# ExistentialRobotics/CORSAIR

Hardware: AMD Instinct MI355X
Metric: end-to-end queries/sec (embed+retrieve+register), Scan2CAD chair (higher is better)
Workload: dtype f32 sparse conv + embedding / f64 RANSAC, k-NN, Chamfer, top-k / f16 MFMA bounds and shortlists (survivors recounted in f64)

## Files before the change

### corsair_amd/_lib.py

```python
from __future__ import annotations

import ctypes
import threading
import os
import re
from ctypes import POINTER, c_char_p, c_double, c_float, c_int, c_int32, c_int64, c_uint64, c_void_p

_HERE = os.path.dirname(os.path.abspath(__file__))
LIB_PATH = os.environ.get("CORSAIR_HIP_LIB") or os.path.join(_HERE, "csrc", "libcorsair_hip.so")
HEADER_PATH = os.path.join(os.path.dirname(_HERE), "include", "corsair_hip.h")

_lib = None


class CorsairHipError(RuntimeError):
    """Raised when a cs_* entry point returns a negative status (message = cs_last_error())."""


def _declare(lib):
    vp = c_void_p
    sigs = {
        "cs_last_error": (c_char_p, []),
        "cs_version": (c_int, []),
        "cs_device_count": (c_int, []),
        "cs_coordmap_create": (c_int, [vp, c_int64, c_int, vp, POINTER(vp)]),
        "cs_coordmap_stride": (c_int, [vp, c_int, vp, POINTER(vp)]),
        "cs_coordmap_pyramid": (c_int, [vp, c_int64, c_int, c_int, c_int, vp, POINTER(vp)]),
        "cs_coordmap_size": (c_int64, [vp]),
        "cs_coordmap_tensor_stride": (c_int, [vp]),
        "cs_coordmap_coords": (vp, [vp]),
        "cs_coordmap_free": (None, [vp]),
        "cs_kernelmap_build": (c_int, [vp, vp, c_int, c_int, vp, POINTER(vp)]),
        "cs_kernelmap_build_many": (c_int, [c_int, POINTER(vp), POINTER(vp), POINTER(c_int), POINTER(c_int), vp, POINTER(vp)]),
        "cs_kernelmap_num_pairs": (c_int64, [vp]),
        "cs_kernelmap_rows": (c_int64, [vp]),
        "cs_kernelmap_table": (vp, [vp]),
        "cs_kernelmap_export": (c_int64, [vp, vp, vp, vp, c_int64, vp]),
        "cs_kernelmap_free": (None, [vp]),
        "cs_conv_fwd": (c_int, [vp, c_int64, c_int64, vp, c_int, c_int, vp, c_int, vp, vp, vp,
                                c_int, c_int, vp, c_int, vp]),
        "cs_conv_wgrad": (c_int, [vp, c_int64, c_int64, vp, c_int, c_int, vp, c_int, c_int, vp, vp]),
        "cs_affine_act": (c_int, [c_int64, c_int, vp, c_int, vp, vp, vp, c_int, c_int, vp, c_int, vp]),
        "cs_row_l2_normalize": (c_int, [c_int64, c_int, vp, c_int, c_float, vp, c_int, vp]),
        "cs_segmented_max": (c_int, [c_int64, c_int, vp, c_int, vp, c_int, c_int, vp, vp]),
        "cs_instance_norm": (c_int, [c_int64, c_int, vp, c_int, vp, c_int, vp, vp, c_float, vp, c_int, vp]),
        "cs_voxelize": (c_int, [vp, POINTER(c_int64), c_int, c_double, vp, vp, POINTER(c_int64), vp]),
        "cs_voxelize_f64": (c_int, [vp, POINTER(c_int64), c_int, c_double, vp, vp, POINTER(c_int64), vp]),
        "cs_l2_topk": (c_int, [vp, c_int64, vp, c_int64, c_int, c_int, vp, vp, vp]),
        "cs_l2_topk_sq": (c_int, [vp, c_int64, vp, c_int64, c_int, c_int, vp, vp, vp]),
        "cs_knn_feat": (c_int, [vp, POINTER(c_int64), vp, POINTER(c_int64), POINTER(c_int32),
                                POINTER(c_int32), c_int, c_int, c_int, vp, vp, vp, vp, vp, vp]),
        "cs_chamfer_1dir": (c_int, [vp, POINTER(c_int64), vp, POINTER(c_int64), POINTER(c_int32),
                                    POINTER(c_int32), c_int, vp, vp, vp]),
        "cs_chamfer_2dir": (c_int, [vp, POINTER(c_int64), vp, POINTER(c_int64), POINTER(c_int32),
                                    POINTER(c_int32), c_int, vp, vp, vp]),
        "cs_hausdorff_1dir": (c_int, [vp, POINTER(c_int64), vp, POINTER(c_int64), POINTER(c_int32),
                                      POINTER(c_int32), c_int, vp, vp, vp]),
        "cs_ransac_batch": (c_int, [vp, vp, POINTER(c_int64), c_int, c_double, c_int, c_int, c_double,
                                    c_uint64, vp, vp, vp, vp, vp]),
        "cs_ransac_prefilter_stats": (None, [POINTER(c_uint64), c_int]),
        "cs_knn_shortlist_stats": (None, [POINTER(c_uint64), c_int]),
        "cs_chamfer_f16_stats": (None, [POINTER(c_uint64), c_int]),
        "cs_l2_topk_stats": (None, [POINTER(c_uint64), c_int]),
        "cs_topk_catalog_create": (c_int, [vp, c_int64, c_int, vp, POINTER(vp)]),
        "cs_l2_topk_catalog": (c_int, [vp, c_int64, vp, c_int, vp, vp, c_int, vp]),
        "cs_topk_catalog_free": (None, [vp]),
        "cs_symcut_fit": (c_int, [vp, c_int, vp, POINTER(c_int64), c_int, vp, c_int,
                                  POINTER(c_int32), c_int, c_int, c_int, vp, vp, vp, vp, vp]),
        "cs_symcut_labels": (c_int, [vp, POINTER(c_int64), c_int, POINTER(c_int32), vp, vp, vp]),
        "cs_partition_by_label": (c_int, [vp, vp, c_int, vp, vp]),
        "cs_cfg_bad": (c_int, [vp, c_int, vp, c_int, vp, vp]),
        "cs_rows_nonfinite": (c_int, [vp, c_int, vp, c_int, vp, vp]),
        "cs_corr_assemble": (c_int, [vp, vp, vp, vp, c_int, vp, c_int, c_int64, vp, vp, vp]),
        "cs_radius_pairs": (c_int, [vp, POINTER(c_int64), vp, POINTER(c_int64), POINTER(c_int32), POINTER(c_int32),
                                    c_int, c_double, c_int, vp, vp, POINTER(vp)]),
        "cs_radius_pairs_fill": (c_int, [vp, vp, vp, vp]),
        "cs_radius_plan_free": (None, [vp]),
        "cs_sample_pairs": (c_int, [vp, POINTER(c_int64), POINTER(c_int32), POINTER(c_int32), POINTER(c_int32),
                                    POINTER(c_int32), c_int, POINTER(c_int64), vp, vp, c_int, c_uint64, c_int,
                                    c_double, c_int, vp, vp, vp, vp, vp]),
        "cs_transform_f64": (c_int, [vp, POINTER(c_int64), POINTER(c_int32), c_int, vp, vp, vp]),
        "cs_pair_loss_fwd": (c_int, [c_int, POINTER(vp), POINTER(c_int64), POINTER(c_int32), c_int, c_int,
                                     POINTER(c_int32), POINTER(c_int32), POINTER(c_int32), POINTER(c_float),
                                     POINTER(c_double), POINTER(vp), POINTER(c_int64), vp, vp, vp]),
        "cs_pair_loss_bwd": (c_int, [c_int, POINTER(vp), POINTER(c_int64), POINTER(c_int32), c_int, c_int,
                                     POINTER(c_int32), POINTER(c_int32), POINTER(c_int32), POINTER(c_float),
                                     POINTER(c_double), POINTER(vp), POINTER(c_int64), vp, POINTER(vp),
                                     POINTER(c_int32), vp]),
        "cs_hardest_negatives": (c_int, [vp, c_int, vp, POINTER(c_int64), vp, c_int, vp, POINTER(c_int64),
                                         POINTER(c_int32), POINTER(c_int32), c_int, c_int, vp, c_int64, c_double, vp, vp,
                                         vp]),
        "cs_hardest_stats": (None, [POINTER(c_uint64), c_int]),
        "cs_icp_batch": (c_int, [vp, POINTER(c_int64), vp, POINTER(c_int64), POINTER(c_int32), POINTER(c_int32), c_int, vp,
                                 c_double, c_int, c_double, c_double, vp, vp, vp, vp, vp, vp, vp, vp]),
        "cs_icp_stats": (None, [POINTER(c_uint64), c_int]),
        "cs_icp_plane_batch": (c_int, [vp, POINTER(c_int64), vp, vp, POINTER(c_int64), POINTER(c_int32), POINTER(c_int32),
                                       c_int, vp, c_double, c_int, c_double, c_double, vp, vp, vp, vp, vp, vp, vp, vp]),
        "cs_icp_plane_robust_batch": (c_int, [vp, POINTER(c_int64), vp, vp, POINTER(c_int64), POINTER(c_int32),
                                              POINTER(c_int32), c_int, vp, c_double, c_int, c_double, c_double, c_int,
                                              c_double, vp, vp, vp, vp, vp, vp, vp, vp, vp]),
        "cs_icp_scale_batch": (c_int, [vp, POINTER(c_int64), vp, vp, POINTER(c_int64), POINTER(c_int32), POINTER(c_int32),
                                       c_int, vp, c_double, c_int, c_double, c_double, c_double, c_double, vp, vp, vp, vp,
                                       vp, vp, vp, vp, vp]),
        "cs_icp_gicp_batch": (c_int, [vp, vp, POINTER(c_int64), vp, vp, POINTER(c_int64), POINTER(c_int32), POINTER(c_int32),
                                      c_int, vp, c_double, c_int, c_double, c_double, c_double, vp, vp, vp, vp, vp, vp, vp,
                                      vp, vp]),
        "cs_estimate_normals": (c_int, [vp, POINTER(c_int64), c_int, c_int, vp, vp]),
        "cs_estimate_normals_hybrid": (c_int, [vp, POINTER(c_int64), c_int, c_double, c_int, vp, vp]),
        "cs_normals_stats": (None, [POINTER(c_uint64), c_int]),
        "cs_fgr_batch": (c_int, [vp, vp, POINTER(c_int64), c_int, c_double, c_double, c_double, c_int, c_int, c_double,
                                 c_int, c_uint64, vp, vp, vp, vp, vp, vp, vp]),
        "cs_prof_enable": (None, [c_int]),
        "cs_prof_reset": (None, []),
        "cs_prof_get": (c_int, [c_char_p, POINTER(c_double), POINTER(c_int64)]),
        "cs_prof_get_units": (c_int, [c_char_p, POINTER(c_double)]),
        "cs_pool_trim": (None, []),
        "cs_pool_stats": (None, [POINTER(c_uint64)]),
    }
    for name, (res, args) in sigs.items():
        fn = getattr(lib, name)
        fn.restype = res
        fn.argtypes = args
    return sigs


def header_symbols():
    with open(HEADER_PATH) as f:
        text = f.read()
    text = re.sub(r"/\*.*?\*/", "", text, flags=re.S)
    return sorted(set(re.findall(r"\b(cs_[a-z0-9_]+)\s*\(", text)))


def load():
    global _lib
    if _lib is None:
        if not os.path.exists(LIB_PATH):
            raise ImportError(
                f"{LIB_PATH} is missing: build it with `python -c 'import __graft_entry__ as g; "
                "g.build()'` (hipcc --offload-arch=gfx950). There is no CPU fallback."
            )
        lib = ctypes.CDLL(LIB_PATH)
        _declare(lib)
        _lib = lib
    return _lib


def check(rc):
    if rc < 0:
        raise CorsairHipError(load().cs_last_error().decode("utf-8", "replace"))
    return rc


def require_gpu():
    if load().cs_device_count() < 1:
        raise CorsairHipError("no HIP device visible: the corsair_amd hot path has no CPU fallback")


def ptr(t):
    if t is None:
        return None
    return c_void_p(t.data_ptr())


def stream_ptr():
    import torch

    return c_void_p(torch.cuda.current_stream().cuda_stream)


def i64_array(values):
    arr = (c_int64 * len(values))(*[int(v) for v in values])
    return arr


def i32_array(values):
    arr = (c_int32 * len(values))(*[int(v) for v in values])
    return arr


def prof_enable(on=True):
    load().cs_prof_enable(1 if on else 0)


def prof_reset():
    load().cs_prof_reset()


def prof_get(name):
    ms = c_double(0.0)
    n = c_int64(0)
    check(load().cs_prof_get(name.encode(), ctypes.byref(ms), ctypes.byref(n)))
    units = c_double(0.0)
    check(load().cs_prof_get_units(name.encode(), ctypes.byref(units)))
    return ms.value, n.value, units.value


_pinned = threading.local()


def to_host(*tensors):
    import torch

    cache = getattr(_pinned, "bufs", None)
    if cache is None:
        cache = _pinned.bufs = {}
    staged = []
    for i, t in enumerate(tensors):
        t = t.detach()
        key = (i, tuple(t.shape), t.dtype)
        buf = cache.get(key)
        if buf is None:
            if len(cache) > 64:
                cache.clear()
            buf = cache[key] = torch.empty(t.shape, dtype=t.dtype, pin_memory=True)
        buf.copy_(t, non_blocking=True)
        staged.append(buf)
    ev = torch.cuda.Event()
    ev.record()
    ev.synchronize()
    return [b.numpy().copy() for b in staged]
```

### corsair_amd/backend.py

```python
from __future__ import annotations

import ctypes
from ctypes import c_void_p
from typing import NamedTuple, Optional

import numpy as np
import torch

from . import _lib
from ._lib import check, i32_array, i64_array, ptr, stream_ptr

KERNEL_VOLUME = 27


def _dev(t, dtype, what):
    if not isinstance(t, torch.Tensor) or not t.is_cuda:
        raise _lib.CorsairHipError(f"{what} must be a device tensor (the HIP path has no CPU fallback)")
    if t.dtype != dtype:
        raise TypeError(f"{what} must be {dtype}, got {t.dtype}")
    return t


def _rows(t, what):
    if t.dim() != 2 or t.stride(1) != 1:
        raise ValueError(f"{what} must be 2-D with unit inner stride")
    return t, t.stride(0) if t.shape[0] > 1 else max(t.stride(0), t.shape[1])


class CoordMap:

    def __init__(self, handle, device):
        self._h = c_void_p(handle)
        self.device = device
        lib = _lib.load()
        self.n = int(lib.cs_coordmap_size(self._h))
        self.tensor_stride = int(lib.cs_coordmap_tensor_stride(self._h))
        self._coords = None

    @classmethod
    def create(cls, coords, tensor_stride=1):
        _lib.require_gpu()
        coords = _dev(coords, torch.int32, "coordinates").contiguous()
        if coords.dim() != 2 or coords.shape[1] != 4:
            raise ValueError("coordinates must be int32 [N, 4] (batch, x, y, z)")
        out = c_void_p()
        check(_lib.load().cs_coordmap_create(ptr(coords), coords.shape[0], tensor_stride,
                                             stream_ptr(), ctypes.byref(out)))
        return cls(out.value, coords.device)

    @classmethod
    def pyramid(cls, coords, n_levels=4, n_batch=0, tensor_stride=1):
        _lib.require_gpu()
        coords = _dev(coords, torch.int32, "coordinates").contiguous()
        if coords.dim() != 2 or coords.shape[1] != 4:
            raise ValueError("coordinates must be int32 [N, 4] (batch, x, y, z)")
        outs = (c_void_p * n_levels)()
        check(_lib.load().cs_coordmap_pyramid(ptr(coords), coords.shape[0], tensor_stride, n_levels, int(n_batch or 0),
                                              stream_ptr(), outs))
        return [cls(h, coords.device) for h in outs]

    def stride(self, s=2):
        out = c_void_p()
        check(_lib.load().cs_coordmap_stride(self._h, s, stream_ptr(), ctypes.byref(out)))
        return CoordMap(out.value, self.device)

    @property
    def coords(self):
        if self._coords is None:
            t = torch.empty((self.n, 4), dtype=torch.int32, device=self.device)
            if self.n:
                src = _lib.load().cs_coordmap_coords(self._h)
                _hip_memcpy_d2d(t.data_ptr(), src, self.n * 16)
            self._coords = t
        return self._coords

    def __del__(self):
        try:
            if self._h:
                _lib.load().cs_coordmap_free(self._h)
                self._h = None
        except Exception:
            pass


def _hip_memcpy_d2d(dst, src, nbytes):
    import ctypes as C

    hip = _hip_runtime()
    rc = hip.hipMemcpyAsync(c_void_p(dst), c_void_p(src), C.c_size_t(nbytes), 3,
                            c_void_p(torch.cuda.current_stream().cuda_stream))
    if rc != 0:
        raise _lib.CorsairHipError(f"hipMemcpyAsync failed with {rc}")


_hip = None


def _hip_runtime():
    global _hip
    if _hip is None:
        _hip = ctypes.CDLL("libamdhip64.so")
    return _hip


class KernelMap:

    def __init__(self, handle, in_map, out_map, transposed, kernel_size=3):
        self._h = c_void_p(handle)
        self.kvol = int(kernel_size) ** 3
        lib = _lib.load()
        self.n_out = int(lib.cs_kernelmap_rows(self._h))
        self.n_in = in_map.n
        self._num_pairs = None
        self.transposed = transposed
        self.stride1 = not transposed and in_map.tensor_stride == out_map.tensor_stride
        self.device = in_map.device

    @property
    def num_pairs(self):
        if self._num_pairs is None:
            self._num_pairs = int(_lib.load().cs_kernelmap_num_pairs(self._h))
        return self._num_pairs

    @classmethod
    def build(cls, in_map, out_map, kernel_size=3, transposed=False):
        out = c_void_p()
        check(_lib.load().cs_kernelmap_build(in_map._h, out_map._h, kernel_size,
                                             1 if transposed else 0, stream_ptr(),
                                             ctypes.byref(out)))
        return cls(out.value, in_map, out_map, transposed, kernel_size)

    @classmethod
    def build_many(cls, specs):
        full = [(sp[0], sp[1], sp[2] if len(sp) > 2 else 3, bool(sp[3]) if len(sp) > 3 else False) for sp in specs]
        n = len(full)
        if n == 0:
            return []
        VP, CI = c_void_p * n, ctypes.c_int * n
        ins = VP(*[sp[0]._h.value for sp in full])
        outs = VP(*[sp[1]._h.value for sp in full])
        ks = CI(*[int(sp[2]) for sp in full])
        tr = CI(*[1 if sp[3] else 0 for sp in full])
        kms = VP()
        check(_lib.load().cs_kernelmap_build_many(n, ins, outs, ks, tr, stream_ptr(), kms))
        return [cls(kms[i], full[i][0], full[i][1], full[i][3], full[i][2]) for i in range(n)]

    def export(self):
        n = max(self.num_pairs, 1)
        k = torch.empty(n, dtype=torch.int32, device=self.device)
        i = torch.empty(n, dtype=torch.int32, device=self.device)
        o = torch.empty(n, dtype=torch.int32, device=self.device)
        got = check(_lib.load().cs_kernelmap_export(self._h, ptr(k), ptr(i), ptr(o), n, stream_ptr()))
        return k[:got], i[:got], o[:got]

    def table(self):
        t = torch.empty((self.n_out, KERNEL_VOLUME), dtype=torch.int32, device=self.device)
        if self.n_out:
            _hip_memcpy_d2d(t.data_ptr(), _lib.load().cs_kernelmap_table(self._h), self.n_out * 27 * 4)
        return t

    def __del__(self):
        try:
            if self._h:
                _lib.load().cs_kernelmap_free(self._h)
                self._h = None
        except Exception:
            pass


def conv_fwd(kmap, x, weight, scale=None, shift=None, residual=None, relu=False, out=None,
             n_out=None):
    x, ld_in = _rows(_dev(x, torch.float32, "input features"), "input features")
    weight = _dev(weight, torch.float32, "kernel").contiguous()
    if weight.dim() == 2:
        cin, cout = weight.shape
    else:
        cin, cout = weight.shape[1], weight.shape[2]
    if x.shape[1] != cin:
        raise ValueError(f"input has {x.shape[1]} channels, kernel expects {cin}")
    n_in = x.shape[0]
    if kmap is None:
        n_out = n_in
    else:
        n_out = kmap.n_out
    if out is None:
        out = torch.empty((n_out, cout), dtype=torch.float32, device=x.device)
    out, ld_out = _rows(out, "output")
    if out.shape[0] != n_out or out.shape[1] != cout:
        raise ValueError("output buffer has the wrong shape")
    ld_res = 0
    if residual is not None:
        residual, ld_res = _rows(_dev(residual, torch.float32, "residual"), "residual")
    check(_lib.load().cs_conv_fwd(kmap._h if kmap is not None else None, n_in, n_out, ptr(x), ld_in,
                                  cin, ptr(weight), cout, ptr(scale), ptr(shift), ptr(residual),
                                  ld_res, 1 if relu else 0, ptr(out), ld_out, stream_ptr()))
    return out


def conv_wgrad(kmap, x, g):
    x, ld_in = _rows(_dev(x, torch.float32, "input features"), "input features")
    g, ld_g = _rows(_dev(g, torch.float32, "output gradient"), "output gradient")
    n_in, cin = x.shape
    n_out, cout = g.shape
    if kmap is not None and (kmap.n_in, kmap.n_out) != (n_in, n_out):
        raise ValueError(f"kernel map is for {kmap.n_in} -> {kmap.n_out} rows, tensors have {n_in} -> {n_out}")
    kvol = 1 if kmap is None else kmap.kvol
    dw = torch.empty((cin, cout) if kvol == 1 else (kvol, cin, cout), dtype=torch.float32, device=x.device)
    check(_lib.load().cs_conv_wgrad(kmap._h if kmap is not None else None, n_in, n_out, ptr(x), ld_in, cin, ptr(g),
                                    ld_g, cout, ptr(dw), stream_ptr()))
    return dw


def dgrad_weight(kmap, weight):
    if kmap is None or kmap.kvol == 1:
        return weight.reshape(weight.shape[-2:]).t().contiguous()
    if kmap.stride1:
        return weight.flip(0).transpose(1, 2).contiguous()
    return weight.transpose(1, 2).contiguous()


def conv_dgrad(kmap, rev_kmap, g, weight):
    wt = dgrad_weight(kmap, weight)
    if kmap is None:
        return conv_fwd(None, g, wt)
    if kmap.stride1:
        rev_kmap = kmap if rev_kmap is None else rev_kmap
    if rev_kmap is None or (rev_kmap.n_in, rev_kmap.n_out, rev_kmap.kvol) != (kmap.n_out, kmap.n_in, kmap.kvol):
        raise ValueError("conv_dgrad: the reverse map must take the forward's output rows to its input rows")
    return conv_fwd(rev_kmap, g, wt)


def affine_act(x, scale=None, shift=None, residual=None, relu=False, out=None):
    x, ld_in = _rows(_dev(x, torch.float32, "input"), "input")
    if out is None:
        out = torch.empty((x.shape[0], x.shape[1]), dtype=torch.float32, device=x.device)
    out, ld_out = _rows(out, "output")
    ld_res = 0
    if residual is not None:
        residual, ld_res = _rows(residual, "residual")
    check(_lib.load().cs_affine_act(x.shape[0], x.shape[1], ptr(x), ld_in, ptr(scale), ptr(shift),
                                    ptr(residual), ld_res, 1 if relu else 0, ptr(out), ld_out,
                                    stream_ptr()))
    return out


def row_l2_normalize(x, eps=0.0, out=None):
    if out is None and torch.is_grad_enabled() and x.requires_grad:
        from .autograd import RowL2NormalizeFunction

        return RowL2NormalizeFunction.apply(x, float(eps))
    x, ld_in = _rows(_dev(x, torch.float32, "input"), "input")
    if out is None:
        out = torch.empty((x.shape[0], x.shape[1]), dtype=torch.float32, device=x.device)
    out, ld_out = _rows(out, "output")
    check(_lib.load().cs_row_l2_normalize(x.shape[0], x.shape[1], ptr(x), ld_in, float(eps), ptr(out),
                                          ld_out, stream_ptr()))
    return out


def segmented_max(x, coords, n_batch):
    if torch.is_grad_enabled() and x.requires_grad:
        from .autograd import SegmentedMaxFunction

        return SegmentedMaxFunction.apply(x, coords, int(n_batch))
    x, ld_in = _rows(_dev(x, torch.float32, "input"), "input")
    coords = _dev(coords, torch.int32, "coords")
    out = torch.empty((n_batch, x.shape[1]), dtype=torch.float32, device=x.device)
    check(_lib.load().cs_segmented_max(x.shape[0], x.shape[1], ptr(x), ld_in, ptr(coords),
                                       coords.stride(0), n_batch, ptr(out), stream_ptr()))
    return out


def instance_norm(x, seg, weight=None, bias=None, eps=1e-8, out=None):
    x, ld_in = _rows(_dev(x, torch.float32, "input"), "input")
    seg = _dev(seg, torch.int32, "segment offsets").contiguous()
    if out is None:
        out = torch.empty((x.shape[0], x.shape[1]), dtype=torch.float32, device=x.device)
    out, ld_out = _rows(_dev(out, torch.float32, "output"), "output")
    if out.shape != x.shape:
        raise ValueError("instance_norm: output buffer has the wrong shape")
    w = _dev(weight, torch.float32, "weight").contiguous().reshape(-1) if weight is not None else None
    b = _dev(bias, torch.float32, "bias").contiguous().reshape(-1) if bias is not None else None
    for t, name in ((w, "weight"), (b, "bias")):
        if t is not None and t.numel() != x.shape[1]:
            raise ValueError("instance_norm: %s must have %d entries" % (name, x.shape[1]))
    check(_lib.load().cs_instance_norm(x.shape[0], x.shape[1], ptr(x), ld_in, ptr(seg), seg.numel() - 1,
                                       ptr(w) if w is not None else None, ptr(b) if b is not None else None,
                                       float(eps), ptr(out), ld_out, stream_ptr()))
    return out


def voxelize(xyz, offsets, voxel_size):
    f64 = torch.is_tensor(xyz) and xyz.dtype == torch.float64
    xyz = _dev(xyz, torch.float64 if f64 else torch.float32, "xyz").contiguous()
    n = xyz.shape[0]
    nseg = len(offsets) - 1
    keep = torch.empty(max(n, 1), dtype=torch.int64, device=xyz.device)
    grid = torch.empty((max(n, 1), 4), dtype=torch.int32, device=xyz.device)
    h_off = i64_array(offsets)
    h_out = (ctypes.c_int64 * (nseg + 1))()
    fn = _lib.load().cs_voxelize_f64 if f64 else _lib.load().cs_voxelize
    check(fn(ptr(xyz), h_off, nseg, float(voxel_size), ptr(keep), ptr(grid), h_out, stream_ptr()))
    out_off = [int(v) for v in h_out]
    m = out_off[-1]
    return keep[:m], grid[:m], out_off


class TopkCatalog:

    def __init__(self, x):
        self.x = _dev(x, torch.float32, "catalog").contiguous()
        out = c_void_p()
        check(_lib.load().cs_topk_catalog_create(ptr(self.x), self.x.shape[0], self.x.shape[1], stream_ptr(),
                                                 ctypes.byref(out)))
        self._h = out
        self.shape = self.x.shape

    def __del__(self):
        try:
            if self._h:
                _lib.load().cs_topk_catalog_free(self._h)
                self._h = None
        except Exception:
            pass


def l2_topk(q, x, k, return_distance=False, squared=False):
    q = _dev(q, torch.float32, "queries").contiguous()
    idx = torch.empty((q.shape[0], k), dtype=torch.int64, device=q.device)
    dist = torch.empty((q.shape[0], k), dtype=torch.float64, device=q.device) if return_distance else None
    if isinstance(x, TopkCatalog):
        if x.shape[1] != q.shape[1]:
            raise ValueError("query and catalog dimensions differ")
        check(_lib.load().cs_l2_topk_catalog(ptr(q), q.shape[0], x._h, k, ptr(idx), ptr(dist), 1 if squared else 0,
                                             stream_ptr()))
        return (idx, dist) if return_distance else idx
    x = _dev(x, torch.float32, "catalog").contiguous()
    fn = _lib.load().cs_l2_topk_sq if squared else _lib.load().cs_l2_topk
    check(fn(ptr(q), q.shape[0], ptr(x), x.shape[0], q.shape[1], k, ptr(idx), ptr(dist), stream_ptr()))
    return (idx, dist) if return_distance else idx


def knn_feat(qf, qoff, tf, toff, k, qseg=None, tseg=None, qlabel=None, tlabel=None, perm=None,
             return_distance=False):
    qf = _dev(qf, torch.float32, "query features").contiguous()
    tf = _dev(tf, torch.float32, "target features").contiguous()
    if qseg is None:
        qseg = list(range(len(qoff) - 1))
        tseg = list(range(len(toff) - 1))
    n_prob = len(qseg)
    total = sum(int(qoff[s + 1]) - int(qoff[s]) for s in qseg)
    idx = torch.empty((total, k), dtype=torch.int32, device=qf.device)
    dist = torch.empty((total, k), dtype=torch.float64, device=qf.device) if return_distance else None
    check(_lib.load().cs_knn_feat(ptr(qf), i64_array(qoff), ptr(tf), i64_array(toff), i32_array(qseg),
                                  i32_array(tseg), n_prob, qf.shape[1], k, ptr(qlabel), ptr(tlabel),
                                  ptr(perm), ptr(idx), ptr(dist), stream_ptr()))
    return (idx, dist) if return_distance else idx


def hardest_negatives(qf, qxyz, qoff, tf, txyz, toff, anchors, radius, qseg=None, tseg=None, return_distance=False):
    qf, ld_q = _rows(_dev(qf, torch.float32, "query features"), "query features")
    tf, ld_t = _rows(_dev(tf, torch.float32, "target features"), "target features")
    qxyz = _dev(qxyz, torch.float32, "query points").contiguous()
    txyz = _dev(txyz, torch.float32, "target points").contiguous()
    anchors = _dev(anchors, torch.int32, "anchors").contiguous()
    if qf.shape[1] != tf.shape[1]:
        raise ValueError("hardest_negatives: query and target widths differ")
    if qxyz.shape != (qf.shape[0], 3) or txyz.shape != (tf.shape[0], 3):
        raise ValueError("hardest_negatives: points must be [n, 3], one row per feature row")
    if anchors.dim() != 1:
        raise ValueError("hardest_negatives: anchors must be 1-D")
    if qseg is None:
        qseg = list(range(len(qoff) - 1))
        tseg = list(range(len(toff) - 1))
    if len(qseg) != len(tseg):
        raise ValueError("hardest_negatives: qseg and tseg differ in length")
    if qseg and (int(qoff[max(qseg) + 1]) > qf.shape[0] or int(toff[max(tseg) + 1]) > tf.shape[0]):
        raise ValueError("hardest_negatives: the offset tables exceed the feature matrices")
    n = anchors.shape[0]
    idx = torch.empty(n, dtype=torch.int32, device=qf.device)
    dist = torch.empty(n, dtype=torch.float64, device=qf.device) if return_distance else None
    check(_lib.load().cs_hardest_negatives(ptr(qf), ld_q, ptr(qxyz), i64_array(qoff), ptr(tf), ld_t, ptr(txyz),
                                           i64_array(toff), i32_array(qseg), i32_array(tseg), len(qseg),
                                           int(qf.shape[1]), ptr(anchors), n, float(radius), ptr(idx), ptr(dist),
                                           stream_ptr()))
    return (idx, dist) if return_distance else idx


def hardest_stats(reset=False):
    out = (ctypes.c_uint64 * 2)()
    _lib.load().cs_hardest_stats(out, 1 if reset else 0)
    return int(out[0]), int(out[1])


def chamfer_1dir(src, soff, tgt, toff, src_seg, tgt_seg, T):
    src = _dev(src, torch.float32, "source").contiguous()
    tgt = _dev(tgt, torch.float32, "target").contiguous()
    T = _dev(T, torch.float32, "transforms").contiguous()
    n_prob = len(src_seg)
    out = torch.empty(n_prob, dtype=torch.float64, device=src.device)
    check(_lib.load().cs_chamfer_1dir(ptr(src), i64_array(soff), ptr(tgt), i64_array(toff),
                                      i32_array(src_seg), i32_array(tgt_seg), n_prob, ptr(T), ptr(out),
                                      stream_ptr()))
    return out


def chamfer_2dir(src, soff, tgt, toff, src_seg, tgt_seg, T):
    src = _dev(src, torch.float32, "source").contiguous()
    tgt = _dev(tgt, torch.float32, "target").contiguous()
    T = _dev(T, torch.float32, "transforms").contiguous()
    n_prob = len(src_seg)
    if len(tgt_seg) != n_prob or T.numel() != 16 * n_prob:
        raise ValueError("chamfer_2dir: %d source segments, %d target segments, %d transform entries"
                         % (n_prob, len(tgt_seg), T.numel()))
    if src.dim() != 2 or src.shape[1] != 3 or tgt.dim() != 2 or tgt.shape[1] != 3:
        raise ValueError("chamfer_2dir: clouds must be [n,3]")
    for name, off, seg, rows in (("source", soff, src_seg, src.shape[0]), ("target", toff, tgt_seg, tgt.shape[0])):
        if n_prob and not (0 <= min(seg) and max(seg) + 1 < len(off)):
            raise ValueError("chamfer_2dir: a %s segment id is outside its offset table" % name)
        if n_prob and not (0 <= int(min(off)) and int(max(off)) <= rows):
            raise ValueError("chamfer_2dir: the %s offset table exceeds the cloud (%d rows)" % (name, rows))
    out = torch.empty((n_prob, 2), dtype=torch.float64, device=src.device)
    if n_prob == 0:
        return out
    check(_lib.load().cs_chamfer_2dir(ptr(src), i64_array(soff), ptr(tgt), i64_array(toff),
                                      i32_array(src_seg), i32_array(tgt_seg), n_prob, ptr(T), ptr(out),
                                      stream_ptr()))
    return out


def hausdorff_1dir(src, soff, tgt, toff, src_seg, tgt_seg, T):
    src = _dev(src, torch.float32, "source").contiguous()
    tgt = _dev(tgt, torch.float32, "target").contiguous()
    T = _dev(T, torch.float32, "transforms").contiguous()
    n_prob = len(src_seg)
    out = torch.empty(n_prob, dtype=torch.float64, device=src.device)
    check(_lib.load().cs_hausdorff_1dir(ptr(src), i64_array(soff), ptr(tgt), i64_array(toff),
                                        i32_array(src_seg), i32_array(tgt_seg), n_prob, ptr(T), ptr(out),
                                        stream_ptr()))
    return out


class IcpResult(NamedTuple):
    T: torch.Tensor
    T32: torch.Tensor
    fitness: torch.Tensor
    rmse: torch.Tensor
    iters: torch.Tensor
    ncorr: torch.Tensor
    corr: Optional[torch.Tensor]
    corr_off: Optional[list]
    wfitness: Optional[torch.Tensor] = None
    scale: Optional[torch.Tensor] = None
    mrmse = None


class GicpResult(IcpResult):
    def __new__(cls, *fields, mrmse=None):
        self = super().__new__(cls, *fields)
        self.mrmse = mrmse
        return self


ICP_KERNELS = {"l2": 0, "huber": 1, "cauchy": 2, "tukey": 3}


def estimate_normals(xyz, offsets, k=16, radius=None):
    xyz = _dev(xyz, torch.float32, "points").contiguous()
    if xyz.dim() != 2 or xyz.shape[1] != 3:
        raise ValueError("estimate_normals: points must be [n, 3]")
    if len(offsets) < 1 or int(offsets[-1]) > xyz.shape[0]:
        raise ValueError("estimate_normals: the offset table exceeds the point array")
    out = torch.empty_like(xyz)
    if radius is None:
        check(_lib.load().cs_estimate_normals(ptr(xyz), i64_array(offsets), len(offsets) - 1, int(k), ptr(out), stream_ptr()))
    else:
        check(_lib.load().cs_estimate_normals_hybrid(ptr(xyz), i64_array(offsets), len(offsets) - 1, float(radius), int(k),
                                                     ptr(out), stream_ptr()))
    return out


def normals_stats(reset=False):
    out = (ctypes.c_uint64 * 2)()
    _lib.load().cs_normals_stats(out, 1 if reset else 0)
    return int(out[0]), int(out[1])


def icp_batch(src, soff, tgt, toff, src_seg, tgt_seg, T0, max_dist, max_iter=30, relative_fitness=1e-6,
              relative_rmse=1e-6, return_corr=False, tgt_normals=None, kernel="l2", kernel_scale=None, with_scaling=False,
              scale_bounds=(0.5, 2.0), *, estimation=None, src_normals=None, gicp_epsilon=1e-3):
    if estimation not in (None, "gicp"):
        raise ValueError("icp_batch: estimation must be None or 'gicp', got %r" % (estimation,))
    gicp = estimation == "gicp"
    if gicp:
        if kernel != "l2" or with_scaling:
            raise ValueError("icp_batch: estimation 'gicp' with a robust kernel or with_scaling is out of scope")
        if tgt_normals is None or src_normals is None:
            raise ValueError("icp_batch: estimation 'gicp' needs tgt_normals and src_normals")
        eps = float(gicp_epsilon)
        if not (np.isfinite(eps) and 2.0 ** -10 <= eps <= 1.0):
            raise ValueError("icp_batch: gicp_epsilon must lie in [2^-10, 1], got %r" % (gicp_epsilon,))
    elif src_normals is not None:
        raise ValueError("icp_batch: src_normals are used by estimation = 'gicp' only")
    if with_scaling:
        if kernel != "l2":
            raise ValueError("icp_batch: with_scaling with a robust kernel (%r) is out of scope: robust kernels exist for "
                             "the rigid plane estimation only" % (kernel,))
        try:
            smin, smax = float(scale_bounds[0]), float(scale_bounds[1])
        except (TypeError, ValueError, IndexError):
            raise ValueError("icp_batch: scale_bounds must be a pair (min, max), got %r" % (scale_bounds,))
        if not (np.isfinite(smin) and np.isfinite(smax) and 0.0 < smin <= 1.0 <= smax):
            raise ValueError("icp_batch: scale_bounds must be finite with 0 < min <= 1 <= max, got %r" % (scale_bounds,))
    if kernel not in ICP_KERNELS:
        raise ValueError("icp_batch: kernel must be one of %s, got %r" % (sorted(ICP_KERNELS), kernel))
    if kernel != "l2" and tgt_normals is None:
        raise ValueError("icp_batch: kernel %r needs tgt_normals (robust kernels exist for the plane estimation only)"
                         % (kernel,))
    if kernel != "l2" and kernel_scale is None:
        raise ValueError("icp_batch: kernel %r needs a kernel_scale" % (kernel,))
    src = _dev(src, torch.float32, "source").contiguous()
    tgt = _dev(tgt, torch.float32, "target").contiguous()
    T0 = _dev(T0, torch.float32, "initial transforms").contiguous()
    n_prob = len(src_seg)
    if len(tgt_seg) != n_prob:
        raise ValueError("icp_batch: src_seg and tgt_seg differ in length")
    if T0.numel() != 16 * n_prob:
        raise ValueError("icp_batch: one 4x4 initial transform per problem")
    if src.dim() != 2 or src.shape[1] != 3 or tgt.dim() != 2 or tgt.shape[1] != 3:
        raise ValueError("icp_batch: points must be [n, 3]")
    sane = all(0 <= int(s) < len(soff) - 1 for s in src_seg) and all(0 <= int(t) < len(toff) - 1 for t in tgt_seg)
    if n_prob and sane and (int(soff[max(src_seg) + 1]) > src.shape[0] or int(toff[max(tgt_seg) + 1]) > tgt.shape[0]):
        raise ValueError("icp_batch: the offset tables exceed the point arrays")
    if n_prob and not sane and min(min(src_seg), min(tgt_seg)) >= 0:
        raise ValueError("icp_batch: a segment id exceeds its offset table")
    dev = src.device
    T = torch.empty((n_prob, 4, 4), dtype=torch.float64, device=dev)
    T32 = torch.empty((n_prob, 4, 4), dtype=torch.float32, device=dev)
    fitness = torch.empty(n_prob, dtype=torch.float64, device=dev)
    rmse = torch.empty(n_prob, dtype=torch.float64, device=dev)
    iters = torch.empty(n_prob, dtype=torch.int32, device=dev)
    ncorr = torch.empty(n_prob, dtype=torch.int32, device=dev)
    corr = corr_off = None
    if return_corr:
        lens = [int(soff[s + 1]) - int(soff[s]) for s in src_seg] if sane else []
        corr_off = np.concatenate([[0], np.cumsum(lens)]).astype(np.int64).tolist()
        corr = torch.full((max(corr_off[-1], 1),), -1, dtype=torch.int32, device=dev)
    head = (i64_array(toff), i32_array(src_seg), i32_array(tgt_seg), n_prob, ptr(T0), float(max_dist), int(max_iter),
            float(relative_fitness), float(relative_rmse))
    tail = head + (ptr(T), ptr(T32), ptr(fitness), ptr(rmse), ptr(iters), ptr(ncorr), ptr(corr), stream_ptr())
    wfitness = scale = None
    nrm = None
    if tgt_normals is not None:
        nrm = _dev(tgt_normals, torch.float32, "target normals").contiguous()
        if nrm.shape != tgt.shape:
            raise ValueError("icp_batch: tgt_normals must have the shape of the target points")
    mrmse = None
    if gicp:
        snrm = _dev(src_normals, torch.float32, "source normals").contiguous()
        if snrm.shape != src.shape:
            raise ValueError("icp_batch: src_normals must have the shape of the source points")
        mrmse = torch.empty(n_prob, dtype=torch.float64, device=dev)
        check(_lib.load().cs_icp_gicp_batch(
            ptr(src), ptr(snrm), i64_array(soff), ptr(tgt), ptr(nrm), *head, eps, ptr(T), ptr(T32), ptr(fitness), ptr(rmse),
            ptr(mrmse), ptr(iters), ptr(ncorr), ptr(corr), stream_ptr()))
    elif with_scaling:
        scale = torch.empty(n_prob, dtype=torch.float64, device=dev)
        check(_lib.load().cs_icp_scale_batch(
            ptr(src), i64_array(soff), ptr(tgt), ptr(nrm), *head, smin, smax, ptr(T), ptr(T32), ptr(fitness), ptr(rmse),
            ptr(scale), ptr(iters), ptr(ncorr), ptr(corr), stream_ptr()))
    elif nrm is None:
        check(_lib.load().cs_icp_batch(ptr(src), i64_array(soff), ptr(tgt), *tail))
    else:
        if kernel == "l2":
            check(_lib.load().cs_icp_plane_batch(ptr(src), i64_array(soff), ptr(tgt), ptr(nrm), *tail))
        else:
            wfitness = torch.empty(n_prob, dtype=torch.float64, device=dev)
            check(_lib.load().cs_icp_plane_robust_batch(
                ptr(src), i64_array(soff), ptr(tgt), ptr(nrm), *head, ICP_KERNELS[kernel], float(kernel_scale), ptr(T),
                ptr(T32), ptr(fitness), ptr(rmse), ptr(wfitness), ptr(iters), ptr(ncorr), ptr(corr), stream_ptr()))
    if corr is not None:
        corr = corr[:corr_off[-1]]
    if gicp:
        return GicpResult(T, T32, fitness, rmse, iters, ncorr, corr, corr_off, wfitness, scale, mrmse=mrmse)
    return IcpResult(T, T32, fitness, rmse, iters, ncorr, corr, corr_off, wfitness, scale)


def icp_stats(reset=False):
    out = (ctypes.c_uint64 * 2)()
    _lib.load().cs_icp_stats(out, 1 if reset else 0)
    return int(out[0]), int(out[1])


def ransac_batch(src, tgt, offsets, max_corr, ransac_n=10, max_iter=100000, confidence=0.999, seed=0):
    src = _dev(src, torch.float32, "source correspondences").contiguous()
    tgt = _dev(tgt, torch.float32, "target correspondences").contiguous()
    n_prob = len(offsets) - 1
    dev = src.device
    T = torch.empty((n_prob, 4, 4), dtype=torch.float32, device=dev)
    inl = torch.empty(n_prob, dtype=torch.int32, device=dev)
    rmse = torch.empty(n_prob, dtype=torch.float64, device=dev)
    iters = torch.empty(n_prob, dtype=torch.int32, device=dev)
    check(_lib.load().cs_ransac_batch(ptr(src), ptr(tgt), i64_array(offsets), n_prob, float(max_corr),
                                      ransac_n, max_iter, float(confidence), int(seed), ptr(T),
                                      ptr(inl), ptr(rmse), ptr(iters), stream_ptr()))
    return T, inl, rmse, iters


class FgrResult(NamedTuple):
    T: torch.Tensor
    T64: torch.Tensor
    inliers: torch.Tensor
    rmse: torch.Tensor
    iters: torch.Tensor
    n_tuple: torch.Tensor


def fgr_batch(src, tgt, offsets, max_corr, mu_floor=0.025, division_factor=1.4, iteration_number=64, tuple_test=True,
              tuple_scale=0.95, max_tuple=1000, seed=0):
    src = _dev(src, torch.float32, "source correspondences").contiguous()
    tgt = _dev(tgt, torch.float32, "target correspondences").contiguous()
    if src.shape != tgt.shape or src.dim() != 2 or src.shape[1] != 3:
        raise ValueError("fgr_batch: correspondences must be two [M, 3] arrays of one shape")
    if len(offsets) < 1 or int(offsets[-1]) > src.shape[0]:
        raise ValueError("fgr_batch: the offset table exceeds the correspondence arrays")
    n_prob = len(offsets) - 1
    dev = src.device
    T = torch.empty((n_prob, 4, 4), dtype=torch.float32, device=dev)
    T64 = torch.empty((n_prob, 4, 4), dtype=torch.float64, device=dev)
    inl = torch.empty(n_prob, dtype=torch.int32, device=dev)
    rmse = torch.empty(n_prob, dtype=torch.float64, device=dev)
    iters = torch.empty(n_prob, dtype=torch.int32, device=dev)
    n_tuple = torch.empty(n_prob, dtype=torch.int32, device=dev)
    check(_lib.load().cs_fgr_batch(ptr(src), ptr(tgt), i64_array(offsets), n_prob, float(max_corr), float(mu_floor),
                                   float(division_factor), int(iteration_number), 1 if tuple_test else 0,
                                   float(tuple_scale), int(max_tuple), int(seed) & 0xFFFFFFFFFFFFFFFF, ptr(T), ptr(T64),
                                   ptr(inl), ptr(rmse), ptr(iters), ptr(n_tuple), stream_ptr()))
    return FgrResult(T, T64, inl, rmse, iters, n_tuple)


def partition_by_label(label, d_off, n_cloud):
    label = _dev(label, torch.int32, "labels").contiguous()
    order = torch.empty(label.shape[0], dtype=torch.int64, device=label.device)
    check(_lib.load().cs_partition_by_label(ptr(label), ptr(d_off), n_cloud, ptr(order), stream_ptr()))
    return order


def cfg_bad(nn, d_first, n_cfg):
    nn = _dev(nn, torch.int32, "neighbour lists").contiguous()
    bad = torch.empty(n_cfg, dtype=torch.int32, device=nn.device)
    check(_lib.load().cs_cfg_bad(ptr(nn), nn.shape[1], ptr(d_first), n_cfg, ptr(bad), stream_ptr()))
    return bad


def rows_nonfinite(x, d_first, n_seg):
    x = _dev(x, torch.float32, "rows").contiguous()
    bad = torch.empty(n_seg, dtype=torch.int32, device=x.device)
    check(_lib.load().cs_rows_nonfinite(ptr(x), x.shape[1], ptr(d_first), n_seg, ptr(bad), stream_ptr()))
    return bad


def corr_assemble(xyz0, xyz1, rows, nn, desc, total, max_len):
    xyz0 = _dev(xyz0, torch.float32, "query xyz").contiguous()
    xyz1 = _dev(xyz1, torch.float32, "CAD xyz").contiguous()
    nn = _dev(nn, torch.int32, "neighbour lists").contiguous()
    k = nn.shape[1]
    dev = xyz0.device
    src = torch.empty((total * k, 3), dtype=torch.float32, device=dev)
    tgt = torch.empty((total * k, 3), dtype=torch.float32, device=dev)
    d_desc = torch.from_numpy(np.ascontiguousarray(desc, dtype=np.int64)).to(dev, non_blocking=True)
    check(_lib.load().cs_corr_assemble(ptr(xyz0), ptr(xyz1), ptr(rows) if rows is not None else None, ptr(nn), k,
                                       ptr(d_desc), len(desc), int(max_len), ptr(src), ptr(tgt), stream_ptr()))
    return src, tgt


def symcut_fit(feat, xyz, offsets, anchors, Ks, n_nn=50, n_init=10, max_iter=300):
    feat = _dev(feat, torch.float32, "features").contiguous()
    xyz = _dev(xyz, torch.float32, "xyz").contiguous()
    anchors = _dev(anchors, torch.int32, "anchors").contiguous()
    nc, na = anchors.shape
    dev = feat.device
    centers = torch.empty((nc, na, 4, 3), dtype=torch.float64, device=dev)
    counts = torch.empty((nc, na, 4), dtype=torch.int32, device=dev)
    mcd = torch.empty((nc, na), dtype=torch.float64, device=dev)
    mer = torch.empty((nc, na), dtype=torch.float64, device=dev)
    check(_lib.load().cs_symcut_fit(ptr(feat), feat.shape[1], ptr(xyz), i64_array(offsets), nc,
                                    ptr(anchors), na, i32_array(Ks), n_nn, n_init, max_iter,
                                    ptr(centers), ptr(counts), ptr(mcd), ptr(mer), stream_ptr()))
    return centers, counts, mcd, mer


def symcut_labels(xyz, offsets, Ks, sel_centers):
    xyz = _dev(xyz, torch.float32, "xyz").contiguous()
    sel_centers = _dev(sel_centers, torch.float64, "centres").contiguous()
    labels = torch.empty(xyz.shape[0], dtype=torch.int32, device=xyz.device)
    check(_lib.load().cs_symcut_labels(ptr(xyz), i64_array(offsets), len(Ks), i32_array(Ks),
                                       ptr(sel_centers), ptr(labels), stream_ptr()))
    return labels


class RadiusPlan:

    def __init__(self, handle, keep):
        self._h = c_void_p(handle)
        self._keep = keep

    def fill(self, row_ptr, total):
        idx = torch.empty(max(int(total), 1), dtype=torch.int32, device=row_ptr.device)
        check(_lib.load().cs_radius_pairs_fill(self._h, ptr(row_ptr), ptr(idx), stream_ptr()))
        return idx[:int(total)]

    def __del__(self):
        try:
            if self._h:
                _lib.load().cs_radius_plan_free(self._h)
                self._h = None
        except Exception:
            pass


def radius_pairs_begin(src, soff, tgt, toff, src_seg=None, tgt_seg=None, radius=0.03, k=None):
    src = _dev(src, torch.float64, "source points").contiguous()
    tgt = _dev(tgt, torch.float64, "target points").contiguous()
    if src_seg is None:
        src_seg = list(range(len(soff) - 1))
        tgt_seg = list(range(len(toff) - 1))
    if len(src_seg) != len(tgt_seg):
        raise ValueError("radius_pairs: src_seg and tgt_seg differ in length")
    if k is not None and int(k) < 1:
        raise ValueError("radius_pairs: k must be None or >= 1")
    rows = sum(int(soff[s + 1]) - int(soff[s]) for s in src_seg)
    row_ptr = torch.empty(rows + 1, dtype=torch.int64, device=src.device)
    plan = c_void_p()
    check(_lib.load().cs_radius_pairs(ptr(src), i64_array(soff), ptr(tgt), i64_array(toff), i32_array(src_seg),
                                      i32_array(tgt_seg), len(src_seg), float(radius), int(k or 0), ptr(row_ptr),
                                      stream_ptr(), ctypes.byref(plan)))
    return row_ptr, RadiusPlan(plan.value, (src, tgt))


def radius_pairs(src, soff, tgt, toff, src_seg=None, tgt_seg=None, radius=0.03, k=None):
    row_ptr, plan = radius_pairs_begin(src, soff, tgt, toff, src_seg, tgt_seg, radius, k)
    total = int(_lib.to_host(row_ptr[-1:])[0][0])
    return row_ptr, plan.fill(row_ptr, total)


def sample_pairs(xyz, offsets, base_seg, pos_seg, neg_seg, slots, row_base, row_ptr, tgt_idx, lists, seed, round_,
                 radius, sample, out=None):
    xyz = _dev(xyz, torch.float32, "points").contiguous()
    n_prob = len(base_seg)
    dev = xyz.device
    if out is None:
        out = tuple(torch.zeros((n_prob * sample, 2), dtype=torch.int32, device=dev) for _ in range(3)) + (
            torch.zeros((n_prob, 4), dtype=torch.int32, device=dev),)
    pip, pin, nin, counts = out
    if tgt_idx is not None and tgt_idx.numel() == 0:
        tgt_idx = torch.zeros(1, dtype=torch.int32, device=dev)
    check(_lib.load().cs_sample_pairs(ptr(xyz), i64_array(offsets), i32_array(base_seg), i32_array(pos_seg),
                                      i32_array(neg_seg), i32_array(slots), n_prob, i64_array(row_base), ptr(row_ptr),
                                      ptr(tgt_idx), int(lists), int(seed) & 0xFFFFFFFFFFFFFFFF, int(round_),
                                      float(radius), int(sample), ptr(pip), ptr(pin), ptr(nin), ptr(counts),
                                      stream_ptr()))
    return out


def transform_f64(xyz, offsets, seg, T):
    xyz = _dev(xyz, torch.float32, "points").contiguous()
    T = _dev(T, torch.float64, "transforms").contiguous()
    if T.shape[0] != len(seg):
        raise ValueError("transform_f64: one transform per segment")
    total = sum(int(offsets[s + 1]) - int(offsets[s]) for s in seg)
    out = torch.empty((max(total, 1), 3), dtype=torch.float64, device=xyz.device)
    check(_lib.load().cs_transform_f64(ptr(xyz), i64_array(offsets), i32_array(seg), len(seg), ptr(T), ptr(out),
                                       stream_ptr()))
    return out[:total]


PAIR_PULL, PAIR_PUSH = 0, 1


def _pair_loss_args(mats, terms):
    if not mats:
        raise ValueError("pair_loss: no feature matrix")
    C = int(mats[0].shape[1])
    lds = []
    for m in mats:
        _dev(m, torch.float32, "features")
        _, ld = _rows(m, "features")
        if int(m.shape[1]) != C:
            raise ValueError("pair_loss: the feature matrices differ in width")
        lds.append(ld)
    pairs = []
    for t in terms:
        p = _dev(t[2], torch.int32, "pairs")
        if p.dim() != 2 or p.shape[1] != 2:
            raise ValueError("pair_loss: pairs must be [P, 2]")
        pairs.append(p.contiguous())
    vp = (c_void_p * len(mats))(*[m.data_ptr() for m in mats])
    pp = (c_void_p * max(len(terms), 1))(*[p.data_ptr() if p.numel() else None for p in pairs])
    head = (len(mats), vp, i64_array([m.shape[0] for m in mats]), i32_array(lds), C, len(terms),
            i32_array([t[0] for t in terms]), i32_array([t[1] for t in terms]), i32_array([t[3] for t in terms]),
            (ctypes.c_float * max(len(terms), 1))(*[float(t[4]) for t in terms]),
            (ctypes.c_double * max(len(terms), 1))(*[float(t[5]) for t in terms]), pp,
            i64_array([p.shape[0] for p in pairs]))
    return head, pairs, C


def pair_loss_fwd(mats, terms, out=None):
    head, keep, _ = _pair_loss_args(mats, terms)
    dev = mats[0].device
    if out is None:
        out = (torch.empty(max(len(terms), 1), dtype=torch.float64, device=dev),
               torch.empty(1, dtype=torch.float32, device=dev))
    check(_lib.load().cs_pair_loss_fwd(*head, ptr(out[0]), ptr(out[1]), stream_ptr()))
    return out[0][:len(terms)], out[1]


def pair_loss_bwd(mats, terms, grad_up, out=None):
    head, keep, C = _pair_loss_args(mats, terms)
    g = _dev(grad_up, torch.float32, "upstream gradient").reshape(-1)
    if g.numel() != 1:
        raise ValueError("pair_loss_bwd: the upstream gradient is one scalar")
    if out is None:
        out = [torch.empty((m.shape[0], C), dtype=torch.float32, device=m.device) for m in mats]
    lds = [_rows(_dev(o, torch.float32, "gradient"), "gradient")[1] for o in out]
    gp = (c_void_p * len(out))(*[o.data_ptr() for o in out])
    check(_lib.load().cs_pair_loss_bwd(*head, ptr(g), gp, i32_array(lds), stream_ptr()))
    return out
```

### corsair_amd/csrc/ransac.hip

```cpp
#include <math.h>

#include <algorithm>
#include <atomic>
#include <vector>

#include "ransac.h"

namespace cs {

__device__ __forceinline__ int est_bound(int c, int m, int ransac_n, double log_1mc, int est_k0) {
  const double ratio = fmin(1.0, (double)c / (double)m);
  double pw = 1.0;
  for (int j = 0; j < ransac_n; ++j) pw = pw * ratio;
  const double den = log(1.0 - pw);
  if (den < 0.0) {
    const double est = log_1mc / den;
    if (est < (double)est_k0) return (int)ceil(est);
  }
  return est_k0;
}

__global__ __launch_bounds__(256) void k_ransac_scan1(RansacProb* probs, int n_prob,
                                                     const int32_t* __restrict__ res_cnt, int it0,
                                                     int bcount, int bmax, int ransac_n,
                                                     int max_iter, double log_1mc,
                                                     int32_t* __restrict__ cand, int* n_active,
                                                     const unsigned long long* __restrict__ err_by_h,
                                                     const double* __restrict__ hyp, int32_t* __restrict__ next_nsurv,
                                                     int* __restrict__ next_nactive) {
  extern __shared__ int32_t lcnt[];
  const int p = blockIdx.x;
  if (err_by_h && threadIdx.x == 0) {
    next_nsurv[p] = 0;
    if (p == 0) *next_nactive = 0;
  }
  RansacProb pr = probs[p];
  if (pr.done) return;
  const int seg = (bcount + 63) / 64;
  {
    const int32_t* g = res_cnt + (int64_t)p * bmax;
    for (int h = threadIdx.x; h < bcount; h += 256) lcnt[h + h / seg] = g[h];
  }
  __syncthreads();
  if (threadIdx.x >= 64) return;
  const int lane = threadIdx.x;
  const int32_t* cnt = lcnt + lane;
  const int s0 = lane * seg, s1 = min(bcount, s0 + seg);
  int lmax = 0;
  for (int h = s0; h < s1; ++h)
    if (it0 + h < pr.est_k) lmax = max(lmax, cnt[h]);
  int incl = lmax;
#pragma unroll
  for (int off = 1; off < 64; off <<= 1) {
    const int o = __shfl_up(incl, off);
    if (lane >= off) incl = max(incl, o);
  }
  int pre = __shfl_up(incl, 1);
  if (lane == 0) pre = 0;
  pre = max(pre, pr.best_cnt);
  int stop = 0x7fffffff;
  {
    int cur = pre;
    int ek = cur > pr.best_cnt ? est_bound(cur, pr.m, ransac_n, log_1mc, pr.est_k) : pr.est_k;
    for (int h = s0; h < s1; ++h) {
      if (it0 + h >= ek) {
        stop = h;
        break;
      }
      const int c = cnt[h];
      if (c > cur) {
        cur = c;
        ek = est_bound(cur, pr.m, ransac_n, log_1mc, pr.est_k);
      }
    }
  }
#pragma unroll
  for (int off = 32; off >= 1; off >>= 1) stop = min(stop, __shfl_xor(stop, off));
  if (stop > bcount) stop = bcount;
  int cmax = 0;
  for (int h = s0; h < min(s1, stop); ++h) cmax = max(cmax, cnt[h]);
#pragma unroll
  for (int off = 32; off >= 1; off >>= 1) cmax = max(cmax, __shfl_xor(cmax, off));
  int new_ek = pr.est_k;
  if (cmax > pr.best_cnt) new_ek = est_bound(cmax, pr.m, ransac_n, log_1mc, pr.est_k);
  int ncand = 0;
  unsigned long long e_min = ~0ULL;
  int h_min = 0x7fffffff;
  if (cmax > 0 && cmax >= pr.best_cnt) {
    if (err_by_h) {
      for (int h = s0; h < min(s1, stop); ++h)
        if (cnt[h] == cmax) {
          const unsigned long long e = err_by_h[(int64_t)p * bmax + h];
          if (e < e_min) {
            e_min = e;
            h_min = h;
          }
        }
#pragma unroll
      for (int off = 32; off >= 1; off >>= 1) {
        const unsigned long long eo = __shfl_xor(e_min, off);
        const int ho = __shfl_xor(h_min, off);
        if (eo < e_min || (eo == e_min && ho < h_min)) {
          e_min = eo;
          h_min = ho;
        }
      }
    } else {
      int mine = 0;
      for (int h = s0; h < min(s1, stop); ++h) mine += cnt[h] == cmax;
      int incl2 = mine;
#pragma unroll
      for (int off = 1; off < 64; off <<= 1) {
        const int o = __shfl_up(incl2, off);
        if (lane >= off) incl2 += o;
      }
      int pos = incl2 - mine;
      ncand = __shfl(incl2, 63);
      for (int h = s0; h < min(s1, stop); ++h)
        if (cnt[h] == cmax) cand[(int64_t)p * bmax + pos++] = h;
    }
  }
  if (lane == 0) {
    const int consumed = it0 + stop;
    pr.est_k = new_ek;
    pr.n_cand = ncand;
    pr.chunk_max = cmax;
    if (consumed >= pr.est_k || consumed >= max_iter) {
      pr.done = 1;
      pr.iters = consumed < max_iter ? consumed : max_iter;
    } else {
      atomicAdd(n_active, 1);
    }
    if (err_by_h && h_min != 0x7fffffff && (cmax > pr.best_cnt || e_min < pr.best_err)) {
      pr.best_cnt = cmax;
      pr.best_err = e_min;
      pr.best_itr = it0 + h_min;
      for (int c = 0; c < 12; ++c) pr.best_T[c] = hyp[((int64_t)p * 12 + c) * bmax + h_min];
    }
    probs[p] = pr;
  }
}

__global__ void k_ransac_scan2(RansacProb* probs, int n_prob, const double* __restrict__ hyp,
                               const int32_t* __restrict__ cand,
                               const unsigned long long* __restrict__ cand_err, int by_h, int it0,
                               int bmax, int32_t* __restrict__ next_nsurv, int* __restrict__ next_nactive) {
  const int p = blockIdx.x * blockDim.x + threadIdx.x;
  if (p >= n_prob) return;
  next_nsurv[p] = 0;
  if (p == 0) *next_nactive = 0;
  RansacProb pr = probs[p];
  if (pr.n_cand <= 0) return;
  bool changed = false;
  int best_h = -1;
  for (int c = 0; c < pr.n_cand; ++c) {
    const unsigned long long e = cand_err[(int64_t)p * bmax + (by_h ? cand[(int64_t)p * bmax + c] : c)];
    if (pr.chunk_max > pr.best_cnt || e < pr.best_err) {
      pr.best_cnt = pr.chunk_max;
      pr.best_err = e;
      best_h = cand[(int64_t)p * bmax + c];
      changed = true;
    }
  }
  pr.n_cand = 0;
  if (changed) {
    pr.best_itr = it0 + best_h;
    for (int c = 0; c < 12; ++c) pr.best_T[c] = hyp[((int64_t)p * 12 + c) * bmax + best_h];
  }
  probs[p] = pr;
}

__global__ void k_ransac_finish(const RansacProb* __restrict__ probs, int n_prob, double scale,
                                float* __restrict__ T, int32_t* __restrict__ inliers,
                                double* __restrict__ rmse, int32_t* __restrict__ iters) {
  const int p = blockIdx.x * blockDim.x + threadIdx.x;
  if (p >= n_prob) return;
  const RansacProb pr = probs[p];
  float* o = T + (int64_t)p * 16;
  if (pr.best_cnt > 0) {
    for (int c = 0; c < 12; ++c) o[c] = (float)pr.best_T[c];
  } else {
    for (int c = 0; c < 12; ++c) o[c] = (c % 5 == 0) ? 1.f : 0.f;
  }
  o[12] = 0.f;
  o[13] = 0.f;
  o[14] = 0.f;
  o[15] = 1.f;
  if (inliers) inliers[p] = pr.best_cnt;
  if (rmse)
    rmse[p] = pr.best_cnt > 0 ? sqrt(((double)pr.best_err / scale) / (double)pr.best_cnt) : 0.0;
  if (iters) iters[p] = pr.iters;
}

}

using namespace cs;

namespace {
std::atomic<unsigned long long> g_pf_stats[5];

struct PinnedScratch {
  char* p = nullptr;
  size_t n = 0;
  ~PinnedScratch() {
    if (p) (void)hipHostFree(p);
  }
};
thread_local PinnedScratch t_pinned;
char* pinned_scratch(size_t bytes) {
  if (t_pinned.n < bytes) {
    if (t_pinned.p) (void)hipHostFree(t_pinned.p);
    t_pinned.p = nullptr;
    t_pinned.n = 0;
    void* q = nullptr;
    if (hipHostMalloc(&q, bytes, hipHostMallocDefault) != hipSuccess) return nullptr;
    t_pinned.p = static_cast<char*>(q);
    t_pinned.n = bytes;
  }
  return t_pinned.p;
}

struct Options {
  bool prefilter;
  bool check;
  int pf_nm;
  bool stage2;
  int first_chunk;
  int force_jacobi;
  bool overlap;
  int trace_it0;
  const char* trace_file;
};
Options read_options() {
  const char* pf = getenv("CS_RANSAC_PREFILTER");
  const char* ck = getenv("CS_RANSAC_CHECK");
  const char* k = getenv("CS_RANSAC_PF_K");
  const char* s2 = getenv("CS_RANSAC_STAGE2");
  const char* first = getenv("CS_RANSAC_FIRST");
  const char* jac = getenv("CS_RANSAC_JACOBI");
  const char* ov = getenv("CS_RANSAC_OVERLAP");
  const char* tr = getenv("CS_PF_TRACE");
  const char* trf = getenv("CS_PF_TRACE_FILE");
  Options o;
  o.prefilter = !(pf && pf[0] == '0');
  o.check = ck && ck[0] == '1';
  o.pf_nm = (k && atoi(k) == 32) ? 2 : 1;
  o.stage2 = !(s2 && s2[0] == '0');
  o.first_chunk = ((std::min(std::max(first ? atoi(first) : 64, 64), BMAX) + 63) / 64) * 64;
  o.force_jacobi = jac && atoi(jac) != 0;
  o.overlap = !(ov && ov[0] == '0');
  o.trace_it0 = tr ? atoi(tr) : -1;
  o.trace_file = trf ? trf : "/tmp/pf_trace.bin";
  return o;
}

struct Scratch {
  int n_prob = 0;
  size_t st_probs = 0, st_surv = 0, st_cnt = 0, st_bytes = 0;
  PoolBuf<char> state;
  char* h_state = nullptr;
  PoolBuf<float> pk;
  PoolBuf<float4> pair32;
  PoolBuf<double> hyp;
  PoolBuf<int32_t> res_cnt, cand;
  PoolBuf<unsigned long long> cand_err;
  PoolBuf<int64_t> off16;
  PoolBuf<_Float16> B16, A16;
  PoolBuf<float> c_h;
  PoolBuf<int32_t> cnt_up, hlist;
  PoolBuf<unsigned> pf_stat;
  PoolBuf<double> pf_sums;
  PoolBuf<_Float16> B32, A16s;
  PoolBuf<float> c_hs;
  PoolBuf<int32_t> cnt2;
  PoolBuf<int32_t> exact_dbg;
  PoolBuf<unsigned long long> chk_stats;
  PoolBuf<int32_t> xcd_buf;
  PoolBuf<unsigned long long> trace;
  size_t trace_cap = 1;

  bool alloc(int n, int64_t tot1, int64_t rows16, int pf_nm, bool pf, bool stage2, bool check, bool tracing) {
    n_prob = n;
    st_probs = sizeof(RansacProb) * (size_t)n;
    st_surv = ((sizeof(int32_t) * (size_t)n + 7) / 8) * 8;
    st_cnt = st_surv + 8;
    st_bytes = st_probs + 2 * st_cnt;
    h_state = pinned_scratch(st_bytes);
    const size_t nb = (size_t)n * BMAX, ns2 = (size_t)n * PF_S2_CAP;
    if (tracing) trace_cap = (size_t)8 * n * 64 * 16 * 16;
    return h_state && state.alloc(st_bytes) && pk.alloc((size_t)tot1 * 6) && pair32.alloc((size_t)tot1 * 2) &&
           hyp.alloc(2 * nb * 12) && res_cnt.alloc(nb) && cand.alloc(nb) && cand_err.alloc(nb) && off16.alloc(n + 1) &&
           B16.alloc(pf ? (size_t)rows16 * pf_pitch(pf_nm) : 8) && A16.alloc(pf ? 2 * nb * PF_K : 8) &&
           c_h.alloc(pf ? 2 * nb : 1) && cnt_up.alloc(pf ? 2 * nb : 1) && hlist.alloc(pf ? nb : 1) &&
           pf_stat.alloc((size_t)n * PF_STAT) && pf_sums.alloc((size_t)n * 6) &&
           B32.alloc(stage2 ? (size_t)rows16 * PF_PITCH : 8) && A16s.alloc(stage2 ? ns2 * PF_K : 8) &&
           c_hs.alloc(stage2 ? ns2 : 1) && cnt2.alloc(stage2 ? ns2 : 1) &&
           exact_dbg.alloc(check ? nb : 1) && chk_stats.alloc(4) && xcd_buf.alloc((size_t)16 * n) && trace.alloc(trace_cap);
  }
  RansacProb* probs() const { return reinterpret_cast<RansacProb*>(state.p); }
  int32_t* nsurv(int par) const { return reinterpret_cast<int32_t*>(state.p + st_probs + par * st_cnt); }
  int* nactive(int par) const { return reinterpret_cast<int*>(state.p + st_probs + par * st_cnt + st_surv); }
  const int32_t* h_nsurv(int par) const { return reinterpret_cast<const int32_t*>(h_state + st_probs + par * st_cnt); }
  int h_nactive(int par) const { return *reinterpret_cast<const int*>(h_state + st_probs + par * st_cnt + st_surv); }
  double* hyp_of(int par) const { return hyp.p + (size_t)par * n_prob * 12 * BMAX; }
  _Float16* A16_of(int par) const { return A16.p + (size_t)par * n_prob * BMAX * PF_K; }
  float* c_h_of(int par) const { return c_h.p + (size_t)par * n_prob * BMAX; }
  int32_t* cnt_up_of(int par) const { return cnt_up.p + (size_t)par * n_prob * BMAX; }
  int32_t* xcd_of(int par) const { return xcd_buf.p + (size_t)par * 8 * n_prob; }
};

struct Event {
  hipEvent_t e = nullptr;
  ~Event() {
    if (e) (void)hipEventDestroy(e);
  }
};
struct SideDrain {
  hipStream_t st = nullptr;
  bool clean = false;
  ~SideDrain() {
    if (st && !clean) (void)hipStreamSynchronize(st);
  }
};

struct RansacCall {
  int n_prob = 0, ransac_n = 0, max_iter = 0, m_max = 0;
  uint64_t seed = 0;
  int64_t total = 0, tot1 = 1;
  double thr2 = 0.0, scale = 0.0, log_1mc = 0.0, tcap = 0.0;
  Options opt;
  bool pf_alloc = false, stage2 = false, check = false;
  std::vector<RansacProb> hp;
  std::vector<int64_t> h_off16;
  std::vector<int32_t> h_xcd[2];
  Scratch sc;
  Event round_done, front_done[2], hyp_done[2];
  hipStream_t s = nullptr, side = nullptr, side_hyp = nullptr;
  SideDrain side_drain, side_hyp_drain;
  int max_surv_prev = 1 << 30;
  unsigned long long tot_surv = 0, tot_eval = 0;
  size_t trace_n = 0;

  int init(const int64_t* h_off, int n, double max_corr, int rn, int iters, double confidence, uint64_t sd, hipStream_t st);
  int setup(const float* d_src, const float* d_tgt);
  int open_streams();
  RansacIn in() const { return RansacIn{sc.probs(), n_prob, m_max, tot1, sc.pk.p, sc.pair32.p}; }
  bool prefiltered(int it0) const { return pf_alloc && it0 >= opt.first_chunk; }
  int chunk_of(int it0) const {
    const int b = it0 < opt.first_chunk ? opt.first_chunk : it0 < 512 ? 512 - it0 : (it0 < BMAX ? it0 : BMAX);
    return b > max_iter - it0 ? max_iter - it0 : b;
  }
  int chunk_splits(int tiles) const {
    int splits = (int)(4096 / ((int64_t)n_prob * tiles > 0 ? (int64_t)n_prob * tiles : 1));
    if (splits < 1) splits = 1;
    if (splits > 16) splits = 16;
    while (splits > 1 && m_max / splits < 4 * RC_CHUNK) --splits;
    return splits;
  }
  int place(int it0, int par, int* live);
  Front enqueue_front(int it0, int par, hipStream_t st);
  int back_half(const Front& cur);
  int count_chunk(const Front& cur, double eval_pairs);
  int count_survivors(const Front& cur, bool* err_known);
  bool read_back(const Front& cur);
  int finish(float* d_T, int32_t* d_inliers, double* d_rmse, int32_t* d_iters);
};

int RansacCall::init(const int64_t* h_off, int n, double max_corr, int rn, int iters, double confidence, uint64_t sd,
                     hipStream_t st) {
  n_prob = n;
  ransac_n = rn;
  max_iter = iters;
  seed = sd;
  s = st;
  total = h_off[n_prob] - h_off[0];
  tot1 = total ? total : 1;
  hp.resize(n_prob);
  h_off16.assign(n_prob + 1, 0);
  for (int p = 0; p < n_prob; ++p) {
    int64_t m = h_off[p + 1] - h_off[p];
    CS_REQUIRE(m >= 0 && m < (1LL << 24), CS_ERR_INVALID,
               "cs_ransac_batch: bad segment %d (a problem holds fewer than 2^24 correspondences)", p);
    RansacProb& pr = hp[p];
    memset(&pr, 0, sizeof(pr));
    pr.off = h_off[p];
    pr.m = (int32_t)m;
    pr.est_k = max_iter;
    pr.best_itr = -1;
    pr.done = m < ransac_n ? 1 : 0;
    if (m > m_max) m_max = (int)m;
    h_off16[p + 1] = h_off16[p] + pf_padded(m);
  }
  thr2 = max_corr * max_corr;
  int ex = 0;
  (void)frexp(thr2, &ex);
  scale = ldexp(1.0, 38 - ex);
  log_1mc = log(1.0 - confidence);
  opt = read_options();
  pf_alloc = opt.prefilter && total > 0 && max_iter > opt.first_chunk;
  stage2 = pf_alloc && opt.pf_nm == 1 && opt.stage2;
  check = pf_alloc && opt.check;
  tcap = opt.pf_nm == 2 ? 0.0 : PF_TCAP;
  const bool ok = sc.alloc(n_prob, tot1, h_off16[n_prob] ? h_off16[n_prob] : 1, opt.pf_nm, pf_alloc, stage2, check,
                           opt.trace_it0 >= 0);
  CS_REQUIRE(ok, CS_ERR_HIP, "cs_ransac_batch: scratch allocation failed");
  return CS_OK;
}

int RansacCall::setup(const float* d_src, const float* d_tgt) {
  memset(sc.h_state, 0, sc.st_bytes);
  memcpy(sc.h_state, hp.data(), sc.st_probs);
  CS_HIP_CHECK(hipMemcpyAsync(sc.state.p, sc.h_state, sc.st_bytes, hipMemcpyHostToDevice, s));
  if (pf_alloc) {
    CS_HIP_CHECK(hipMemcpyAsync(sc.off16.p, h_off16.data(), sizeof(int64_t) * (n_prob + 1),
                                hipMemcpyHostToDevice, s));
    ransac_launch_images(in(), sc.off16.p, d_src, d_tgt, sc.pf_sums.p, sc.pf_stat.p, sc.chk_stats.p,
                         opt.pf_nm == 2 ? sc.B16.p : (stage2 ? sc.B32.p : nullptr), opt.pf_nm == 1 ? sc.B16.p : nullptr, tcap, s);
    CS_LAUNCH_CHECK();
  } else if (total > 0) {
    ransac_launch_pack(in(), d_src, d_tgt, s);
    CS_LAUNCH_CHECK();
  }
  if (opt.trace_it0 >= 0) CS_HIP_CHECK(hipMemsetAsync(sc.trace.p, 0, sizeof(unsigned long long) * sc.trace_cap, s));
  return CS_OK;
}

int RansacCall::open_streams() {
  for (Event* ev : {&round_done, &front_done[0], &front_done[1], &hyp_done[0], &hyp_done[1]})
    CS_HIP_CHECK(hipEventCreateWithFlags(&ev->e, hipEventDisableTiming));
  side = opt.overlap ? side_stream() : nullptr;
  side_hyp = side ? side_stream(1) : nullptr;
  side_drain.st = side;
  side_hyp_drain.st = side_hyp;
  return CS_OK;
}

int RansacCall::place(int it0, int par, int* live) {
  std::vector<int> order;
  for (int p = 0; p < n_prob; ++p)
    if (!hp[p].done && hp[p].est_k > it0) order.push_back(p);
  *live = (int)order.size();
  std::sort(order.begin(), order.end(), [&](int a, int c) { return hp[a].m > hp[c].m; });
  std::vector<std::vector<int>> lists(8);
  int64_t load[8] = {0, 0, 0, 0, 0, 0, 0, 0};
  for (int p : order) {
    int best = 0;
    for (int x = 1; x < 8; ++x)
      if (load[x] < load[best]) best = x;
    lists[best].push_back(p);
    load[best] += pf_padded(hp[p].m);
  }
  int pslots = 1;
  for (int x = 0; x < 8; ++x) pslots = std::max(pslots, (int)lists[x].size());
  std::vector<int32_t>& tab = h_xcd[par];
  tab.assign((size_t)8 * pslots, -1);
  for (int x = 0; x < 8; ++x)
    for (size_t i = 0; i < lists[x].size(); ++i) tab[(size_t)x * pslots + i] = lists[x][i];
  return pslots;
}

Front RansacCall::enqueue_front(int it0, int par, hipStream_t st) {
  Front f;
  f.it0 = it0;
  f.b = chunk_of(it0);
  f.par = par;
  f.pf = prefiltered(it0);
  f.on_side = st != s;
  const int b = f.b;
  int live = 0;
  f.pslots = place(it0, par, &live);
  const int pslots = f.pslots;
  hipStream_t sh = (f.on_side && f.pf && side_hyp) ? side_hyp : st;
  if (pslots <= XCD_SLOTS) {
    memcpy(f.xtab.v, h_xcd[par].data(), sizeof(int32_t) * 8 * pslots);
  } else {
    (void)hipMemcpyAsync(sc.xcd_of(par), h_xcd[par].data(), sizeof(int32_t) * 8 * pslots, hipMemcpyHostToDevice, sh);
    f.xcd_prob = sc.xcd_of(par);
  }
  _Float16* A16_r = f.pf ? sc.A16_of(par) : nullptr;
  float* c_h_r = f.pf ? sc.c_h_of(par) : nullptr;
  int32_t* cnt_up_r = f.pf ? sc.cnt_up_of(par) : nullptr;
  const int ptiles = (b + PF_HYP - 1) / PF_HYP;
  int psplits = (int)((8 * 1024 + (int64_t)live * ptiles - 1) / std::max<int64_t>((int64_t)live * ptiles, 1));
  if (psplits < 1) psplits = 1;
  if (psplits > 16) psplits = 16;
  while (psplits > 1 && m_max / psplits < 8 * PF_ROWS) --psplits;
  {
    ProfScope prof("ransac_hyp", sh);
    int32_t* fz = psplits > 1 ? cnt_up_r : nullptr;
    ransac_launch_hyp(in(), f, ransac_n, seed, opt.force_jacobi, sc.hyp_of(par), sc.pf_stat.p, sc.pf_sums.p, thr2, tcap, A16_r,
                      c_h_r, fz, sh);
  }
  if (f.pf) {
    if (sh != st) {
      (void)hipEventRecord(hyp_done[par].e, sh);
      (void)hipStreamWaitEvent(st, hyp_done[par].e, 0);
    }
    ProfScope prof("ransac_pre", st);
    unsigned long long* tr = (opt.trace_it0 == it0) ? sc.trace.p : nullptr;
    const unsigned nblk = ransac_launch_prefilter(opt.pf_nm, in(), sc.off16.p, sc.B16.p, A16_r, c_h_r, f, ptiles, psplits,
                                                  cnt_up_r, tr, nullptr, st);
    if (tr) trace_n = (size_t)nblk * 16;
  }
  if (f.on_side) (void)hipEventRecord(front_done[par].e, st);
  return f;
}

int RansacCall::count_chunk(const Front& cur, double eval_pairs) {
  const int b = cur.b;
  const int hpw = b <= 64 ? 64 : RC_HYP;
  const int tiles = (b + hpw - 1) / hpw;
  const int splits = chunk_splits(tiles);
  if (splits > 1 || hpw != RC_HYP)
    CS_HIP_CHECK(hipMemset2DAsync(sc.res_cnt.p, sizeof(int32_t) * BMAX, 0, sizeof(int32_t) * b, n_prob, s));
  ProfScope prof("ransac_eval", s, 30.0 * eval_pairs);
  ransac_launch_count_chunk(in(), sc.hyp_of(cur.par), cur.it0, b, hpw, tiles, splits, thr2, sc.res_cnt.p, s);
  return CS_OK;
}

int RansacCall::count_survivors(const Front& cur, bool* err_known) {
  const int b = cur.b;
  const double* hyp_r = sc.hyp_of(cur.par);
  const int32_t* cnt_up_r = sc.cnt_up_of(cur.par);
  int32_t* const d_nsurv = sc.nsurv(cur.par);
  const int surv_cap = std::min(max_surv_prev, b);
  const bool few = max_surv_prev <= FEW_MAX || b <= FEW_MAX;
  const bool run_s2 = stage2 && few && surv_cap <= PF_S2_CAP;
  Stage2Rows s2rows{};
  if (run_s2) {
    s2rows.A16 = sc.A16_of(cur.par);
    s2rows.c_h = sc.c_h_of(cur.par);
    s2rows.stat = sc.pf_stat.p;
    s2rows.tcap = tcap;
    s2rows.A16s = sc.A16s.p;
    s2rows.c_hs = sc.c_hs.p;
    s2rows.cnt2 = sc.cnt2.p;
  }
  ransac_launch_survivors(in(), cur, cnt_up_r, sc.res_cnt.p, sc.cand_err.p, sc.hlist.p, d_nsurv, s2rows, s);
  {
    ProfScope prof("ransac_eval", s);
    if (few) {
      if (run_s2) {
        const int s2tiles = std::max(1, (std::min(b, PF_S2_CAP) + PF_HYP - 1) / PF_HYP);
        int s2splits = 8;
        while (s2splits > 1 && m_max / s2splits < 8 * PF_ROWS) --s2splits;
        ransac_launch_prefilter(2, in(), sc.off16.p, sc.B32.p, sc.A16s.p, sc.c_hs.p, cur, s2tiles, s2splits, sc.cnt2.p, nullptr,
                                d_nsurv, s);
      }
      const int fslots = surv_cap <= 256 ? 4 : 8;
      ransac_launch_count_few(in(), hyp_r, thr2, scale, sc.res_cnt.p, sc.cand_err.p, sc.hlist.p, d_nsurv, fslots,
                              run_s2 ? sc.cnt2.p : nullptr, s);
      *err_known = true;
    } else {
      ransac_launch_count_list(in(), hyp_r, cur.it0, b, thr2, sc.res_cnt.p, sc.hlist.p, d_nsurv, s);
    }
  }
  if (check) {
    const int tiles = (b + RC_HYP - 1) / RC_HYP;
    const int splits = chunk_splits(tiles);
    CS_HIP_CHECK(hipMemset2DAsync(sc.exact_dbg.p, sizeof(int32_t) * BMAX, 0, sizeof(int32_t) * b, n_prob, s));
    ransac_launch_count_chunk(in(), hyp_r, cur.it0, b, RC_HYP, tiles, splits, thr2, sc.exact_dbg.p, s);
    ransac_launch_check(in(), cur, sc.exact_dbg.p, cnt_up_r, sc.hlist.p, d_nsurv, run_s2 ? sc.cnt2.p : nullptr, sc.chk_stats.p, s);
  }
  return CS_OK;
}

int RansacCall::back_half(const Front& cur) {
  const int it0 = cur.it0, b = cur.b;
  double eval_pairs = 0.0;
  for (int p = 0; p < n_prob; ++p) {
    if (hp[p].done) continue;
    const int nh = std::min(hp[p].est_k - it0, b);
    if (nh > 0) {
      eval_pairs += (double)nh * (double)hp[p].m;
      tot_eval += (unsigned long long)nh;
    }
  }
  bool err_known = false;
  if (!cur.pf) {
    if (int rc = count_chunk(cur, eval_pairs)) return rc;
  } else {
    prof_add_units("ransac_pre", 30.0 * eval_pairs);
    if (int rc = count_survivors(cur, &err_known)) return rc;
  }
  static const hipError_t scan1_lds = hipFuncSetAttribute(
      reinterpret_cast<const void*>(k_ransac_scan1), hipFuncAttributeMaxDynamicSharedMemorySize, 80 * 1024);
  CS_REQUIRE(scan1_lds == hipSuccess, CS_ERR_HIP, "cs_ransac_batch: cannot reserve LDS for k_ransac_scan1");
  RansacProb* const d_probs = sc.probs();
  const double* hyp_r = sc.hyp_of(cur.par);
  int32_t* const next_nsurv = sc.nsurv(cur.par ^ 1);
  int* const next_nactive = sc.nactive(cur.par ^ 1);
  hipLaunchKernelGGL(k_ransac_scan1, dim3((unsigned)n_prob), dim3(256), sizeof(int32_t) * (b + 64), s, d_probs, n_prob,
                     sc.res_cnt.p, it0, b, BMAX, ransac_n, max_iter, log_1mc, sc.cand.p, sc.nactive(cur.par),
                     err_known ? sc.cand_err.p : (const unsigned long long*)nullptr, hyp_r, next_nsurv, next_nactive);
  if (!err_known) {
    ransac_launch_err(in(), hyp_r, sc.cand.p, thr2, scale, sc.cand_err.p, s);
    hipLaunchKernelGGL(k_ransac_scan2, dim3((unsigned)ceil_div(n_prob, 64)), dim3(64), 0, s,
                       d_probs, n_prob, hyp_r, sc.cand.p, sc.cand_err.p, 0, it0, BMAX, next_nsurv, next_nactive);
  }
  CS_LAUNCH_CHECK();
  return CS_OK;
}

bool RansacCall::read_back(const Front& cur) {
  if (cur.pf) {
    const int32_t* h_surv = sc.h_nsurv(cur.par);
    max_surv_prev = 0;
    for (int p = 0; p < n_prob; ++p)
      if (!hp[p].done) {
        tot_surv += (unsigned long long)h_surv[p];
        if (h_surv[p] > max_surv_prev) max_surv_prev = h_surv[p];
      }
  }
  memcpy(hp.data(), sc.h_state, sc.st_probs);
  return sc.h_nactive(cur.par) != 0;
}

int RansacCall::finish(float* d_T, int32_t* d_inliers, double* d_rmse, int32_t* d_iters) {
  if (trace_n) {
    std::vector<unsigned long long> ht(trace_n);
    CS_HIP_CHECK(hipMemcpy(ht.data(), sc.trace.p, sizeof(unsigned long long) * trace_n, hipMemcpyDeviceToHost));
    FILE* f = fopen(opt.trace_file, "wb");
    if (f) {
      fwrite(ht.data(), sizeof(unsigned long long), trace_n, f);
      fclose(f);
    }
  }
  g_pf_stats[3] += tot_surv;
  g_pf_stats[4] += tot_eval;
  if (check) {
    unsigned long long h_stats[4] = {0, 0, 0, 0};
    CS_HIP_CHECK(hipMemcpyAsync(h_stats, sc.chk_stats.p, sizeof(h_stats), hipMemcpyDeviceToHost, s));
    CS_HIP_CHECK(hipStreamSynchronize(s));
    g_pf_stats[0] += h_stats[0];
    g_pf_stats[1] += h_stats[1];
    g_pf_stats[2] += h_stats[2];
    CS_REQUIRE(h_stats[0] == 0, CS_ERR_INTERNAL,
               "cs_ransac_batch: prefilter bound violated for %llu hypotheses", h_stats[0]);
  }
  hipLaunchKernelGGL(k_ransac_finish, dim3((unsigned)ceil_div(n_prob, 64)), dim3(64), 0, s,
                     sc.probs(), n_prob, scale, d_T, d_inliers, d_rmse, d_iters);
  CS_LAUNCH_CHECK();
  CS_HIP_CHECK(hipStreamSynchronize(s));
  side_drain.clean = true;
  side_hyp_drain.clean = true;
  return CS_OK;
}
}

extern "C" {

void cs_ransac_prefilter_stats(uint64_t out[5], int reset) {
  for (int i = 0; i < 5; ++i) {
    if (out) out[i] = g_pf_stats[i].load();
    if (reset) g_pf_stats[i].store(0);
  }
}

int cs_ransac_batch(const float* d_src, const float* d_tgt, const int64_t* h_off, int n_prob,
                    double max_corr, int ransac_n, int max_iter, double confidence, uint64_t seed,
                    float* d_T, int32_t* d_inliers, double* d_rmse, int32_t* d_iters,
                    void* stream) {
  CS_REQUIRE(h_off && d_T, CS_ERR_INVALID, "cs_ransac_batch: NULL argument");
  CS_REQUIRE(ransac_n >= 3 && ransac_n <= 64, CS_ERR_INVALID,
             "cs_ransac_batch: ransac_n %d not in [3, 64]", ransac_n);
  CS_REQUIRE(max_corr > 0.0 && max_iter >= 1, CS_ERR_INVALID,
             "cs_ransac_batch: need max_corr > 0 and max_iter >= 1");
  CS_REQUIRE(confidence > 0.0 && confidence <= 1.0, CS_ERR_INVALID,
             "cs_ransac_batch: confidence must be in (0, 1]");
  if (n_prob <= 0) return CS_OK;
  hipStream_t s = (hipStream_t)stream;
  pool_use_stream(s);
  const int64_t total = h_off[n_prob] - h_off[0];
  CS_REQUIRE(h_off[0] == 0 && total >= 0, CS_ERR_INVALID, "cs_ransac_batch: bad offsets");
  CS_REQUIRE(total == 0 || (d_src && d_tgt), CS_ERR_INVALID, "cs_ransac_batch: NULL correspondences");
  RansacCall c;
  if (int rc = c.init(h_off, n_prob, max_corr, ransac_n, max_iter, confidence, seed, s)) return rc;
  if (int rc = c.setup(d_src, d_tgt)) return rc;
  if (int rc = c.open_streams()) return rc;

  Front cur = c.enqueue_front(0, 0, s);
  CS_LAUNCH_CHECK();
  bool side_pending = false;
  int side_par = 0;
  while (true) {
    if (cur.on_side) {
      CS_HIP_CHECK(hipStreamWaitEvent(s, c.front_done[cur.par].e, 0));
      side_pending = false;
    }
    if (int rc = c.back_half(cur)) return rc;
    CS_HIP_CHECK(hipMemcpyAsync(c.sc.h_state, c.sc.state.p, c.sc.st_bytes, hipMemcpyDeviceToHost, s));
    CS_HIP_CHECK(hipEventRecord(c.round_done.e, s));
    Front nxt;
    const int it1 = cur.it0 + cur.b;
    const bool have_next = it1 < max_iter;
    if (have_next) {
      nxt = c.enqueue_front(it1, cur.par ^ 1, (c.side && cur.pf && c.prefiltered(it1)) ? c.side : s);
      if (nxt.on_side) {
        side_pending = true;
        side_par = nxt.par;
      }
      CS_LAUNCH_CHECK();
    }
    CS_HIP_CHECK(hipEventSynchronize(c.round_done.e));
    const bool active = c.read_back(cur);
    if (!active || !have_next) break;
    cur = nxt;
  }
  if (side_pending) CS_HIP_CHECK(hipStreamWaitEvent(s, c.front_done[side_par].e, 0));
  return c.finish(d_T, d_inliers, d_rmse, d_iters);
}

}
```

### corsair_amd/csrc/symcut.hip

```cpp
#include <algorithm>
#include <vector>

#include "common.h"
#define KM_DRAWS_QUAL __device__
#include "kmeans_draws.h"

namespace cs {

constexpr int SYM_MAX_NN = 64;
constexpr int SYM_SEL_J = 32;
constexpr int SYM_MAX_INIT = 10;

__device__ __forceinline__ double dist2_3(double ax, double ay, double az, double bx, double by,
                                          double bz) {
  const double dx = ax - bx, dy = ay - by, dz = az - bz;
  return fma(dz, dz, fma(dy, dy, dx * dx));
}

struct KmState {
  double cx[4], cy[4], cz[4];
};

__device__ __forceinline__ int nearest_center(const KmState& st, int K, double px, double py,
                                              double pz, double* dmin) {
  int best = 0;
  double bd = dist2_3(px, py, pz, st.cx[0], st.cy[0], st.cz[0]);
#pragma unroll
  for (int c = 1; c < 4; ++c) {
    if (c < K) {
      const double d = dist2_3(px, py, pz, st.cx[c], st.cy[c], st.cz[c]);
      if (d < bd) {
        bd = d;
        best = c;
      }
    }
  }
  *dmin = bd;
  return best;
}

__device__ __forceinline__ int block_excl_scan256(int v, int* wsum, int* total) {
  const int lane = threadIdx.x & 63, wave = threadIdx.x >> 6;
  int incl = v;
#pragma unroll
  for (int off = 1; off < 64; off <<= 1) {
    const int o = __shfl_up(incl, off);
    if (lane >= off) incl += o;
  }
  __syncthreads();
  if (lane == 63) wsum[wave] = incl;
  __syncthreads();
  int base = 0;
#pragma unroll
  for (int w = 0; w < 4; ++w) base += w < wave ? wsum[w] : 0;
  *total = wsum[0] + wsum[1] + wsum[2] + wsum[3];
  return base + incl - v;
}

constexpr int SYM_KEYS_MAX_ANCHOR = 128;
template <int DIM>
__global__ __launch_bounds__(256) void k_symcut_keys(const float* __restrict__ feat,
                                                     const int64_t* __restrict__ off,
                                                     const int32_t* __restrict__ anchors, int n_anchor,
                                                     unsigned long long* __restrict__ key_scratch,
                                                     const int64_t* __restrict__ key_off) {
  __shared__ double af[SYM_KEYS_MAX_ANCHOR][DIM];
  const int cloud = blockIdx.y;
  const int64_t base = off[cloud];
  const int n = (int)(off[cloud + 1] - base);
  if ((int)blockIdx.x * 256 >= n) return;
  for (int a0 = 0; a0 < n_anchor; a0 += SYM_KEYS_MAX_ANCHOR) {
    const int na = min(SYM_KEYS_MAX_ANCHOR, n_anchor - a0);
    __syncthreads();
    for (int i = threadIdx.x; i < na * DIM; i += 256) {
      const int a = i / DIM, c = i - a * DIM;
      af[a][c] = (double)feat[(base + anchors[(int64_t)cloud * n_anchor + a0 + a]) * DIM + c];
    }
    __syncthreads();
    const int row = blockIdx.x * 256 + threadIdx.x;
    if (row < n) {
      double f[DIM];
#pragma unroll
      for (int c = 0; c < DIM; ++c) f[c] = (double)feat[(base + row) * DIM + c];
      unsigned long long* keys = key_scratch + key_off[cloud] * n_anchor + (int64_t)a0 * n + row;
      for (int a = 0; a < na; ++a) {
        double d = 0.0;
#pragma unroll
        for (int c = 0; c < DIM; ++c) {
          const double diff = af[a][c] - f[c];
          d = fma(diff, diff, d);
        }
        keys[(int64_t)a * n] = (unsigned long long)__double_as_longlong(d);
      }
    }
  }
}

template <int DIM>
__global__ __launch_bounds__(256) void k_symcut_select(
    const float* __restrict__ feat, const float* __restrict__ xyz,
    const int64_t* __restrict__ off, const int32_t* __restrict__ anchors, int n_anchor,
    const int32_t* __restrict__ Ks, int n_nn, int n_init, int max_iter, uint64_t seed,
    unsigned long long* __restrict__ key_scratch, const int64_t* __restrict__ key_off,
    double* __restrict__ out_centers, int32_t* __restrict__ out_counts,
    double* __restrict__ out_min_cdist, double* __restrict__ out_max_err,
    double* __restrict__ pts_g, int32_t* __restrict__ nsel_g) {
  __shared__ int hist[256];
  __shared__ unsigned long long s_prefix;
  __shared__ int s_remaining;
  __shared__ int scan_a[256], scan_b[256];
  __shared__ int wsum[4];
  double (*pts)[3] = reinterpret_cast<double (*)[3]>(pts_g + (int64_t)blockIdx.x * SYM_MAX_NN * 3);

  const int blk = blockIdx.x;
  const int cloud = blk / n_anchor;
  const int tid = threadIdx.x;
  const int64_t base = off[cloud];
  const int n = (int)(off[cloud + 1] - base);
  const int K = Ks[cloud];
  const int n_sel = n < n_nn ? n : n_nn;
  double* oc = out_centers + (int64_t)blk * 12;
  if (n_sel < K || n == 0) {
    if (tid < 12) oc[tid] = 0.0;
    if (tid < 4) out_counts[(int64_t)blk * 4 + tid] = 0;
    if (tid == 0) {
      out_min_cdist[blk] = 0.0;
      out_max_err[blk] = INFINITY;
      nsel_g[blk] = 0;
    }
    return;
  }
  unsigned long long* keys = key_scratch + key_off[cloud] * n_anchor + (int64_t)(blk % n_anchor) * n;

  const int sel_q = ((n + 3) / 4 + 63) / 64 * 64;
  const bool in_regs = sel_q <= 64 * SYM_SEL_J;
  unsigned long long kr[SYM_SEL_J];
  if (in_regs) {
    const int r0 = (tid >> 6) * sel_q + (tid & 63);
#pragma unroll
    for (int j = 0; j < SYM_SEL_J; ++j) {
      const int row = r0 + 64 * j;
      kr[j] = (64 * j < sel_q && row < n) ? keys[row] : ~0ULL;
    }
  }
  if (tid == 0) {
    s_prefix = 0;
    s_remaining = n_sel;
  }
  __syncthreads();

  __shared__ int s_done;
  int shift_final = 0;
  if (tid == 0) s_done = 0;
  for (int pass = 0; pass < 8; ++pass) {
    const int shift = 56 - 8 * pass;
    hist[tid] = 0;
    __syncthreads();
    const unsigned long long prefix = s_prefix;
    int last = -1, run = 0;
    auto tally = [&](unsigned long long key) {
      if (pass == 0 || (key >> (shift + 8)) == prefix) {
        const int digit = (int)((key >> shift) & 255ULL);
        if (digit == last) {
          ++run;
        } else {
          if (run) atomicAdd(&hist[last], run);
          last = digit;
          run = 1;
        }
      }
    };
    if (in_regs) {
#pragma unroll
      for (int j = 0; j < SYM_SEL_J; ++j)
        if (kr[j] != ~0ULL) tally(kr[j]);
    } else {
      for (int i = tid; i < n; i += 256) tally(keys[i]);
    }
    if (run) atomicAdd(&hist[last], run);
    __syncthreads();
    {
      const int rem = s_remaining;
      int total;
      const int hv = hist[tid];
      const int excl = block_excl_scan256(hv, wsum, &total);
      const bool here = excl < rem && excl + hv >= rem;
      if (here) {
        s_remaining = rem - excl;
        s_prefix = (prefix << 8) | (unsigned long long)tid;
        if (excl + hv == rem) s_done = 1;
      }
      if (tid == 0 && total < rem) {
        s_remaining = rem - (total - hist[255]);
        s_prefix = (prefix << 8) | 255ULL;
      }
    }
    __syncthreads();
    shift_final = shift;
    if (s_done) break;
  }
  const unsigned long long kth = s_prefix;
  const int need_eq = s_remaining;

  {
    const int lane = tid & 63, wave = tid >> 6;
    const int q = ((n + 3) / 4 + 63) / 64 * 64;
    const int w0 = wave * q, w1 = min(n, w0 + q);
    const unsigned long long below = (1ULL << lane) - 1ULL;
    int n_lt = 0, n_eq = 0;
    if (in_regs) {
#pragma unroll
      for (int j = 0; j < SYM_SEL_J; ++j) {
        if (w0 + 64 * j >= w1) break;
        const bool in = kr[j] != ~0ULL;
        const unsigned long long key = kr[j] >> shift_final;
        n_lt += __popcll(__ballot(in && key < kth));
        n_eq += __popcll(__ballot(in && key == kth));
      }
    } else {
      for (int i = w0; i < w1; i += 64) {
        const bool in = i + lane < w1;
        const unsigned long long key = in ? keys[i + lane] >> shift_final : ~0ULL;
        n_lt += __popcll(__ballot(in && key < kth));
        n_eq += __popcll(__ballot(in && key == kth));
      }
    }
    if (lane == 0) {
      scan_a[wave] = n_lt;
      scan_b[wave] = n_eq;
    }
    __syncthreads();
    int eq_rank = 0, pos = 0;
    for (int w = 0; w < wave; ++w) {
      const int eq_taken = max(0, min(scan_b[w], need_eq - eq_rank));
      pos += scan_a[w] + eq_taken;
      eq_rank += scan_b[w];
    }
    auto emit = [&](int i, bool in, unsigned long long key) {
      const bool lt = in && key < kth, eq = in && key == kth;
      const unsigned long long eqm = __ballot(eq);
      const bool take = lt || (eq && eq_rank + __popcll(eqm & below) < need_eq);
      const unsigned long long tm = __ballot(take);
      const int my = pos + __popcll(tm & below);
      if (take && my < SYM_MAX_NN) {
        pts[my][0] = (double)xyz[(base + i + lane) * 3 + 0];
        pts[my][1] = (double)xyz[(base + i + lane) * 3 + 1];
        pts[my][2] = (double)xyz[(base + i + lane) * 3 + 2];
      }
      pos += __popcll(tm);
      eq_rank += __popcll(eqm);
    };
    if (in_regs) {
#pragma unroll
      for (int j = 0; j < SYM_SEL_J; ++j) {
        if (w0 + 64 * j >= w1) break;
        emit(w0 + 64 * j, kr[j] != ~0ULL, kr[j] >> shift_final);
      }
    } else {
      for (int i = w0; i < w1; i += 64) {
        const bool in = i + lane < w1;
        emit(i, in, in ? keys[i + lane] >> shift_final : ~0ULL);
      }
    }
  }
  if (tid == 0) nsel_g[blk] = n_sel;
}

__global__ __launch_bounds__(256) void k_symcut_kmeans(const int32_t* __restrict__ Ks, int n_anchor,
                                                       int n_blk, int n_init, int max_iter, int per,
                                                       const double* __restrict__ pts_g,
                                                       const int32_t* __restrict__ nsel_g,
                                                       double* __restrict__ km_centers_g,
                                                       double* __restrict__ km_inertia_g,
                                                       unsigned long long* __restrict__ km_labels_g) {
  extern __shared__ double km_lds[];
  double (*pts_s)[SYM_MAX_NN][3] = reinterpret_cast<double (*)[SYM_MAX_NN][3]>(km_lds);
  double* closest_s = km_lds + (size_t)per * SYM_MAX_NN * 3;
  const int tid = threadIdx.x;
  const int sub = tid / n_init;
  const int blk = blockIdx.x * per + sub;
  for (int i = tid; i < per * SYM_MAX_NN * 3; i += 256) {
    const int sb = i / (SYM_MAX_NN * 3);
    const int64_t gb = (int64_t)blockIdx.x * per + sb;
    (&pts_s[0][0][0])[i] = gb < n_blk ? pts_g[gb * SYM_MAX_NN * 3 + (i - sb * SYM_MAX_NN * 3)] : 0.0;
  }
  __syncthreads();
  if (sub >= per || blk >= n_blk) return;
  const int n_sel = nsel_g[blk];
  if (n_sel == 0) return;
  const int K = Ks[blk / n_anchor];
  double (*pts)[3] = pts_s[sub];
  double* closest = closest_s + tid;
  const int init_id = tid - sub * n_init;
  const int trials = K == 2 ? 2 : 3;
  const double* u = KM_DRAWS + init_id * (1 + (K - 1) * trials);
  KmState st;
#pragma unroll
  for (int c = 0; c < 4; ++c) st.cx[c] = st.cy[c] = st.cz[c] = 0.0;
  double tol;
  {
    double v[3];
#pragma unroll
    for (int a = 0; a < 3; ++a) {
      double m = 0.0, q = 0.0;
      for (int i = 0; i < n_sel; ++i) m += pts[i][a];
      m /= (double)n_sel;
      for (int i = 0; i < n_sel; ++i) q = fma(pts[i][a] - m, pts[i][a] - m, q);
      v[a] = q / (double)n_sel;
    }
    tol = ((v[0] + v[1]) + v[2]) / 3.0 * 1e-4;
  }
  {
    const double p_uniform = (double)(1.0f / (float)n_sel);
    double cdf_last = 0.0;
    for (int i = 0; i < n_sel; ++i) cdf_last += p_uniform;
    int c0 = n_sel - 1;
    double acc = 0.0;
    for (int i = 0; i < n_sel; ++i) {
      acc += p_uniform;
      if (acc / cdf_last > u[0]) {
        c0 = i;
        break;
      }
    }
    st.cx[0] = pts[c0][0];
    st.cy[0] = pts[c0][1];
    st.cz[0] = pts[c0][2];
  }
  double pot = 0.0;
  for (int i = 0; i < n_sel; ++i) {
    const double d = dist2_3(pts[i][0], pts[i][1], pts[i][2], st.cx[0], st.cy[0], st.cz[0]);
    closest[i * 256] = d;
    pot += d;
  }
#pragma unroll
  for (int c = 1; c < 4; ++c) {
    if (c < K) {
      int best_cand = -1;
      double best_pot = 0.0;
      for (int t = 0; t < trials; ++t) {
        const double rv = u[1 + (c - 1) * trials + t] * pot;
        int cand = n_sel - 1;
        double cum = 0.0;
        for (int i = 0; i < n_sel; ++i) {
          cum += closest[i * 256];
          if (cum >= rv) {
            cand = i;
            break;
          }
        }
        const double qx = pts[cand][0], qy = pts[cand][1], qz = pts[cand][2];
        double pc = 0.0;
        for (int i = 0; i < n_sel; ++i) {
          const double d = dist2_3(pts[i][0], pts[i][1], pts[i][2], qx, qy, qz);
          const double cl = closest[i * 256];
          pc += d < cl ? d : cl;
        }
        if (best_cand < 0 || pc < best_pot) {
          best_cand = cand;
          best_pot = pc;
        }
      }
      st.cx[c] = pts[best_cand][0];
      st.cy[c] = pts[best_cand][1];
      st.cz[c] = pts[best_cand][2];
      pot = best_pot;
      for (int i = 0; i < n_sel; ++i) {
        const double d = dist2_3(pts[i][0], pts[i][1], pts[i][2], st.cx[c], st.cy[c], st.cz[c]);
        if (d < closest[i * 256]) closest[i * 256] = d;
      }
    }
  }
  unsigned long long lab_lo = ~0ULL, lab_hi = ~0ULL;
  bool strict = false;
  for (int it = 0; it < max_iter; ++it) {
    double sx[4] = {0, 0, 0, 0}, sy[4] = {0, 0, 0, 0}, sz[4] = {0, 0, 0, 0};
    int cn[4] = {0, 0, 0, 0};
    unsigned long long nlo = 0, nhi = 0;
    for (int i = 0; i < n_sel; ++i) {
      double dm;
      const double px = pts[i][0], py = pts[i][1], pz = pts[i][2];
      const int b = nearest_center(st, K, px, py, pz, &dm);
      if (i < 32)
        nlo |= (unsigned long long)b << (2 * i);
      else
        nhi |= (unsigned long long)b << (2 * (i - 32));
#pragma unroll
      for (int c = 0; c < 4; ++c) {
        if (b == c) {
          sx[c] += px;
          sy[c] += py;
          sz[c] += pz;
          cn[c] += 1;
        }
      }
    }
    unsigned long long taken = 0;
#pragma unroll
    for (int c = 0; c < 4; ++c) {
      if (c < K && cn[c] == 0) {
        int far = -1;
        double fd = -1.0;
        for (int i = 0; i < n_sel; ++i) {
          double dm;
          nearest_center(st, K, pts[i][0], pts[i][1], pts[i][2], &dm);
          if ((taken >> i) & 1ULL) dm = -1.0;
          if (far < 0 || dm > fd) {
            far = i;
            fd = dm;
          }
        }
        taken |= 1ULL << far;
        const int old = (int)((far < 32 ? nlo >> (2 * far) : nhi >> (2 * (far - 32))) & 3ULL);
#pragma unroll
        for (int o = 0; o < 4; ++o) {
          if (o == old) {
            sx[o] -= pts[far][0];
            sy[o] -= pts[far][1];
            sz[o] -= pts[far][2];
            cn[o] -= 1;
          }
        }
        sx[c] = pts[far][0];
        sy[c] = pts[far][1];
        sz[c] = pts[far][2];
        cn[c] = 1;
      }
    }
    double shift = 0.0;
#pragma unroll
    for (int c = 0; c < 4; ++c) {
      if (c < K) {
        const double nx = cn[c] > 0 ? sx[c] / (double)cn[c] : st.cx[c];
        const double ny = cn[c] > 0 ? sy[c] / (double)cn[c] : st.cy[c];
        const double nz = cn[c] > 0 ? sz[c] / (double)cn[c] : st.cz[c];
        shift += dist2_3(nx, ny, nz, st.cx[c], st.cy[c], st.cz[c]);
        st.cx[c] = nx;
        st.cy[c] = ny;
        st.cz[c] = nz;
      }
    }
    const bool same = it > 0 && nlo == lab_lo && nhi == lab_hi;
    lab_lo = nlo;
    lab_hi = nhi;
    if (same) {
      strict = true;
      break;
    }
    if (shift <= tol) break;
  }
  double inertia = 0.0;
  if (!strict) {
    lab_lo = lab_hi = 0;
    for (int i = 0; i < n_sel; ++i) {
      double dm;
      const int b = nearest_center(st, K, pts[i][0], pts[i][1], pts[i][2], &dm);
      if (i < 32)
        lab_lo |= (unsigned long long)b << (2 * i);
      else
        lab_hi |= (unsigned long long)b << (2 * (i - 32));
      inertia += dm;
    }
  } else {
    for (int i = 0; i < n_sel; ++i) {
      const int b = (int)((i < 32 ? lab_lo >> (2 * i) : lab_hi >> (2 * (i - 32))) & 3ULL);
      double cx = st.cx[0], cy = st.cy[0], cz = st.cz[0];
#pragma unroll
      for (int c = 1; c < 4; ++c)
        if (b == c) {
          cx = st.cx[c];
          cy = st.cy[c];
          cz = st.cz[c];
        }
      inertia += dist2_3(pts[i][0], pts[i][1], pts[i][2], cx, cy, cz);
    }
  }
  const int64_t slot = (int64_t)blk * n_init + init_id;
#pragma unroll
  for (int c = 0; c < 4; ++c) {
    km_centers_g[slot * 12 + 3 * c + 0] = st.cx[c];
    km_centers_g[slot * 12 + 3 * c + 1] = st.cy[c];
    km_centers_g[slot * 12 + 3 * c + 2] = st.cz[c];
  }
  km_inertia_g[slot] = inertia;
  km_labels_g[slot * 2 + 0] = lab_lo;
  km_labels_g[slot * 2 + 1] = lab_hi;
}

template <int DIM>
__global__ __launch_bounds__(256) void k_symcut_finish(
    const float* __restrict__ xyz, const int64_t* __restrict__ off, int n_anchor,
    const int32_t* __restrict__ Ks, int n_init, const double* __restrict__ pts_g,
    const int32_t* __restrict__ nsel_g, const double* __restrict__ km_centers_g,
    const double* __restrict__ km_inertia_g, const unsigned long long* __restrict__ km_labels_g,
    double* __restrict__ out_centers, int32_t* __restrict__ out_counts, double* __restrict__ out_min_cdist,
    double* __restrict__ out_max_err) {
  __shared__ double sel_centers[12];
  __shared__ int counts[4];
  const int blk = blockIdx.x;
  const int cloud = blk / n_anchor;
  const int tid = threadIdx.x;
  const int n_sel = nsel_g[blk];
  if (n_sel == 0) return;
  const int64_t base = off[cloud];
  const int n = (int)(off[cloud + 1] - base);
  const int K = Ks[cloud];
  double* oc = out_centers + (int64_t)blk * 12;
  const double (*pts)[3] = reinterpret_cast<const double (*)[3]>(pts_g + (int64_t)blk * SYM_MAX_NN * 3);
  const double (*km_centers)[12] = reinterpret_cast<const double (*)[12]>(km_centers_g + (int64_t)blk * n_init * 12);
  const double* km_inertia = km_inertia_g + (int64_t)blk * n_init;
  __shared__ double s_dist[SYM_MAX_NN];
  __shared__ int s_b[SYM_MAX_NN];
  KmState st;
  if (tid < 64) {
    const unsigned long long* km_lab = km_labels_g + (int64_t)blk * n_init * 2;
    const bool has_r = tid < n_init;
    const double my_in = has_r ? km_inertia[tid] : 0.0;
    const unsigned long long my_lo = has_r ? km_lab[2 * tid] : 0ULL, my_hi = has_r ? km_lab[2 * tid + 1] : 0ULL;
    const bool act = tid < n_sel;
    const int sh = 2 * (tid & 31);
    int best = 0;
    for (int r = 1; r < n_init; ++r) {
      if (!(__shfl(my_in, r) < __shfl(my_in, best))) continue;
      const unsigned long long r_lo = __shfl(my_lo, r), r_hi = __shfl(my_hi, r);
      const unsigned long long b_lo = __shfl(my_lo, best), b_hi = __shfl(my_hi, best);
      const unsigned long long rw = tid < 32 ? r_lo : r_hi;
      const unsigned long long bw = tid < 32 ? b_lo : b_hi;
      const int la = (int)((rw >> sh) & 3ULL), lb = (int)((bw >> sh) & 3ULL);
      bool same_clu = true;
#pragma unroll
      for (int c = 0; c < 4; ++c) {
        const unsigned long long mk = __ballot(act && la == c);
        const int lb_first = __shfl(lb, mk ? __ffsll((long long)mk) - 1 : 0);
        if (__ballot(act && la == c && lb != lb_first)) same_clu = false;
      }
      if (!same_clu) best = r;
    }
    if (tid < 12) {
      const double v = tid < 3 * K ? km_centers[best][tid] : 0.0;
      sel_centers[tid] = v;
      oc[tid] = v;
    }
#pragma unroll
    for (int c = 0; c < 4; ++c) {
      st.cx[c] = km_centers[best][3 * c + 0];
      st.cy[c] = km_centers[best][3 * c + 1];
      st.cz[c] = km_centers[best][3 * c + 2];
    }
    if (act) {
      double dm;
      s_b[tid] = nearest_center(st, K, pts[tid][0], pts[tid][1], pts[tid][2], &dm);
      s_dist[tid] = sqrt(dm);
    }
  }
  __syncthreads();
  {
    if (tid == 0) {
      double min_cd = INFINITY;
#pragma unroll
      for (int c = 0; c < 4; ++c)
#pragma unroll
        for (int d = c + 1; d < 4; ++d)
          if (d < K) {
            const double dd = sqrt(dist2_3(st.cx[c], st.cy[c], st.cz[c], st.cx[d], st.cy[d], st.cz[d]));
            if (dd < min_cd) min_cd = dd;
          }
      double esum[4] = {0, 0, 0, 0};
      int ecnt[4] = {0, 0, 0, 0};
      for (int i = 0; i < n_sel; ++i) {
        const int bsel = s_b[i];
        const double dist = s_dist[i];
#pragma unroll
        for (int c = 0; c < 4; ++c)
          if (bsel == c) {
            esum[c] += dist;
            ecnt[c] += 1;
          }
      }
      double max_err = 0.0;
#pragma unroll
      for (int c = 0; c < 4; ++c) {
        if (c < K) {
          const double e = ecnt[c] > 0 ? esum[c] / (double)ecnt[c] : INFINITY;
          if (e > max_err) max_err = e;
        }
      }
      out_min_cdist[blk] = min_cd;
      out_max_err[blk] = max_err;
    }
  }
  if (tid < 4) counts[tid] = 0;
  __syncthreads();
  {
    KmState st;
#pragma unroll
    for (int c = 0; c < 4; ++c) {
      st.cx[c] = sel_centers[3 * c + 0];
      st.cy[c] = sel_centers[3 * c + 1];
      st.cz[c] = sel_centers[3 * c + 2];
    }
    int local[4] = {0, 0, 0, 0};
    for (int i0 = tid; i0 < n; i0 += 256 * 4) {
      float p[4][3];
#pragma unroll
      for (int u = 0; u < 4; ++u) {
        const int i = i0 + 256 * u;
        const int64_t g = base + (i < n ? i : i0);
#pragma unroll
        for (int a = 0; a < 3; ++a) p[u][a] = xyz[g * 3 + a];
      }
#pragma unroll
      for (int u = 0; u < 4; ++u) {
        double dm;
        const int b = nearest_center(st, K, (double)p[u][0], (double)p[u][1], (double)p[u][2], &dm);
        const bool in = i0 + 256 * u < n;
#pragma unroll
        for (int c = 0; c < 4; ++c) local[c] += (in && b == c);
      }
    }
#pragma unroll
    for (int c = 0; c < 4; ++c)
      if (local[c]) atomicAdd(&counts[c], local[c]);
  }
  __syncthreads();
  if (tid < 4) out_counts[(int64_t)blk * 4 + tid] = counts[tid];
}

__global__ void k_symcut_labels(const float* __restrict__ xyz, const int64_t* __restrict__ off,
                                const int32_t* __restrict__ Ks,
                                const double* __restrict__ centers, int32_t* __restrict__ labels) {
  const int cloud = blockIdx.y;
  const int64_t base = off[cloud];
  const int n = (int)(off[cloud + 1] - base);
  const int K = Ks[cloud];
  KmState st;
#pragma unroll
  for (int c = 0; c < 4; ++c) {
    st.cx[c] = centers[(int64_t)cloud * 12 + 3 * c + 0];
    st.cy[c] = centers[(int64_t)cloud * 12 + 3 * c + 1];
    st.cz[c] = centers[(int64_t)cloud * 12 + 3 * c + 2];
  }
  for (int i = blockIdx.x * blockDim.x + threadIdx.x; i < n; i += gridDim.x * blockDim.x) {
    double dm;
    labels[base + i] = nearest_center(st, K, (double)xyz[(base + i) * 3 + 0],
                                      (double)xyz[(base + i) * 3 + 1],
                                      (double)xyz[(base + i) * 3 + 2], &dm);
  }
}

}

using namespace cs;

extern "C" {

int cs_symcut_fit(const float* d_feat, int dim, const float* d_xyz, const int64_t* h_off,
                  int n_cloud, const int32_t* d_anchor, int n_anchor, const int32_t* h_K,
                  int n_nn, int n_init, int max_iter, double* d_centers,
                  int32_t* d_counts, double* d_min_center_dist, double* d_max_error,
                  void* stream) {
  const uint64_t seed = 0;
  CS_REQUIRE(d_feat && d_xyz && h_off && d_anchor && h_K && d_centers && d_counts &&
                 d_min_center_dist && d_max_error,
             CS_ERR_INVALID, "cs_symcut_fit: NULL argument");
  CS_REQUIRE(dim == 16 || dim == 32, CS_ERR_UNSUPPORTED, "cs_symcut_fit: dim %d unsupported", dim);
  CS_REQUIRE(n_nn >= 4 && n_nn <= SYM_MAX_NN, CS_ERR_UNSUPPORTED,
             "cs_symcut_fit: n_nn %d not in [4, %d]", n_nn, SYM_MAX_NN);
  CS_REQUIRE(n_init >= 1 && n_init <= SYM_MAX_INIT, CS_ERR_UNSUPPORTED,
             "cs_symcut_fit: n_init %d not in [1, %d]", n_init, SYM_MAX_INIT);
  CS_REQUIRE(n_anchor >= 1 && max_iter >= 1, CS_ERR_INVALID, "cs_symcut_fit: bad counts");
  if (n_cloud <= 0) return CS_OK;
  hipStream_t s = (hipStream_t)stream;
  pool_use_stream(s);
  std::vector<int64_t> off(h_off, h_off + n_cloud + 1), key_off(n_cloud + 1, 0);
  std::vector<int32_t> Ks(h_K, h_K + n_cloud);
  for (int c = 0; c < n_cloud; ++c) {
    CS_REQUIRE(off[c + 1] >= off[c] && off[c + 1] - off[c] < (1LL << 31), CS_ERR_INVALID,
               "cs_symcut_fit: bad segment %d", c);
    CS_REQUIRE(Ks[c] == 2 || Ks[c] == 4, CS_ERR_UNSUPPORTED,
               "cs_symcut_fit: K must be 2 or 4 (utils/symmetry.py:246-257)");
    key_off[c + 1] = key_off[c] + (off[c + 1] - off[c]);
  }
  PoolBuf<int64_t> d_off(n_cloud + 1), d_koff(n_cloud + 1);
  PoolBuf<int32_t> d_K(n_cloud);
  PoolBuf<unsigned long long> keys((size_t)key_off[n_cloud] * n_anchor + 1);
  const size_t n_ca = (size_t)n_cloud * n_anchor;
  PoolBuf<double> pts_g(n_ca * SYM_MAX_NN * 3), kmc_g(n_ca * n_init * 12), kmi_g(n_ca * n_init);
  PoolBuf<int32_t> nsel_g(n_ca);
  PoolBuf<unsigned long long> kml_g(n_ca * n_init * 2);
  CS_REQUIRE(d_off.p && d_koff.p && d_K.p && keys.p && pts_g.p && kmc_g.p && kmi_g.p && nsel_g.p && kml_g.p, CS_ERR_HIP,
             "cs_symcut_fit: scratch allocation failed");
  CS_HIP_CHECK(hipMemcpyAsync(d_off.p, off.data(), sizeof(int64_t) * (n_cloud + 1),
                              hipMemcpyHostToDevice, s));
  CS_HIP_CHECK(hipMemcpyAsync(d_koff.p, key_off.data(), sizeof(int64_t) * (n_cloud + 1),
                              hipMemcpyHostToDevice, s));
  CS_HIP_CHECK(hipMemcpyAsync(d_K.p, Ks.data(), sizeof(int32_t) * n_cloud, hipMemcpyHostToDevice, s));
  {
    ProfScope prof("symcut", s);
    const int n_blk = n_cloud * n_anchor;
    dim3 grid((unsigned)n_blk);
    int64_t n_max = 0;
    for (int c = 0; c < n_cloud; ++c) n_max = std::max<int64_t>(n_max, off[c + 1] - off[c]);
    const dim3 kgrid((unsigned)std::max<int64_t>(ceil_div(n_max, 256), 1), (unsigned)n_cloud);
    if (dim == 16)
      hipLaunchKernelGGL((k_symcut_keys<16>), kgrid, dim3(256), 0, s, d_feat, d_off.p, d_anchor, n_anchor,
                         keys.p, d_koff.p);
    else
      hipLaunchKernelGGL((k_symcut_keys<32>), kgrid, dim3(256), 0, s, d_feat, d_off.p, d_anchor, n_anchor,
                         keys.p, d_koff.p);
    if (dim == 16)
      hipLaunchKernelGGL((k_symcut_select<16>), grid, dim3(256), 0, s, d_feat, d_xyz, d_off.p,
                         d_anchor, n_anchor, d_K.p, n_nn, n_init, max_iter, seed, keys.p,
                         d_koff.p, d_centers, d_counts, d_min_center_dist, d_max_error, pts_g.p, nsel_g.p);
    else
      hipLaunchKernelGGL((k_symcut_select<32>), grid, dim3(256), 0, s, d_feat, d_xyz, d_off.p,
                         d_anchor, n_anchor, d_K.p, n_nn, n_init, max_iter, seed, keys.p,
                         d_koff.p, d_centers, d_counts, d_min_center_dist, d_max_error, pts_g.p, nsel_g.p);
    const size_t closest_bytes = sizeof(double) * 256 * (size_t)n_nn;
    const size_t lds_budget = 156 * 1024;
    int per = 256 / n_init;
    const int per_fit = (int)((lds_budget - closest_bytes) / (sizeof(double) * SYM_MAX_NN * 3));
    if (per > per_fit) per = per_fit;
    if (per < 1) per = 1;
    const size_t km_lds_bytes = closest_bytes + sizeof(double) * SYM_MAX_NN * 3 * (size_t)per;
    CS_HIP_CHECK(hipFuncSetAttribute((const void*)k_symcut_kmeans, hipFuncAttributeMaxDynamicSharedMemorySize, (int)lds_budget));
    hipLaunchKernelGGL(k_symcut_kmeans, dim3((unsigned)((n_blk + per - 1) / per)), dim3(256), km_lds_bytes, s, d_K.p, n_anchor,
                       n_blk, n_init, max_iter, per, pts_g.p, nsel_g.p, kmc_g.p, kmi_g.p, kml_g.p);
    hipLaunchKernelGGL((k_symcut_finish<16>), grid, dim3(256), 0, s, d_xyz, d_off.p, n_anchor, d_K.p,
                       n_init, pts_g.p, nsel_g.p, kmc_g.p, kmi_g.p, kml_g.p, d_centers, d_counts,
                       d_min_center_dist, d_max_error);
    CS_LAUNCH_CHECK();
  }
  return CS_OK;
}

int cs_symcut_labels(const float* d_xyz, const int64_t* h_off, int n_cloud, const int32_t* h_K,
                     const double* d_sel_centers, int32_t* d_labels, void* stream) {
  CS_REQUIRE(d_xyz && h_off && h_K && d_sel_centers && d_labels, CS_ERR_INVALID,
             "cs_symcut_labels: NULL argument");
  if (n_cloud <= 0) return CS_OK;
  hipStream_t s = (hipStream_t)stream;
  pool_use_stream(s);
  PoolBuf<int64_t> d_off(n_cloud + 1);
  PoolBuf<int32_t> d_K(n_cloud);
  CS_REQUIRE(d_off.p && d_K.p, CS_ERR_HIP, "cs_symcut_labels: scratch allocation failed");
  int64_t nmax = 0;
  for (int c = 0; c < n_cloud; ++c) {
    CS_REQUIRE(h_K[c] == 2 || h_K[c] == 4, CS_ERR_UNSUPPORTED, "cs_symcut_labels: K must be 2 or 4");
    if (h_off[c + 1] - h_off[c] > nmax) nmax = h_off[c + 1] - h_off[c];
  }
  CS_HIP_CHECK(hipMemcpyAsync(d_off.p, h_off, sizeof(int64_t) * (n_cloud + 1),
                              hipMemcpyHostToDevice, s));
  CS_HIP_CHECK(hipMemcpyAsync(d_K.p, h_K, sizeof(int32_t) * n_cloud, hipMemcpyHostToDevice, s));
  if (nmax > 0) {
    dim3 grid((unsigned)ceil_div(nmax, 256), (unsigned)n_cloud);
    hipLaunchKernelGGL(k_symcut_labels, grid, dim3(256), 0, s, d_xyz, d_off.p, d_K.p,
                       d_sel_centers, d_labels);
    CS_LAUNCH_CHECK();
  }
  return CS_OK;
}

}
```

### corsair_amd/csrc/sympose.hip

```cpp
#include "common.h"

namespace cs {

__global__ __launch_bounds__(256) void k_partition_by_label(const int32_t* __restrict__ label,
                                                            const int64_t* __restrict__ off,
                                                            int64_t* __restrict__ order) {
  __shared__ int hist[8];
  __shared__ int base[8];
  __shared__ int wcnt[4][8];
  const int c = blockIdx.x;
  const int64_t r0 = off[c], r1 = off[c + 1];
  const int tid = threadIdx.x, lane = tid & 63, wave = tid >> 6;
  if (tid < 8) hist[tid] = 0;
  __syncthreads();
  for (int64_t r = r0 + tid; r < r1; r += 256) {
    int l = label[r];
    l = l < 0 ? 0 : (l > 7 ? 7 : l);
    atomicAdd(&hist[l], 1);
  }
  __syncthreads();
  if (tid == 0) {
    int run = 0;
    for (int l = 0; l < 8; ++l) {
      base[l] = run;
      run += hist[l];
    }
  }
  __syncthreads();
  for (int64_t rb = r0; rb < r1; rb += 256) {
    const int64_t r = rb + tid;
    int l = -1;
    if (r < r1) {
      l = label[r];
      l = l < 0 ? 0 : (l > 7 ? 7 : l);
    }
    int my_rank = 0;
#pragma unroll
    for (int q = 0; q < 8; ++q) {
      const unsigned long long m = __ballot(l == q);
      if (l == q) my_rank = __popcll(m & ((1ULL << lane) - 1ULL));
      if (lane == 0) wcnt[wave][q] = __popcll(m);
    }
    __syncthreads();
    if (l >= 0) {
      int pos = base[l] + my_rank;
      for (int w = 0; w < wave; ++w) pos += wcnt[w][l];
      order[r0 + pos] = r;
    }
    __syncthreads();
    if (tid < 8) base[tid] += wcnt[0][tid] + wcnt[1][tid] + wcnt[2][tid] + wcnt[3][tid];
    __syncthreads();
  }
}

struct CorrDesc {
  int64_t q_first, n_first, t_first, len, out_first;
};
__global__ __launch_bounds__(256) void k_corr_assemble(const float* __restrict__ xyz0, const float* __restrict__ xyz1,
                                                       const int64_t* __restrict__ rows, const int32_t* __restrict__ nn,
                                                       int k, const CorrDesc* __restrict__ desc,
                                                       float* __restrict__ src, float* __restrict__ tgt) {
  const CorrDesc d = desc[blockIdx.y];
  for (int64_t e = (int64_t)blockIdx.x * 256 + threadIdx.x; e < d.len * k; e += (int64_t)gridDim.x * 256) {
    const int64_t i = e / k;
    const int nb = (int)(e - i * k);
    const int64_t q = rows ? rows[d.q_first + i] : d.q_first + i;
    const int32_t nbv = nn[(d.n_first + i) * k + nb];
    const int64_t t = d.t_first + (nbv < 0 ? 0 : nbv);
    const int64_t o = (d.out_first * k + e) * 3;
    src[o] = xyz0[q * 3];
    src[o + 1] = xyz0[q * 3 + 1];
    src[o + 2] = xyz0[q * 3 + 2];
    tgt[o] = xyz1[t * 3];
    tgt[o + 1] = xyz1[t * 3 + 1];
    tgt[o + 2] = xyz1[t * 3 + 2];
  }
}

__global__ __launch_bounds__(256) void k_cfg_bad(const int32_t* __restrict__ nn, int k, const int64_t* __restrict__ first,
                                                 int32_t* __restrict__ bad) {
  const int j = blockIdx.y;
  const int64_t a = first[j] * k, b = first[j + 1] * k;
  int any = 0;
  for (int64_t e = a + (int64_t)blockIdx.x * 256 + threadIdx.x; e < b; e += (int64_t)gridDim.x * 256) any |= nn[e] < 0;
  if (__any(any) && (threadIdx.x & 63) == 0) atomicOr(&bad[j], 1);
}
__global__ void k_zero_i32(int32_t* p, int n) {
  const int i = blockIdx.x * blockDim.x + threadIdx.x;
  if (i < n) p[i] = 0;
}

__global__ __launch_bounds__(256) void k_rows_nonfinite(const float* __restrict__ x, int dim,
                                                        const int64_t* __restrict__ first, int32_t* __restrict__ bad) {
  const int j = blockIdx.y;
  const int64_t a = first[j] * dim, b = first[j + 1] * dim;
  int any = 0;
  for (int64_t e = a + (int64_t)blockIdx.x * 256 + threadIdx.x; e < b; e += (int64_t)gridDim.x * 256)
    any |= !(fabsf(x[e]) < INFINITY);
  if (__any(any) && (threadIdx.x & 63) == 0) atomicOr(&bad[j], 1);
}

}

using namespace cs;

extern "C" {

int cs_partition_by_label(const int32_t* d_label, const int64_t* d_off, int n_cloud, int64_t* d_order, void* stream) {
  CS_REQUIRE(n_cloud >= 0 && (n_cloud == 0 || (d_label && d_off && d_order)), CS_ERR_INVALID,
             "cs_partition_by_label: bad argument");
  if (n_cloud == 0) return CS_OK;
  hipLaunchKernelGGL(k_partition_by_label, dim3((unsigned)n_cloud), dim3(256), 0, (hipStream_t)stream, d_label, d_off,
                     d_order);
  CS_LAUNCH_CHECK();
  return CS_OK;
}

int cs_corr_assemble(const float* d_xyz0, const float* d_xyz1, const int64_t* d_rows, const int32_t* d_nn, int k,
                     const int64_t* d_desc, int n_cfg, int64_t max_len, float* d_src, float* d_tgt, void* stream) {
  CS_REQUIRE(k >= 1 && n_cfg >= 0 && max_len >= 0, CS_ERR_INVALID, "cs_corr_assemble: bad argument");
  if (n_cfg == 0 || max_len == 0) return CS_OK;
  CS_REQUIRE(d_xyz0 && d_xyz1 && d_nn && d_desc && d_src && d_tgt, CS_ERR_INVALID, "cs_corr_assemble: NULL tensor");
  unsigned gx = (unsigned)ceil_div(max_len * k, 256);
  if (gx > 64) gx = 64;
  hipLaunchKernelGGL(k_corr_assemble, dim3(gx, (unsigned)n_cfg), dim3(256), 0, (hipStream_t)stream, d_xyz0, d_xyz1, d_rows,
                     d_nn, k, reinterpret_cast<const CorrDesc*>(d_desc), d_src, d_tgt);
  CS_LAUNCH_CHECK();
  return CS_OK;
}

int cs_cfg_bad(const int32_t* d_nn, int k, const int64_t* d_first, int n_cfg, int32_t* d_bad, void* stream) {
  CS_REQUIRE(k >= 1 && n_cfg >= 0, CS_ERR_INVALID, "cs_cfg_bad: bad argument");
  if (n_cfg == 0) return CS_OK;
  CS_REQUIRE(d_nn && d_first && d_bad, CS_ERR_INVALID, "cs_cfg_bad: NULL tensor");
  hipStream_t s = (hipStream_t)stream;
  hipLaunchKernelGGL(k_zero_i32, dim3((unsigned)ceil_div(n_cfg, 256)), dim3(256), 0, s, d_bad, n_cfg);
  hipLaunchKernelGGL(k_cfg_bad, dim3(16, (unsigned)n_cfg), dim3(256), 0, s, d_nn, k, d_first, d_bad);
  CS_LAUNCH_CHECK();
  return CS_OK;
}

int cs_rows_nonfinite(const float* d_x, int dim, const int64_t* d_first, int n_seg, int32_t* d_bad, void* stream) {
  CS_REQUIRE(dim >= 1 && n_seg >= 0, CS_ERR_INVALID, "cs_rows_nonfinite: bad argument");
  if (n_seg == 0) return CS_OK;
  CS_REQUIRE(d_x && d_first && d_bad, CS_ERR_INVALID, "cs_rows_nonfinite: NULL tensor");
  hipStream_t s = (hipStream_t)stream;
  hipLaunchKernelGGL(k_zero_i32, dim3((unsigned)ceil_div(n_seg, 256)), dim3(256), 0, s, d_bad, n_seg);
  hipLaunchKernelGGL(k_rows_nonfinite, dim3(16, (unsigned)n_seg), dim3(256), 0, s, d_x, dim, d_first, d_bad);
  CS_LAUNCH_CHECK();
  return CS_OK;
}

}
```

### corsair_amd/registration.py

```python
from __future__ import annotations

import inspect
import os
from dataclasses import dataclass

import numpy as np
import torch

from . import _helper
from . import backend as B
from ._lib import to_host

ANCHOR_KEY = 0x5A11C0DE



@dataclass
class SymPoseResult:
    T_best: torch.Tensor
    cd_best: torch.Tensor
    T_ransac: torch.Tensor
    cd_ransac: torch.Tensor
    ok: np.ndarray
    iters: torch.Tensor
    n_problems: int
    T_all: torch.Tensor = None
    cd_all: torch.Tensor = None
    inliers: torch.Tensor = None
    prob_pair: list = None
    prob_cfg: list = None
    best: np.ndarray = None
    T_icp: torch.Tensor = None
    cd_icp: torch.Tensor = None
    icp_fitness: torch.Tensor = None
    icp_rmse: torch.Tensor = None
    icp_iters: torch.Tensor = None
    icp_wfitness: torch.Tensor = None
    icp_scale: torch.Tensor = None
    icp_mrmse: torch.Tensor = None

    def hypotheses(self, p):
        return [j for j, q in enumerate(self.prob_pair) if q == p]


def draw_anchors(n, n_anchor, counter):
    if n < n_anchor:
        return None
    gen = np.random.Generator(np.random.Philox(key=ANCHOR_KEY, counter=counter))
    return gen.choice(n, n_anchor, replace=False).astype(np.int32)


GATE_REFERENCE = (0.15, 0.15)
GATE_ANY = (0.0, float("inf"))


def gate_and_order(centers, counts, min_cdist, max_err, n, K, gate=GATE_REFERENCE):
    ratios = counts[:, :K].astype(np.float64) / float(n)
    std = np.sqrt(np.var(ratios, axis=1))
    valid = (min_cdist > gate[0]) & (gate[1] > max_err) & (std < 100)
    if not valid.any():
        return None
    a = int(np.argmin(np.where(valid, std, np.inf)))
    c = centers[a]
    out = np.zeros((4, 3), np.float64)
    if K == 2:
        out[:2] = c[:2]
        return out
    d = np.linalg.norm(c[0][None, :] - c[1:4], axis=1)
    rank = np.argsort(d, kind="stable")
    out[:] = c[[0, rank[0] + 1, rank[2] + 1, rank[1] + 1]]
    return out


def gate_and_order_batch(centers, counts, min_cdist, max_err, n, Ks, cand, gate=GATE_REFERENCE):
    P = centers.shape[0]
    sel = np.zeros((P, 4, 3), np.float64)
    ok = np.zeros(P, dtype=bool)
    n = np.asarray(n, dtype=np.float64)
    Ks = np.asarray(Ks)
    cand = np.asarray(cand, dtype=np.int64)
    for K in (2, 4):
        idx = cand[Ks[cand] == K]
        if idx.size == 0:
            continue
        ratios = counts[idx][:, :, :K].astype(np.float64) / n[idx][:, None, None]
        std = np.sqrt(np.var(ratios, axis=2))
        valid = (min_cdist[idx] > gate[0]) & (gate[1] > max_err[idx]) & (std < 100)
        has = valid.any(axis=1)
        a = np.argmin(np.where(valid, std, np.inf), axis=1)
        c = centers[idx, a]
        out = np.zeros((idx.size, 4, 3), np.float64)
        if K == 2:
            out[:, :2] = c[:, :2]
        else:
            d = np.linalg.norm(c[:, 0:1] - c[:, 1:4], axis=2)
            rank = np.argsort(d, axis=1, kind="stable")
            order = np.stack([np.zeros(idx.size, np.int64), rank[:, 0] + 1, rank[:, 2] + 1, rank[:, 1] + 1], 1)
            out = np.take_along_axis(c, order[:, :, None], axis=1)
        sel[idx[has]] = out[has]
        ok[idx[has]] = True
    return sel, ok


def part_configs(K, pos_sym):
    cfgs = [[(i + s) % K for i in range(K)] for s in range(K)]
    if pos_sym >= 2:
        mirror = [0, 3, 2, 1]
        cfgs += [[mirror[(i + s) % 4] for i in range(4)] for s in range(4)]
    return cfgs


def _refuse_nonfinite(bad_query, bad_cad):
    for side, bad, said in (("CAD", bad_cad, "data must be finite"), ("query", bad_query, "'x' must be finite")):
        hit = np.flatnonzero(np.asarray(bad))
        if hit.size:
            raise ValueError("sym_pose_batch: the %s descriptors of pair %d hold a NaN or an infinite value (the "
                             "reference's KD-tree refuses them: %s)" % (side, int(hit[0]), said))


def _sym_pose_batch(estimator, baseF, xyz0, off0, posF, xyz1, off1, pos_syms, k_nn=5, max_corr=0.20, seed=0,
                    anchor_ids=None, n_anchor=100, max_iter=100000, confidence=0.999,
                    use_symmetry=True, force_gate=False, query_anchors=None, icp_max_iter=0, icp_max_dist=None,
                    icp_estimation="point", icp_normal_k=16, normals1=None, icp_normal_radius=None, icp_with_scaling=False,
                    icp_scale_bounds=None, icp_kernel="l2", icp_kernel_scale=None):
    registration, fgr_mu_floor, fgr_iterations, fgr_tuple_test, normals0, gicp_epsilon = estimator
    if icp_estimation == "gicp" and (icp_with_scaling or icp_kernel != "l2"):
        raise ValueError("sym_pose_batch: icp_estimation 'gicp' with icp_with_scaling or a robust icp_kernel is out of scope")
    if icp_estimation != "gicp" and normals0 is not None:
        raise ValueError("sym_pose_batch: normals0 is used by icp_estimation = 'gicp' only")
    if icp_with_scaling and icp_kernel != "l2":
        raise ValueError("sym_pose_batch: icp_with_scaling with a robust icp_kernel (%r) is out of scope" % (icp_kernel,))
    if icp_kernel not in B.ICP_KERNELS:
        raise ValueError("sym_pose_batch: icp_kernel must be one of %s, got %r" % (sorted(B.ICP_KERNELS), icp_kernel))
    if icp_kernel != "l2" and icp_estimation != "plane":
        raise ValueError("sym_pose_batch: icp_kernel %r needs icp_estimation = 'plane'" % (icp_kernel,))
    if icp_max_iter > 0 and icp_kernel != "l2" and not (icp_kernel_scale is not None and icp_kernel_scale > 0):
        raise ValueError("sym_pose_batch: icp_kernel %r needs a positive icp_kernel_scale" % (icp_kernel,))
    if icp_estimation not in ("point", "plane", "gicp"):
        raise ValueError("sym_pose_batch: icp_estimation must be 'point', 'plane' or 'gicp', got %r" % (icp_estimation,))
    if icp_normal_radius is not None and not (0 < icp_normal_radius < float("inf")):
        raise ValueError("sym_pose_batch: icp_normal_radius must be positive and finite (None = k-NN), got %r"
                         % (icp_normal_radius,))
    if icp_max_iter > 0 and not (icp_max_dist is not None and icp_max_dist > 0):
        raise ValueError("sym_pose_batch: icp_max_iter > 0 needs a positive icp_max_dist")
    dev = baseF.device
    P = len(off0) - 1
    off0 = [int(v) for v in off0]
    off1 = [int(v) for v in off1]
    n0 = [off0[p + 1] - off0[p] for p in range(P)]
    n1 = [off1[p + 1] - off1[p] for p in range(P)]
    k = k_nn

    short = [p for p in range(P) if n0[p] > 0 and n1[p] < k]
    if short:
        raise IndexError("sym_pose_batch: CAD cloud of pair %d has %d voxels, fewer than k_nn = %d (the reference's "
                         "find_kcorr fails on such a pair too)" % (short[0], n1[short[0]], k))
    nn = B.knn_feat(baseF, off0, posF, off1, k)
    nonfinite = None
    if P:
        pair_rows = torch.from_numpy(np.asarray(off0 + off1, dtype=np.int64)).to(dev, non_blocking=True)
        nonfinite = (B.cfg_bad(nn, pair_rows[:P + 1], P), B.rows_nonfinite(posF, pair_rows[P + 1:], P))
    desc_v = np.asarray([[off0[p], off0[p], off1[p], n0[p], off0[p]] for p in range(P)], dtype=np.int64).reshape(P, 5)
    v_src, v_tgt = B.corr_assemble(xyz0, xyz1, None, nn, desc_v, off0[-1], max(n0) if P else 0)
    corr_src = [v_src]
    corr_tgt = [v_tgt]
    prob_len = [n0[p] * k for p in range(P)]
    prob_pair = list(range(P))
    prob_cfg = [None] * P
    ok = np.zeros(P, dtype=bool)
    vanilla = None
    if registration == "ransac" and use_symmetry and dev.type == "cuda" and \
            os.environ.get("CORSAIR_SPLIT_RANSAC", "1") != "0":
        v_offs = np.concatenate([[0], np.cumsum(prob_len)]).tolist()
        for t in (v_src, v_tgt):
            t.record_stream(_helper.stream(dev))
        vanilla = _helper.submit(dev, lambda: B.ransac_batch(v_src, v_tgt, v_offs, max_corr, 10, max_iter,
                                                            confidence, seed))

    try:
        if use_symmetry:
            Ks = [4 if int(pos_syms[p]) >= 2 else 2 for p in range(P)]
            if anchor_ids is None:
                anchor_ids = [(2 * p, 2 * p + 1) for p in range(P)]
            anc0 = query_anchors if query_anchors is not None else \
                [draw_anchors(n0[p], n_anchor, anchor_ids[p][0]) for p in range(P)]
            anc1 = [draw_anchors(n1[p], n_anchor, anchor_ids[p][1]) for p in range(P)]
            cand = [p for p in range(P) if anc0[p] is not None and anc1[p] is not None]
            sel0 = np.zeros((P, 4, 3))
            sel1 = np.zeros((P, 4, 3))
            if cand:
                def anchors_of(anc):
                    return np.stack([anc[p] if anc[p] is not None else np.zeros(n_anchor, np.int32) for p in range(P)])

                a_all = torch.from_numpy(np.concatenate([anchors_of(anc0), anchors_of(anc1)])).to(dev)
                off_all = off0 + [off0[-1] + o for o in off1[1:]]
                c, cnt, mcd, mer = B.symcut_fit(torch.cat([baseF, posF]), torch.cat([xyz0, xyz1]), off_all, a_all,
                                                Ks + Ks, 50, 10, 300)
                if nonfinite is not None:
                    c, cnt, mcd, mer, bad_q, bad_c = to_host(c, cnt, mcd, mer, *nonfinite)
                    nonfinite = None
                    _refuse_nonfinite(bad_q, bad_c)
                else:
                    c, cnt, mcd, mer = to_host(c, cnt, mcd, mer)
                c0, cnt0, mcd0, mer0 = c[:P], cnt[:P], mcd[:P], mer[:P]
                c1, cnt1, mcd1, mer1 = c[P:], cnt[P:], mcd[P:], mer[P:]
                gate = GATE_ANY if force_gate else GATE_REFERENCE
                g0, ok0 = gate_and_order_batch(c0, cnt0, mcd0, mer0, n0, Ks, cand, gate)
                g1, ok1 = gate_and_order_batch(c1, cnt1, mcd1, mer1, n1, Ks, cand, gate)
                ok = ok0 & ok1
                sel0[ok], sel1[ok] = g0[ok], g1[ok]
            good = [p for p in range(P) if ok[p]]
            if good:
                lab0 = B.symcut_labels(xyz0, off0, Ks, torch.from_numpy(sel0).to(dev))
                lab1 = B.symcut_labels(xyz1, off1, Ks, torch.from_numpy(sel1).to(dev))
                qseg, tseg, perms, cfg_pair = [], [], [], []
                for p in good:
                    for cfg in part_configs(Ks[p], int(pos_syms[p])):
                        qseg.append(p)
                        tseg.append(p)
                        perms.append(cfg + [-3] * (8 - len(cfg)))
                        cfg_pair.append(p)
                lens = np.asarray([n0[p] for p in cfg_pair], dtype=np.int64)
                row_start = np.concatenate([[0], np.cumsum(lens)])
                n_cfg = len(cfg_pair)
                host_blk = np.concatenate([np.asarray(off0, np.int64), row_start,
                                           np.asarray(perms, np.int32).reshape(-1).view(np.int64)])
                dev_blk = torch.from_numpy(host_blk).to(dev)
                off0_t = dev_blk[:P + 1]
                first_t = dev_blk[P + 1:P + 2 + n_cfg]
                perm_t = dev_blk[P + 2 + n_cfg:].view(torch.int32).view(n_cfg, 8)
                sorted_rows = B.partition_by_label(lab0, off0_t, P)
                nn_cfg = B.knn_feat(baseF[sorted_rows], off0, posF, off1, k, qseg=qseg, tseg=tseg,
                                    qlabel=lab0[sorted_rows].contiguous(), tlabel=lab1, perm=perm_t)
                bad = to_host(B.cfg_bad(nn_cfg, first_t, n_cfg))[0] > 0
                keep = [j for j in range(n_cfg) if not bad[j]]
                if keep:
                    out_first = np.concatenate([[0], np.cumsum(lens[keep])])
                    desc = np.asarray([[off0[cfg_pair[j]], row_start[j], off1[cfg_pair[j]], lens[j], out_first[i]]
                                       for i, j in enumerate(keep)], dtype=np.int64)
                    s_src, s_tgt = B.corr_assemble(xyz0, xyz1, sorted_rows, nn_cfg, desc, int(out_first[-1]),
                                                   int(lens[keep].max()))
                    corr_src.append(s_src)
                    corr_tgt.append(s_tgt)
                    for j in keep:
                        prob_len.append(n0[cfg_pair[j]] * k)
                        prob_pair.append(cfg_pair[j])
                        prob_cfg.append([c for c in perms[j] if c >= 0])
    except BaseException:
        if vanilla is not None:
            try:
                vanilla.result()
            except Exception:
                pass
        raise

    if vanilla is None:
        src = corr_src[0] if len(corr_src) == 1 else torch.cat(corr_src)
        tgt = corr_tgt[0] if len(corr_tgt) == 1 else torch.cat(corr_tgt)
        offs = np.concatenate([[0], np.cumsum(prob_len)]).tolist()
        if registration == "fgr":
            r = B.fgr_batch(src, tgt, offs, max_corr, mu_floor=fgr_mu_floor, iteration_number=fgr_iterations,
                            tuple_test=fgr_tuple_test, seed=seed)
            T, inl, rmse, iters = r.T, r.inliers, r.rmse, r.iters
        else:
            T, inl, rmse, iters = B.ransac_batch(src, tgt, offs, max_corr, 10, max_iter, confidence, seed)
    else:
        parts = []
        if len(corr_src) > 1:
            offs = np.concatenate([[0], np.cumsum(prob_len[P:])]).tolist()
            parts = [B.ransac_batch(corr_src[1], corr_tgt[1], offs, max_corr, 10, max_iter, confidence, seed)]
        first = vanilla.result()
        cur = torch.cuda.current_stream(dev)
        for t in first:
            t.record_stream(cur)
        T, inl, rmse, iters = (torch.cat([a] + [q[i] for q in parts]) for i, a in enumerate(first))

    cd = B.chamfer_1dir(xyz0, off0, xyz1, off1, prob_pair, prob_pair, T)

    if nonfinite is not None:
        cd_h, bad_q, bad_c = to_host(cd, *nonfinite)
        _refuse_nonfinite(bad_q, bad_c)
    else:
        cd_h = to_host(cd)[0]
    pair_h = np.asarray(prob_pair)
    best = np.arange(P)
    for j in range(P, len(pair_h)):
        p = pair_h[j]
        if cd_h[best[p]] > cd_h[j]:
            best[p] = j
    best_t = torch.from_numpy(best).to(dev)
    res = SymPoseResult(T_best=T[best_t], cd_best=cd[best_t], T_ransac=T[:P], cd_ransac=cd[:P],
                        ok=ok, iters=iters, n_problems=len(prob_pair), T_all=T, cd_all=cd, inliers=inl,
                        prob_pair=prob_pair, prob_cfg=prob_cfg, best=best)

    if icp_max_iter > 0:
        pairs = list(range(P))
        nrm = None
        if icp_estimation in ("plane", "gicp"):
            nrm = normals1 if normals1 is not None else B.estimate_normals(xyz1, off1, icp_normal_k, icp_normal_radius)
        scaling = {}
        if icp_with_scaling:
            scaling = {"with_scaling": True}
            if icp_scale_bounds is not None:
                scaling["scale_bounds"] = icp_scale_bounds
        if icp_estimation == "gicp":
            snrm = normals0 if normals0 is not None else B.estimate_normals(xyz0, off0, icp_normal_k, icp_normal_radius)
            scaling = {"estimation": "gicp", "src_normals": snrm, "gicp_epsilon": gicp_epsilon}
        r = B.icp_batch(xyz0, off0, xyz1, off1, pairs, pairs, res.T_best, icp_max_dist, icp_max_iter, tgt_normals=nrm,
                        kernel=icp_kernel, kernel_scale=icp_kernel_scale, **scaling)
        res.T_icp, res.icp_fitness, res.icp_rmse, res.icp_iters = r.T32, r.fitness, r.rmse, r.iters
        res.icp_wfitness = r.wfitness
        res.icp_scale = r.scale
        res.icp_mrmse = r.mrmse
        res.cd_icp = B.chamfer_1dir(xyz0, off0, xyz1, off1, pairs, pairs, r.T32)
    return res


def sym_pose_batch(*args, registration="ransac", fgr_mu_floor=0.025, fgr_iterations=64, fgr_tuple_test=True, **kwargs):
    if registration not in ("ransac", "fgr"):
        raise ValueError("sym_pose_batch: registration must be 'ransac' or 'fgr', got %r" % (registration,))
    normals0, gicp_epsilon = kwargs.pop("normals0", None), kwargs.pop("gicp_epsilon", 1e-3)
    return _sym_pose_batch((registration, fgr_mu_floor, fgr_iterations, fgr_tuple_test, normals0, gicp_epsilon), *args,
                           **kwargs)


sym_pose_batch.__signature__ = inspect.Signature(list(inspect.signature(_sym_pose_batch).parameters.values())[1:])
```

### include/corsair_hip.h

```cpp
#ifndef CORSAIR_HIP_H
#define CORSAIR_HIP_H

#include <stdint.h>

#ifdef __cplusplus
extern "C" {
#endif

#define CS_OK 0
#define CS_ERR_INVALID (-1)
#define CS_ERR_HIP (-2)
#define CS_ERR_RANGE (-3)
#define CS_ERR_DUPLICATE (-4)
#define CS_ERR_UNSUPPORTED (-5)
#define CS_ERR_INTERNAL (-6)

typedef struct cs_coordmap cs_coordmap;
typedef struct cs_kernelmap cs_kernelmap;

const char* cs_last_error(void);
int cs_version(void);
int cs_device_count(void);

int cs_coordmap_create(const int32_t* d_coords, int64_t n, int tensor_stride, void* stream,
                       cs_coordmap** out);
int cs_coordmap_stride(const cs_coordmap* in, int stride, void* stream, cs_coordmap** out);
int cs_coordmap_pyramid(const int32_t* d_coords, int64_t n, int tensor_stride, int n_levels, int n_batch, void* stream,
                        cs_coordmap** out);
int64_t cs_coordmap_size(const cs_coordmap* m);
int cs_coordmap_tensor_stride(const cs_coordmap* m);
const int32_t* cs_coordmap_coords(const cs_coordmap* m);
void cs_coordmap_free(cs_coordmap* m);

int cs_kernelmap_build(const cs_coordmap* in, const cs_coordmap* out, int kernel_size,
                       int transposed, void* stream, cs_kernelmap** km);
int cs_kernelmap_build_many(int n, const cs_coordmap* const* in, const cs_coordmap* const* out, const int* kernel_size,
                            const int* transposed, void* stream, cs_kernelmap** km);
int64_t cs_kernelmap_num_pairs(const cs_kernelmap* km);
int64_t cs_kernelmap_rows(const cs_kernelmap* km);
const int32_t* cs_kernelmap_table(const cs_kernelmap* km);
int64_t cs_kernelmap_export(const cs_kernelmap* km, int32_t* d_k, int32_t* d_in, int32_t* d_out,
                            int64_t capacity, void* stream);
void cs_kernelmap_free(cs_kernelmap* km);

int cs_conv_fwd(const cs_kernelmap* km, int64_t n_in, int64_t n_out, const float* d_in, int ld_in,
                int cin, const float* d_w, int cout, const float* d_scale, const float* d_shift,
                const float* d_residual, int ld_res, int relu, float* d_out, int ld_out,
                void* stream);

int cs_conv_wgrad(const cs_kernelmap* km, int64_t n_in, int64_t n_out, const float* d_in, int ld_in, int cin,
                  const float* d_gout, int ld_gout, int cout, float* d_dw, void* stream);

int cs_affine_act(int64_t n, int c, const float* d_in, int ld_in, const float* d_scale,
                  const float* d_shift, const float* d_residual, int ld_res, int relu,
                  float* d_out, int ld_out, void* stream);

int cs_row_l2_normalize(int64_t n, int c, const float* d_in, int ld_in, float eps, float* d_out,
                        int ld_out, void* stream);

int cs_segmented_max(int64_t n, int c, const float* d_in, int ld_in, const int32_t* d_batch,
                     int batch_ld, int n_batch, float* d_out, void* stream);

int cs_instance_norm(int64_t n, int c, const float* d_in, int ld_in, const int32_t* d_seg, int n_batch,
                     const float* d_weight, const float* d_bias, float eps, float* d_out, int ld_out,
                     void* stream);

int cs_voxelize(const float* d_xyz, const int64_t* h_offsets, int n_seg, double voxel_size,
                int64_t* d_keep_idx, int32_t* d_grid, int64_t* h_out_offsets, void* stream);
int cs_voxelize_f64(const double* d_xyz, const int64_t* h_offsets, int n_seg, double voxel_size,
                    int64_t* d_keep_idx, int32_t* d_grid, int64_t* h_out_offsets, void* stream);

int cs_l2_topk(const float* d_q, int64_t nq, const float* d_x, int64_t nx, int d, int k,
               int64_t* d_idx, double* d_dist, void* stream);
int cs_l2_topk_sq(const float* d_q, int64_t nq, const float* d_x, int64_t nx, int d, int k, int64_t* d_idx,
                  double* d_dist2, void* stream);
void cs_l2_topk_stats(uint64_t out[2], int reset);
typedef struct cs_topk_catalog cs_topk_catalog;
int cs_topk_catalog_create(const float* d_x, int64_t nx, int d, void* stream, cs_topk_catalog** out);
int cs_l2_topk_catalog(const float* d_q, int64_t nq, const cs_topk_catalog* catalog, int k, int64_t* d_idx,
                       double* d_dist, int squared, void* stream);
void cs_topk_catalog_free(cs_topk_catalog* catalog);

int cs_knn_feat(const float* d_qf, const int64_t* h_qoff, const float* d_tf,
                const int64_t* h_toff, const int32_t* h_qseg, const int32_t* h_tseg, int n_prob,
                int dim, int k, const int32_t* d_qlabel, const int32_t* d_tlabel,
                const int32_t* d_perm, int32_t* d_idx, double* d_dist, void* stream);

void cs_knn_shortlist_stats(uint64_t out[2], int reset);

void cs_chamfer_f16_stats(uint64_t out[2], int reset);
int cs_chamfer_1dir(const float* d_src, const int64_t* h_soff, const float* d_tgt,
                    const int64_t* h_toff, const int32_t* h_src_seg, const int32_t* h_tgt_seg,
                    int n_prob, const float* d_T, double* d_out, void* stream);

int cs_hausdorff_1dir(const float* d_src, const int64_t* h_soff, const float* d_tgt,
                      const int64_t* h_toff, const int32_t* h_src_seg, const int32_t* h_tgt_seg,
                      int n_prob, const float* d_T, double* d_out, void* stream);

int cs_chamfer_2dir(const float* d_src, const int64_t* h_soff, const float* d_tgt, const int64_t* h_toff,
                    const int32_t* h_src_seg, const int32_t* h_tgt_seg, int n_prob, const float* d_T,
                    double* d_out , void* stream);

int cs_ransac_batch(const float* d_src, const float* d_tgt, const int64_t* h_off, int n_prob,
                    double max_corr, int ransac_n, int max_iter, double confidence, uint64_t seed,
                    float* d_T, int32_t* d_inliers, double* d_rmse, int32_t* d_iters,
                    void* stream);
void cs_ransac_prefilter_stats(uint64_t out[5], int reset);

int cs_symcut_fit(const float* d_feat, int dim, const float* d_xyz, const int64_t* h_off,
                  int n_cloud, const int32_t* d_anchor, int n_anchor, const int32_t* h_K,
                  int n_nn, int n_init, int max_iter, double* d_centers,
                  int32_t* d_counts, double* d_min_center_dist, double* d_max_error,
                  void* stream);
int cs_symcut_labels(const float* d_xyz, const int64_t* h_off, int n_cloud, const int32_t* h_K,
                     const double* d_sel_centers, int32_t* d_labels, void* stream);

int cs_partition_by_label(const int32_t* d_label, const int64_t* d_off, int n_cloud, int64_t* d_order, void* stream);
int cs_cfg_bad(const int32_t* d_nn, int k, const int64_t* d_first, int n_cfg, int32_t* d_bad, void* stream);
int cs_rows_nonfinite(const float* d_x, int dim, const int64_t* d_first, int n_seg, int32_t* d_bad, void* stream);
int cs_corr_assemble(const float* d_xyz0, const float* d_xyz1, const int64_t* d_rows, const int32_t* d_nn, int k,
                     const int64_t* d_desc, int n_cfg, int64_t max_len, float* d_src, float* d_tgt, void* stream);

typedef struct cs_radius_plan cs_radius_plan;
int cs_radius_pairs(const double* d_src, const int64_t* h_soff, const double* d_tgt, const int64_t* h_toff,
                    const int32_t* h_src_seg, const int32_t* h_tgt_seg, int n_prob, double radius, int k_max,
                    int64_t* d_row_ptr, void* stream, cs_radius_plan** plan);
int cs_radius_pairs_fill(const cs_radius_plan* plan, const int64_t* d_row_ptr, int32_t* d_tgt_idx, void* stream);
void cs_radius_plan_free(cs_radius_plan* plan);

int cs_sample_pairs(const float* d_xyz, const int64_t* h_off, const int32_t* h_base_seg, const int32_t* h_pos_seg,
                    const int32_t* h_neg_seg, const int32_t* h_slot, int n_prob, const int64_t* h_row_base,
                    const int64_t* d_row_ptr, const int32_t* d_tgt_idx, int lists, uint64_t seed, int round,
                    double radius, int sample, int32_t* d_pip, int32_t* d_pin, int32_t* d_nin, int32_t* d_counts,
                    void* stream);

int cs_transform_f64(const float* d_xyz, const int64_t* h_off, const int32_t* h_seg, int n_prob, const double* d_T,
                     double* d_out, void* stream);

#define CS_PAIR_LOSS_MAX_TERMS 8
#define CS_PAIR_PULL 0
#define CS_PAIR_PUSH 1
int cs_pair_loss_fwd(int n_mat, const float* const* d_mat, const int64_t* h_rows, const int32_t* h_ld, int C,
                     int n_term, const int32_t* h_a, const int32_t* h_b, const int32_t* h_kind, const float* h_margin,
                     const double* h_weight, const int32_t* const* d_pairs, const int64_t* h_npairs,
                     double* d_term_loss, float* d_total, void* stream);
int cs_pair_loss_bwd(int n_mat, const float* const* d_mat, const int64_t* h_rows, const int32_t* h_ld, int C,
                     int n_term, const int32_t* h_a, const int32_t* h_b, const int32_t* h_kind, const float* h_margin,
                     const double* h_weight, const int32_t* const* d_pairs, const int64_t* h_npairs,
                     const float* d_grad_up, float* const* d_grad, const int32_t* h_ld_grad, void* stream);

int cs_hardest_negatives(const float* d_qf, int ld_q, const float* d_qxyz, const int64_t* h_qoff, const float* d_tf,
                         int ld_t, const float* d_txyz, const int64_t* h_toff, const int32_t* h_qseg,
                         const int32_t* h_tseg, int n_prob, int C, const int32_t* d_anchor, int64_t A, double radius,
                         int32_t* d_idx, double* d_dist, void* stream);
void cs_hardest_stats(uint64_t out[2], int reset);

int cs_icp_batch(const float* d_src, const int64_t* h_soff, const float* d_tgt, const int64_t* h_toff,
                 const int32_t* h_src_seg, const int32_t* h_tgt_seg, int n_prob, const float* d_T0, double max_dist,
                 int max_iter, double relative_fitness, double relative_rmse, double* d_T, float* d_T32,
                 double* d_fitness, double* d_rmse, int32_t* d_iters, int32_t* d_ncorr, int32_t* d_corr, void* stream);
void cs_icp_stats(uint64_t out[2], int reset);

int cs_icp_plane_batch(const float* d_src, const int64_t* h_soff, const float* d_tgt, const float* d_tgt_normal,
                       const int64_t* h_toff, const int32_t* h_src_seg, const int32_t* h_tgt_seg, int n_prob,
                       const float* d_T0, double max_dist, int max_iter, double relative_fitness, double relative_rmse,
                       double* d_T, float* d_T32, double* d_fitness, double* d_rmse, int32_t* d_iters, int32_t* d_ncorr,
                       int32_t* d_corr, void* stream);

#define CS_ICP_KERNEL_L2 0
#define CS_ICP_KERNEL_HUBER 1
#define CS_ICP_KERNEL_CAUCHY 2
#define CS_ICP_KERNEL_TUKEY 3
int cs_icp_plane_robust_batch(const float* d_src, const int64_t* h_soff, const float* d_tgt, const float* d_tgt_normal,
                              const int64_t* h_toff, const int32_t* h_src_seg, const int32_t* h_tgt_seg, int n_prob,
                              const float* d_T0, double max_dist, int max_iter, double relative_fitness,
                              double relative_rmse, int kernel, double kernel_scale, double* d_T, float* d_T32,
                              double* d_fitness, double* d_rmse, double* d_wfitness, int32_t* d_iters, int32_t* d_ncorr,
                              int32_t* d_corr, void* stream);

int cs_icp_scale_batch(const float* d_src, const int64_t* h_soff, const float* d_tgt, const float* d_tgt_normal,
                       const int64_t* h_toff, const int32_t* h_src_seg, const int32_t* h_tgt_seg, int n_prob,
                       const float* d_T0, double max_dist, int max_iter, double relative_fitness, double relative_rmse,
                       double scale_min, double scale_max, double* d_T, float* d_T32, double* d_fitness, double* d_rmse,
                       double* d_scale, int32_t* d_iters, int32_t* d_ncorr, int32_t* d_corr, void* stream);

int cs_icp_gicp_batch(const float* d_src, const float* d_src_normal, const int64_t* h_soff, const float* d_tgt,
                      const float* d_tgt_normal, const int64_t* h_toff, const int32_t* h_src_seg, const int32_t* h_tgt_seg,
                      int n_prob, const float* d_T0, double max_dist, int max_iter, double relative_fitness,
                      double relative_rmse, double epsilon, double* d_T, float* d_T32, double* d_fitness, double* d_rmse,
                      double* d_mrmse, int32_t* d_iters, int32_t* d_ncorr, int32_t* d_corr, void* stream);

int cs_estimate_normals(const float* d_xyz, const int64_t* h_off, int n_seg, int k, float* d_normal, void* stream);

int cs_estimate_normals_hybrid(const float* d_xyz, const int64_t* h_off, int n_seg, double radius, int max_nn,
                               float* d_normal, void* stream);
void cs_normals_stats(uint64_t out[2], int reset);

int cs_fgr_batch(const float* d_src, const float* d_tgt, const int64_t* h_off, int n_prob, double max_corr,
                 double mu_floor, double division_factor, int iteration_number, int tuple_test, double tuple_scale,
                 int max_tuple, uint64_t seed, float* d_T, double* d_T64, int32_t* d_inliers, double* d_rmse,
                 int32_t* d_iters, int32_t* d_ntuple, void* stream);

void cs_prof_enable(int on);
void cs_prof_reset(void);
int cs_prof_get(const char* name, double* total_ms, int64_t* launches);
int cs_prof_get_units(const char* name, double* units);

void cs_pool_trim(void);
void cs_pool_stats(uint64_t out[3]);

#ifdef __cplusplus
}
#endif
#endif
```

Measured before the change: 2120.

## Keep symmetry-pose gating, dead masking and best selection on device

Moves the symmetry-cut gate, the dead-configuration flags and the per-pair best-pose selection into new GPU kernels. RANSAC gains a masked entry that marks dead problems as done up front, so vanilla and symmetric problems can run in one batch with shared correspondence buffers. This is meant to remove host round-trips and syncs between the symcut, kNN, RANSAC and Chamfer stages, and to skip RANSAC work on dead configurations. The cost is more kernels and per-call host metadata packing, plus the risk that the device gate does not match the earlier host logic exactly.

```diff
diff --git a/corsair_amd/_lib.py b/corsair_amd/_lib.py
--- a/corsair_amd/_lib.py
+++ b/corsair_amd/_lib.py
@@ -58,6 +58,8 @@
                                       POINTER(c_int32), c_int, vp, vp, vp]),
         "cs_ransac_batch": (c_int, [vp, vp, POINTER(c_int64), c_int, c_double, c_int, c_int, c_double,
                                     c_uint64, vp, vp, vp, vp, vp]),
+        "cs_ransac_batch_masked": (c_int, [vp, vp, POINTER(c_int64), c_int, c_double, c_int, c_int, c_double,
+                                           c_uint64, vp, vp, vp, vp, vp, vp]),
         "cs_ransac_prefilter_stats": (None, [POINTER(c_uint64), c_int]),
         "cs_knn_shortlist_stats": (None, [POINTER(c_uint64), c_int]),
         "cs_chamfer_f16_stats": (None, [POINTER(c_uint64), c_int]),
@@ -68,6 +70,10 @@
         "cs_symcut_fit": (c_int, [vp, c_int, vp, POINTER(c_int64), c_int, vp, c_int,
                                   POINTER(c_int32), c_int, c_int, c_int, vp, vp, vp, vp, vp]),
         "cs_symcut_labels": (c_int, [vp, POINTER(c_int64), c_int, POINTER(c_int32), vp, vp, vp]),
+        "cs_symcut_gate": (c_int, [vp, vp, vp, vp, c_int, c_int, POINTER(c_int64), POINTER(c_int32), POINTER(c_int32),
+                                   c_double, c_double, vp, vp, vp, vp]),
+        "cs_cfg_dead": (c_int, [vp, c_int, vp, c_int, vp, vp, c_int, vp, vp]),
+        "cs_sympose_select": (c_int, [vp, vp, vp, vp, c_int, vp, vp, vp, vp]),
         "cs_partition_by_label": (c_int, [vp, vp, c_int, vp, vp]),
         "cs_cfg_bad": (c_int, [vp, c_int, vp, c_int, vp, vp]),
         "cs_rows_nonfinite": (c_int, [vp, c_int, vp, c_int, vp, vp]),
diff --git a/corsair_amd/backend.py b/corsair_amd/backend.py
--- a/corsair_amd/backend.py
+++ b/corsair_amd/backend.py
@@ -592,7 +592,7 @@
     return int(out[0]), int(out[1])
 
 
-def ransac_batch(src, tgt, offsets, max_corr, ransac_n=10, max_iter=100000, confidence=0.999, seed=0):
+def ransac_batch(src, tgt, offsets, max_corr, ransac_n=10, max_iter=100000, confidence=0.999, seed=0, dead=None):
     src = _dev(src, torch.float32, "source correspondences").contiguous()
     tgt = _dev(tgt, torch.float32, "target correspondences").contiguous()
     n_prob = len(offsets) - 1
@@ -601,9 +601,17 @@
     inl = torch.empty(n_prob, dtype=torch.int32, device=dev)
     rmse = torch.empty(n_prob, dtype=torch.float64, device=dev)
     iters = torch.empty(n_prob, dtype=torch.int32, device=dev)
-    check(_lib.load().cs_ransac_batch(ptr(src), ptr(tgt), i64_array(offsets), n_prob, float(max_corr),
-                                      ransac_n, max_iter, float(confidence), int(seed), ptr(T),
-                                      ptr(inl), ptr(rmse), ptr(iters), stream_ptr()))
+    if dead is None:
+        check(_lib.load().cs_ransac_batch(ptr(src), ptr(tgt), i64_array(offsets), n_prob, float(max_corr),
+                                          ransac_n, max_iter, float(confidence), int(seed), ptr(T),
+                                          ptr(inl), ptr(rmse), ptr(iters), stream_ptr()))
+        return T, inl, rmse, iters
+    dead = _dev(dead, torch.int32, "dead flags").contiguous()
+    if dead.shape != (n_prob,):
+        raise ValueError("ransac_batch: dead must hold one flag per problem")
+    check(_lib.load().cs_ransac_batch_masked(ptr(src), ptr(tgt), i64_array(offsets), n_prob, float(max_corr),
+                                             ransac_n, max_iter, float(confidence), int(seed), ptr(dead), ptr(T),
+                                             ptr(inl), ptr(rmse), ptr(iters), stream_ptr()))
     return T, inl, rmse, iters
 
 
@@ -653,6 +661,32 @@
     return bad
 
 
+def cfg_dead(nn, d_first, n_cfg, d_cfg_pair, pair_ok, n_lead):
+    nn = _dev(nn, torch.int32, "neighbour lists").contiguous()
+    d_cfg_pair = _dev(d_cfg_pair, torch.int32, "configuration pairs")
+    pair_ok = _dev(pair_ok, torch.int32, "pair flags")
+    if d_cfg_pair.shape != (n_cfg,) or not d_cfg_pair.is_contiguous():
+        raise ValueError("cfg_dead: d_cfg_pair must be a contiguous int32 [n_cfg]")
+    dead = torch.empty(n_lead + n_cfg, dtype=torch.int32, device=nn.device)
+    check(_lib.load().cs_cfg_dead(ptr(nn), nn.shape[1], ptr(d_first), n_cfg, ptr(d_cfg_pair), ptr(pair_ok), n_lead,
+                                  ptr(dead), stream_ptr()))
+    return dead
+
+
+def sympose_select(cd, dead, T, d_cfg_first, n_pair):
+    cd = _dev(cd, torch.float64, "Chamfer distances").contiguous()
+    dead = _dev(dead, torch.int32, "dead flags").contiguous()
+    T = _dev(T, torch.float32, "transforms").contiguous()
+    if dead.shape != cd.shape or T.shape[0] != cd.shape[0]:
+        raise ValueError("sympose_select: cd, dead and T must hold one entry per problem")
+    best = torch.empty(n_pair, dtype=torch.int64, device=cd.device)
+    T_best = torch.empty((n_pair, 4, 4), dtype=torch.float32, device=cd.device)
+    cd_best = torch.empty(n_pair, dtype=torch.float64, device=cd.device)
+    check(_lib.load().cs_sympose_select(ptr(cd), ptr(dead), ptr(T), ptr(d_cfg_first), n_pair, ptr(best), ptr(T_best),
+                                        ptr(cd_best), stream_ptr()))
+    return best, T_best, cd_best
+
+
 def rows_nonfinite(x, d_first, n_seg):
     x = _dev(x, torch.float32, "rows").contiguous()
     bad = torch.empty(n_seg, dtype=torch.int32, device=x.device)
@@ -660,14 +694,20 @@
     return bad
 
 
-def corr_assemble(xyz0, xyz1, rows, nn, desc, total, max_len):
+def corr_assemble(xyz0, xyz1, rows, nn, desc, total, max_len, out=None):
     xyz0 = _dev(xyz0, torch.float32, "query xyz").contiguous()
     xyz1 = _dev(xyz1, torch.float32, "CAD xyz").contiguous()
     nn = _dev(nn, torch.int32, "neighbour lists").contiguous()
     k = nn.shape[1]
     dev = xyz0.device
-    src = torch.empty((total * k, 3), dtype=torch.float32, device=dev)
-    tgt = torch.empty((total * k, 3), dtype=torch.float32, device=dev)
+    if out is None:
+        src = torch.empty((total * k, 3), dtype=torch.float32, device=dev)
+        tgt = torch.empty((total * k, 3), dtype=torch.float32, device=dev)
+    else:
+        src, tgt = out
+        for t in out:
+            if t.dtype != torch.float32 or not t.is_contiguous() or t.dim() != 2 or t.shape[1] != 3 or t.shape[0] < total * k:
+                raise ValueError("corr_assemble: out must be two contiguous f32 [>= total * k, 3] tensors")
     d_desc = torch.from_numpy(np.ascontiguousarray(desc, dtype=np.int64)).to(dev, non_blocking=True)
     check(_lib.load().cs_corr_assemble(ptr(xyz0), ptr(xyz1), ptr(rows) if rows is not None else None, ptr(nn), k,
                                        ptr(d_desc), len(desc), int(max_len), ptr(src), ptr(tgt), stream_ptr()))
@@ -688,6 +728,25 @@
                                     ptr(anchors), na, i32_array(Ks), n_nn, n_init, max_iter,
                                     ptr(centers), ptr(counts), ptr(mcd), ptr(mer), stream_ptr()))
     return centers, counts, mcd, mer
+
+
+def symcut_gate(centers, counts, mcd, mer, n, Ks, cand, gate):
+    centers = _dev(centers, torch.float64, "centres").contiguous()
+    counts = _dev(counts, torch.int32, "counts").contiguous()
+    mcd = _dev(mcd, torch.float64, "centre distances").contiguous()
+    mer = _dev(mer, torch.float64, "errors").contiguous()
+    nc, na = counts.shape[0], counts.shape[1]
+    if nc % 2 or not (len(n) == len(Ks) == len(cand) == nc) or centers.shape != (nc, na, 4, 3) or mcd.shape != (nc, na) \
+            or mer.shape != (nc, na):
+        raise ValueError("symcut_gate: shapes do not describe 2 P clouds")
+    dev = centers.device
+    sel = torch.empty((nc, 4, 3), dtype=torch.float64, device=dev)
+    ok = torch.empty(nc, dtype=torch.int32, device=dev)
+    pair_ok = torch.empty(nc // 2, dtype=torch.int32, device=dev)
+    check(_lib.load().cs_symcut_gate(ptr(centers), ptr(counts), ptr(mcd), ptr(mer), nc // 2, na, i64_array(n),
+                                     i32_array(Ks), i32_array(cand), float(gate[0]), float(gate[1]), ptr(sel), ptr(ok),
+                                     ptr(pair_ok), stream_ptr()))
+    return sel, ok, pair_ok
 
 
 def symcut_labels(xyz, offsets, Ks, sel_centers):
diff --git a/corsair_amd/csrc/ransac.hip b/corsair_amd/csrc/ransac.hip
--- a/corsair_amd/csrc/ransac.hip
+++ b/corsair_amd/csrc/ransac.hip
@@ -192,6 +192,11 @@
   if (iters) iters[p] = pr.iters;
 }
 
+__global__ void k_ransac_mask(RansacProb* probs, int n_prob, const int32_t* __restrict__ dead) {
+  const int p = blockIdx.x * blockDim.x + threadIdx.x;
+  if (p < n_prob && dead[p]) probs[p].done = 1;
+}
+
 }
 
 using namespace cs;
@@ -340,6 +345,7 @@
   int max_surv_prev = 1 << 30;
   unsigned long long tot_surv = 0, tot_eval = 0;
   size_t trace_n = 0;
+  const int32_t* d_dead = nullptr;
 
   int init(const int64_t* h_off, int n, double max_corr, int rn, int iters, double confidence, uint64_t sd, hipStream_t st);
   int setup(const float* d_src, const float* d_tgt);
@@ -411,6 +417,10 @@
   memset(sc.h_state, 0, sc.st_bytes);
   memcpy(sc.h_state, hp.data(), sc.st_probs);
   CS_HIP_CHECK(hipMemcpyAsync(sc.state.p, sc.h_state, sc.st_bytes, hipMemcpyHostToDevice, s));
+  if (d_dead) {
+    hipLaunchKernelGGL(k_ransac_mask, dim3((unsigned)ceil_div(n_prob, 64)), dim3(64), 0, s, sc.probs(), n_prob, d_dead);
+    CS_LAUNCH_CHECK();
+  }
   if (pf_alloc) {
     CS_HIP_CHECK(hipMemcpyAsync(sc.off16.p, h_off16.data(), sizeof(int64_t) * (n_prob + 1),
                                 hipMemcpyHostToDevice, s));
@@ -612,6 +622,11 @@
         if (h_surv[p] > max_surv_prev) max_surv_prev = h_surv[p];
       }
   }
+  if (d_dead && cur.it0 == 0) {
+    const RansacProb* now = reinterpret_cast<const RansacProb*>(sc.h_state);
+    for (int p = 0; p < n_prob; ++p)
+      if (!hp[p].done && now[p].done && now[p].iters == 0) tot_eval -= (unsigned long long)std::min(hp[p].est_k, cur.b);
+  }
   memcpy(hp.data(), sc.h_state, sc.st_probs);
   return sc.h_nactive(cur.par) != 0;
 }
@@ -661,6 +676,14 @@
                     double max_corr, int ransac_n, int max_iter, double confidence, uint64_t seed,
                     float* d_T, int32_t* d_inliers, double* d_rmse, int32_t* d_iters,
                     void* stream) {
+  return cs_ransac_batch_masked(d_src, d_tgt, h_off, n_prob, max_corr, ransac_n, max_iter, confidence, seed, nullptr, d_T,
+                                d_inliers, d_rmse, d_iters, stream);
+}
+
+int cs_ransac_batch_masked(const float* d_src, const float* d_tgt, const int64_t* h_off, int n_prob,
+                           double max_corr, int ransac_n, int max_iter, double confidence, uint64_t seed,
+                           const int32_t* d_dead, float* d_T, int32_t* d_inliers, double* d_rmse, int32_t* d_iters,
+                           void* stream) {
   CS_REQUIRE(h_off && d_T, CS_ERR_INVALID, "cs_ransac_batch: NULL argument");
   CS_REQUIRE(ransac_n >= 3 && ransac_n <= 64, CS_ERR_INVALID,
              "cs_ransac_batch: ransac_n %d not in [3, 64]", ransac_n);
@@ -675,6 +698,7 @@
   CS_REQUIRE(h_off[0] == 0 && total >= 0, CS_ERR_INVALID, "cs_ransac_batch: bad offsets");
   CS_REQUIRE(total == 0 || (d_src && d_tgt), CS_ERR_INVALID, "cs_ransac_batch: NULL correspondences");
   RansacCall c;
+  c.d_dead = d_dead;
   if (int rc = c.init(h_off, n_prob, max_corr, ransac_n, max_iter, confidence, seed, s)) return rc;
   if (int rc = c.setup(d_src, d_tgt)) return rc;
   if (int rc = c.open_streams()) return rc;
diff --git a/corsair_amd/csrc/symcut.hip b/corsair_amd/csrc/symcut.hip
--- a/corsair_amd/csrc/symcut.hip
+++ b/corsair_amd/csrc/symcut.hip
@@ -4,6 +4,7 @@
 #include "common.h"
 #define KM_DRAWS_QUAL __device__
 #include "kmeans_draws.h"
+#include "symcut_gate.h"
 
 namespace cs {
 
@@ -646,6 +647,52 @@
                                       (double)xyz[(base + i) * 3 + 1],
                                       (double)xyz[(base + i) * 3 + 2], &dm);
   }
+}
+
+__global__ __launch_bounds__(128) void k_symcut_gate(const double* __restrict__ centers, const int32_t* __restrict__ counts,
+                                                     const double* __restrict__ min_cdist, const double* __restrict__ max_err,
+                                                     int n_anchor, const int32_t* __restrict__ meta, int n_cloud, int n_pair,
+                                                     double g0, double g1, double* __restrict__ sel, int32_t* __restrict__ ok,
+                                                     int32_t* __restrict__ pair_ok) {
+  __shared__ int side_ok[2];
+  const int p = blockIdx.x, lane = threadIdx.x & 63, side = threadIdx.x >> 6;
+  const int c = side * n_pair + p;
+  const double n = (double)meta[c];
+  const int K = meta[n_cloud + c];
+  const bool cand = meta[2 * n_cloud + c] != 0 && (K == 2 || K == 4);
+  double best = 0.0;
+  int a = 0x7fffffff;
+  if (cand)
+    for (int i = lane; i < n_anchor; i += 64) {
+      const int64_t r = (int64_t)c * n_anchor + i;
+      const double sd = gate_std(counts + r * 4, n, K);
+      if (gate_valid(min_cdist[r], max_err[r], sd, g0, g1) && (a == 0x7fffffff || sd < best)) {
+        best = sd;
+        a = i;
+      }
+    }
+#pragma unroll
+  for (int off = 32; off >= 1; off >>= 1) {
+    const double bo = __shfl_xor(best, off);
+    const int ao = __shfl_xor(a, off);
+    if (ao != 0x7fffffff && (a == 0x7fffffff || bo < best || (bo == best && ao < a))) {
+      best = bo;
+      a = ao;
+    }
+  }
+  if (lane == 0) {
+    double out[12];
+    const int good = a != 0x7fffffff;
+    if (good)
+      gate_order(centers + ((int64_t)c * n_anchor + a) * 12, K, out);
+    else
+      for (int i = 0; i < 12; ++i) out[i] = 0.0;
+    for (int i = 0; i < 12; ++i) sel[(int64_t)c * 12 + i] = out[i];
+    ok[c] = good;
+    side_ok[side] = good;
+  }
+  __syncthreads();
+  if (threadIdx.x == 0) pair_ok[p] = side_ok[0] & side_ok[1];
 }
 
 }
@@ -761,4 +808,32 @@
   return CS_OK;
 }
 
-}
+int cs_symcut_gate(const double* d_centers, const int32_t* d_counts, const double* d_min_center_dist,
+                   const double* d_max_error, int n_pair, int n_anchor, const int64_t* h_n, const int32_t* h_K,
+                   const int32_t* h_cand, double gate_min_cdist, double gate_max_err, double* d_sel, int32_t* d_ok,
+                   int32_t* d_pair_ok, void* stream) {
+  CS_REQUIRE(n_pair >= 0 && n_anchor >= 1, CS_ERR_INVALID, "cs_symcut_gate: bad counts");
+  if (n_pair == 0) return CS_OK;
+  CS_REQUIRE(d_centers && d_counts && d_min_center_dist && d_max_error && h_n && h_K && h_cand && d_sel && d_ok && d_pair_ok,
+             CS_ERR_INVALID, "cs_symcut_gate: NULL argument");
+  const int n_cloud = 2 * n_pair;
+  hipStream_t s = (hipStream_t)stream;
+  pool_use_stream(s);
+  std::vector<int32_t> meta((size_t)3 * n_cloud);
+  for (int c = 0; c < n_cloud; ++c) {
+    CS_REQUIRE(h_n[c] >= 0 && h_n[c] < (1LL << 31), CS_ERR_INVALID, "cs_symcut_gate: bad voxel count of cloud %d", c);
+    CS_REQUIRE(h_K[c] == 2 || h_K[c] == 4, CS_ERR_UNSUPPORTED, "cs_symcut_gate: K must be 2 or 4");
+    meta[c] = (int32_t)h_n[c];
+    meta[n_cloud + c] = h_K[c];
+    meta[2 * n_cloud + c] = h_cand[c] != 0;
+  }
+  PoolBuf<int32_t> d_meta(meta.size());
+  CS_REQUIRE(d_meta.p, CS_ERR_HIP, "cs_symcut_gate: scratch allocation failed");
+  CS_HIP_CHECK(hipMemcpyAsync(d_meta.p, meta.data(), sizeof(int32_t) * meta.size(), hipMemcpyHostToDevice, s));
+  hipLaunchKernelGGL(k_symcut_gate, dim3((unsigned)n_pair), dim3(128), 0, s, d_centers, d_counts, d_min_center_dist,
+                     d_max_error, n_anchor, d_meta.p, n_cloud, n_pair, gate_min_cdist, gate_max_err, d_sel, d_ok, d_pair_ok);
+  CS_LAUNCH_CHECK();
+  return CS_OK;
+}
+
+}
diff --git a/corsair_amd/csrc/symcut_gate.h b/corsair_amd/csrc/symcut_gate.h
--- /dev/null
+++ b/corsair_amd/csrc/symcut_gate.h
@@ -0,0 +1,79 @@
+#pragma once
+#include <stdint.h>
+
+#if defined(__HIPCC__)
+#define CS_GATE_FN __host__ __device__ inline
+#else
+#include <math.h>
+#define CS_GATE_FN static inline
+#endif
+
+namespace cs {
+
+CS_GATE_FN bool gate_before(double a, double b) { return a < b || (b != b && a == a); }
+
+CS_GATE_FN double gate_std(const int32_t* counts, double n, int K) {
+  double r[4];
+  double sum = 0.0;
+  for (int c = 0; c < K; ++c) {
+    r[c] = (double)counts[c] / n;
+    sum = sum + r[c];
+  }
+  const double mean = sum / (double)K;
+  double sq = 0.0;
+  for (int c = 0; c < K; ++c) {
+    const double d = r[c] - mean;
+    sq = sq + d * d;
+  }
+  return sqrt(sq / (double)K);
+}
+
+CS_GATE_FN bool gate_valid(double min_cdist, double max_err, double sd, double g0, double g1) {
+  return min_cdist > g0 && g1 > max_err && sd < 100.0;
+}
+
+CS_GATE_FN void gate_order(const double* c, int K, double* sel) {
+  for (int i = 0; i < 12; ++i) sel[i] = 0.0;
+  if (K == 2) {
+    for (int i = 0; i < 6; ++i) sel[i] = c[i];
+    return;
+  }
+  double d[3];
+  for (int i = 0; i < 3; ++i) {
+    const double x = c[0] - c[3 * (i + 1)], y = c[1] - c[3 * (i + 1) + 1], z = c[2] - c[3 * (i + 1) + 2];
+    d[i] = sqrt((x * x + y * y) + z * z);
+  }
+  int rank[3] = {0, 1, 2};
+  for (int i = 1; i < 3; ++i) {
+    const int v = rank[i];
+    int j = i;
+    while (j > 0 && gate_before(d[v], d[rank[j - 1]])) {
+      rank[j] = rank[j - 1];
+      --j;
+    }
+    rank[j] = v;
+  }
+  const int order[4] = {0, rank[0] + 1, rank[2] + 1, rank[1] + 1};
+  for (int i = 0; i < 4; ++i)
+    for (int e = 0; e < 3; ++e) sel[3 * i + e] = c[3 * order[i] + e];
+}
+
+CS_GATE_FN int symcut_gate(const double* centers, const int32_t* counts, const double* min_cdist, const double* max_err,
+                           int n_anchor, double n, int K, int cand, double g0, double g1, double* sel) {
+  for (int i = 0; i < 12; ++i) sel[i] = 0.0;
+  if (!cand || (K != 2 && K != 4)) return 0;
+  double best = 0.0;
+  int a = -1;
+  for (int i = 0; i < n_anchor; ++i) {
+    const double sd = gate_std(counts + i * 4, n, K);
+    if (gate_valid(min_cdist[i], max_err[i], sd, g0, g1) && (a < 0 || sd < best)) {
+      best = sd;
+      a = i;
+    }
+  }
+  if (a < 0) return 0;
+  gate_order(centers + (int64_t)a * 12, K, sel);
+  return 1;
+}
+
+}
diff --git a/corsair_amd/csrc/sympose.hip b/corsair_amd/csrc/sympose.hip
--- a/corsair_amd/csrc/sympose.hip
+++ b/corsair_amd/csrc/sympose.hip
@@ -100,6 +100,33 @@
   if (__any(any) && (threadIdx.x & 63) == 0) atomicOr(&bad[j], 1);
 }
 
+__global__ void k_cfg_dead_init(const int32_t* __restrict__ cfg_pair, const int32_t* __restrict__ pair_ok, int n_lead,
+                                int n_cfg, int32_t* __restrict__ dead) {
+  const int i = blockIdx.x * blockDim.x + threadIdx.x;
+  if (i >= n_lead + n_cfg) return;
+  dead[i] = i < n_lead ? 0 : (pair_ok[cfg_pair[i - n_lead]] ? 0 : 1);
+}
+
+__global__ void k_sympose_select(const double* __restrict__ cd, const int32_t* __restrict__ dead, const float* __restrict__ T,
+                                 const int64_t* __restrict__ cfg_first, int n_pair, int64_t* __restrict__ best,
+                                 float* __restrict__ T_best, double* __restrict__ cd_best) {
+  const int p = blockIdx.x * blockDim.x + threadIdx.x;
+  if (p >= n_pair) return;
+  int64_t b = p;
+  double cb = cd[p];
+  for (int64_t j = n_pair + cfg_first[p]; j < n_pair + cfg_first[p + 1]; ++j) {
+    if (dead[j]) continue;
+    const double c = cd[j];
+    if (cb > c) {
+      cb = c;
+      b = j;
+    }
+  }
+  best[p] = b;
+  cd_best[p] = cb;
+  for (int e = 0; e < 16; ++e) T_best[(int64_t)p * 16 + e] = T[b * 16 + e];
+}
+
 }
 
 using namespace cs;
@@ -151,4 +178,30 @@
   return CS_OK;
 }
 
-}
+int cs_cfg_dead(const int32_t* d_nn, int k, const int64_t* d_first, int n_cfg, const int32_t* d_cfg_pair,
+                const int32_t* d_pair_ok, int n_lead, int32_t* d_dead, void* stream) {
+  CS_REQUIRE(k >= 1 && n_cfg >= 0 && n_lead >= 0, CS_ERR_INVALID, "cs_cfg_dead: bad argument");
+  if (n_lead + n_cfg == 0) return CS_OK;
+  CS_REQUIRE(d_dead && (n_cfg == 0 || (d_nn && d_first && d_cfg_pair && d_pair_ok)), CS_ERR_INVALID,
+             "cs_cfg_dead: NULL tensor");
+  hipStream_t s = (hipStream_t)stream;
+  hipLaunchKernelGGL(k_cfg_dead_init, dim3((unsigned)ceil_div(n_lead + n_cfg, 256)), dim3(256), 0, s, d_cfg_pair, d_pair_ok,
+                     n_lead, n_cfg, d_dead);
+  if (n_cfg > 0) hipLaunchKernelGGL(k_cfg_bad, dim3(16, (unsigned)n_cfg), dim3(256), 0, s, d_nn, k, d_first, d_dead + n_lead);
+  CS_LAUNCH_CHECK();
+  return CS_OK;
+}
+
+int cs_sympose_select(const double* d_cd, const int32_t* d_dead, const float* d_T, const int64_t* d_cfg_first, int n_pair,
+                      int64_t* d_best, float* d_T_best, double* d_cd_best, void* stream) {
+  CS_REQUIRE(n_pair >= 0, CS_ERR_INVALID, "cs_sympose_select: bad argument");
+  if (n_pair == 0) return CS_OK;
+  CS_REQUIRE(d_cd && d_dead && d_T && d_cfg_first && d_best && d_T_best && d_cd_best, CS_ERR_INVALID,
+             "cs_sympose_select: NULL tensor");
+  hipLaunchKernelGGL(k_sympose_select, dim3((unsigned)ceil_div(n_pair, 64)), dim3(64), 0, (hipStream_t)stream, d_cd, d_dead,
+                     d_T, d_cfg_first, n_pair, d_best, d_T_best, d_cd_best);
+  CS_LAUNCH_CHECK();
+  return CS_OK;
+}
+
+}
diff --git a/corsair_amd/registration.py b/corsair_amd/registration.py
--- a/corsair_amd/registration.py
+++ b/corsair_amd/registration.py
@@ -118,12 +118,8 @@
                              "reference's KD-tree refuses them: %s)" % (side, int(hit[0]), said))
 
 
-def _sym_pose_batch(estimator, baseF, xyz0, off0, posF, xyz1, off1, pos_syms, k_nn=5, max_corr=0.20, seed=0,
-                    anchor_ids=None, n_anchor=100, max_iter=100000, confidence=0.999,
-                    use_symmetry=True, force_gate=False, query_anchors=None, icp_max_iter=0, icp_max_dist=None,
-                    icp_estimation="point", icp_normal_k=16, normals1=None, icp_normal_radius=None, icp_with_scaling=False,
-                    icp_scale_bounds=None, icp_kernel="l2", icp_kernel_scale=None):
-    registration, fgr_mu_floor, fgr_iterations, fgr_tuple_test, normals0, gicp_epsilon = estimator
+def _check_options(normals0, icp_max_iter, icp_max_dist, icp_estimation, icp_normal_radius, icp_with_scaling, icp_kernel,
+                   icp_kernel_scale):
     if icp_estimation == "gicp" and (icp_with_scaling or icp_kernel != "l2"):
         raise ValueError("sym_pose_batch: icp_estimation 'gicp' with icp_with_scaling or a robust icp_kernel is out of scope")
     if icp_estimation != "gicp" and normals0 is not None:
@@ -143,6 +139,43 @@
                          % (icp_normal_radius,))
     if icp_max_iter > 0 and not (icp_max_dist is not None and icp_max_dist > 0):
         raise ValueError("sym_pose_batch: icp_max_iter > 0 needs a positive icp_max_dist")
+
+
+def _refine(res, estimator, xyz0, off0, xyz1, off1, icp_max_iter, icp_max_dist, icp_estimation, icp_normal_k, normals1,
+            icp_normal_radius, icp_with_scaling, icp_scale_bounds, icp_kernel, icp_kernel_scale):
+    normals0, gicp_epsilon = estimator[4], estimator[5]
+    P = len(off0) - 1
+    if icp_max_iter > 0:
+        pairs = list(range(P))
+        nrm = None
+        if icp_estimation in ("plane", "gicp"):
+            nrm = normals1 if normals1 is not None else B.estimate_normals(xyz1, off1, icp_normal_k, icp_normal_radius)
+        scaling = {}
+        if icp_with_scaling:
+            scaling = {"with_scaling": True}
+            if icp_scale_bounds is not None:
+                scaling["scale_bounds"] = icp_scale_bounds
+        if icp_estimation == "gicp":
+            snrm = normals0 if normals0 is not None else B.estimate_normals(xyz0, off0, icp_normal_k, icp_normal_radius)
+            scaling = {"estimation": "gicp", "src_normals": snrm, "gicp_epsilon": gicp_epsilon}
+        r = B.icp_batch(xyz0, off0, xyz1, off1, pairs, pairs, res.T_best, icp_max_dist, icp_max_iter, tgt_normals=nrm,
+                        kernel=icp_kernel, kernel_scale=icp_kernel_scale, **scaling)
+        res.T_icp, res.icp_fitness, res.icp_rmse, res.icp_iters = r.T32, r.fitness, r.rmse, r.iters
+        res.icp_wfitness = r.wfitness
+        res.icp_scale = r.scale
+        res.icp_mrmse = r.mrmse
+        res.cd_icp = B.chamfer_1dir(xyz0, off0, xyz1, off1, pairs, pairs, r.T32)
+    return res
+
+
+def _sym_pose_batch_host(estimator, baseF, xyz0, off0, posF, xyz1, off1, pos_syms, k_nn=5, max_corr=0.20, seed=0,
+                         anchor_ids=None, n_anchor=100, max_iter=100000, confidence=0.999,
+                         use_symmetry=True, force_gate=False, query_anchors=None, icp_max_iter=0, icp_max_dist=None,
+                         icp_estimation="point", icp_normal_k=16, normals1=None, icp_normal_radius=None,
+                         icp_with_scaling=False, icp_scale_bounds=None, icp_kernel="l2", icp_kernel_scale=None):
+    registration, fgr_mu_floor, fgr_iterations, fgr_tuple_test, normals0, gicp_epsilon = estimator
+    _check_options(normals0, icp_max_iter, icp_max_dist, icp_estimation, icp_normal_radius, icp_with_scaling, icp_kernel,
+                   icp_kernel_scale)
     dev = baseF.device
     P = len(off0) - 1
     off0 = [int(v) for v in off0]
@@ -293,27 +326,147 @@
                         ok=ok, iters=iters, n_problems=len(prob_pair), T_all=T, cd_all=cd, inliers=inl,
                         prob_pair=prob_pair, prob_cfg=prob_cfg, best=best)
 
-    if icp_max_iter > 0:
-        pairs = list(range(P))
-        nrm = None
-        if icp_estimation in ("plane", "gicp"):
-            nrm = normals1 if normals1 is not None else B.estimate_normals(xyz1, off1, icp_normal_k, icp_normal_radius)
-        scaling = {}
-        if icp_with_scaling:
-            scaling = {"with_scaling": True}
-            if icp_scale_bounds is not None:
-                scaling["scale_bounds"] = icp_scale_bounds
-        if icp_estimation == "gicp":
-            snrm = normals0 if normals0 is not None else B.estimate_normals(xyz0, off0, icp_normal_k, icp_normal_radius)
-            scaling = {"estimation": "gicp", "src_normals": snrm, "gicp_epsilon": gicp_epsilon}
-        r = B.icp_batch(xyz0, off0, xyz1, off1, pairs, pairs, res.T_best, icp_max_dist, icp_max_iter, tgt_normals=nrm,
-                        kernel=icp_kernel, kernel_scale=icp_kernel_scale, **scaling)
-        res.T_icp, res.icp_fitness, res.icp_rmse, res.icp_iters = r.T32, r.fitness, r.rmse, r.iters
-        res.icp_wfitness = r.wfitness
-        res.icp_scale = r.scale
-        res.icp_mrmse = r.mrmse
-        res.cd_icp = B.chamfer_1dir(xyz0, off0, xyz1, off1, pairs, pairs, r.T32)
-    return res
+    return _refine(res, estimator, xyz0, off0, xyz1, off1, icp_max_iter, icp_max_dist, icp_estimation, icp_normal_k, normals1,
+                   icp_normal_radius, icp_with_scaling, icp_scale_bounds, icp_kernel, icp_kernel_scale)
+
+
+def _sym_pose_batch(estimator, baseF, xyz0, off0, posF, xyz1, off1, pos_syms, k_nn=5, max_corr=0.20, seed=0,
+                    anchor_ids=None, n_anchor=100, max_iter=100000, confidence=0.999,
+                    use_symmetry=True, force_gate=False, query_anchors=None, icp_max_iter=0, icp_max_dist=None,
+                    icp_estimation="point", icp_normal_k=16, normals1=None, icp_normal_radius=None, icp_with_scaling=False,
+                    icp_scale_bounds=None, icp_kernel="l2", icp_kernel_scale=None):
+    registration = estimator[0]
+    _check_options(estimator[4], icp_max_iter, icp_max_dist, icp_estimation, icp_normal_radius, icp_with_scaling, icp_kernel,
+                   icp_kernel_scale)
+    everything = (baseF, xyz0, off0, posF, xyz1, off1, pos_syms, k_nn, max_corr, seed, anchor_ids, n_anchor, max_iter,
+                  confidence, use_symmetry, force_gate, query_anchors, icp_max_iter, icp_max_dist, icp_estimation,
+                  icp_normal_k, normals1, icp_normal_radius, icp_with_scaling, icp_scale_bounds, icp_kernel, icp_kernel_scale)
+    if registration != "ransac" or not use_symmetry or baseF.device.type != "cuda":
+        return _sym_pose_batch_host(estimator, *everything)
+    dev = baseF.device
+    P = len(off0) - 1
+    off0 = [int(v) for v in off0]
+    off1 = [int(v) for v in off1]
+    n0 = [off0[p + 1] - off0[p] for p in range(P)]
+    n1 = [off1[p + 1] - off1[p] for p in range(P)]
+    k = k_nn
+    short = [p for p in range(P) if n0[p] > 0 and n1[p] < k]
+    if short:
+        raise IndexError("sym_pose_batch: CAD cloud of pair %d has %d voxels, fewer than k_nn = %d (the reference's "
+                         "find_kcorr fails on such a pair too)" % (short[0], n1[short[0]], k))
+
+    Ks = [4 if int(pos_syms[p]) >= 2 else 2 for p in range(P)]
+    if anchor_ids is None:
+        anchor_ids = [(2 * p, 2 * p + 1) for p in range(P)]
+    anc0 = query_anchors if query_anchors is not None else \
+        [draw_anchors(n0[p], n_anchor, anchor_ids[p][0]) for p in range(P)]
+    anc1 = [draw_anchors(n1[p], n_anchor, anchor_ids[p][1]) for p in range(P)]
+    is_cand = [int(anc0[p] is not None and anc1[p] is not None) for p in range(P)]
+    perms, cfg_pair, cfg_first = [], [], [0]
+    for p in range(P):
+        if is_cand[p]:
+            for cfg in part_configs(Ks[p], int(pos_syms[p])):
+                perms.append(cfg + [-3] * (8 - len(cfg)))
+                cfg_pair.append(p)
+        cfg_first.append(len(cfg_pair))
+    n_cfg = len(cfg_pair)
+    if n_cfg == 0:
+        return _sym_pose_batch_host(estimator, *everything[:16], anc0, *everything[17:])
+    split = os.environ.get("CORSAIR_SPLIT_RANSAC", "0") != "0"
+    lens = np.asarray([n0[p] for p in cfg_pair], dtype=np.int64)
+    row_start = np.concatenate([[0], np.cumsum(lens)])
+    n_sym = int(row_start[-1])
+    host_blk = np.concatenate([np.asarray(off0 + off1, np.int64), row_start, np.asarray(cfg_first, np.int64),
+                               np.asarray(perms, np.int32).reshape(-1).view(np.int64),
+                               np.asarray(cfg_pair + [0] * (n_cfg % 2), np.int32).view(np.int64)])
+    dev_blk = torch.from_numpy(host_blk).to(dev, non_blocking=True)
+    at = [0]
+
+    def take(n):
+        at[0] += n
+        return dev_blk[at[0] - n:at[0]]
+
+    off0_t, off1_t, first_t, cfg_first_t = take(P + 1), take(P + 1), take(n_cfg + 1), take(P + 1)
+    perm_t = take(4 * n_cfg).view(torch.int32).view(n_cfg, 8)
+    cfg_pair_t = take((n_cfg + 1) // 2).view(torch.int32)[:n_cfg]
+
+    nn = B.knn_feat(baseF, off0, posF, off1, k)
+    nonfinite = (B.cfg_bad(nn, off0_t, P), B.rows_nonfinite(posF, off1_t, P))
+    desc_v = np.asarray([[off0[p], off0[p], off1[p], n0[p], off0[p]] for p in range(P)], dtype=np.int64).reshape(P, 5)
+    prob_len = [n0[p] * k for p in range(P)] + [int(v) * k for v in lens]
+    vanilla = None
+    if split:
+        v_src, v_tgt = B.corr_assemble(xyz0, xyz1, None, nn, desc_v, off0[-1], max(n0))
+        v_offs = np.concatenate([[0], np.cumsum(prob_len[:P])]).tolist()
+        for t in (v_src, v_tgt):
+            t.record_stream(_helper.stream(dev))
+        vanilla = _helper.submit(dev, lambda: B.ransac_batch(v_src, v_tgt, v_offs, max_corr, 10, max_iter,
+                                                            confidence, seed))
+        s_src = s_tgt = None
+        lead = 0
+    else:
+        lead = off0[-1]
+        s_src = torch.empty(((lead + n_sym) * k, 3), dtype=torch.float32, device=dev)
+        s_tgt = torch.empty(((lead + n_sym) * k, 3), dtype=torch.float32, device=dev)
+        B.corr_assemble(xyz0, xyz1, None, nn, desc_v, off0[-1], max(n0), out=(s_src, s_tgt))
+
+    try:
+        def anchors_of(anc):
+            return np.stack([anc[p] if anc[p] is not None else np.zeros(n_anchor, np.int32) for p in range(P)])
+
+        a_all = torch.from_numpy(np.concatenate([anchors_of(anc0), anchors_of(anc1)])).to(dev, non_blocking=True)
+        off_all = off0 + [off0[-1] + o for o in off1[1:]]
+        xyz_all = torch.cat([xyz0, xyz1])
+        c, cnt, mcd, mer = B.symcut_fit(torch.cat([baseF, posF]), xyz_all, off_all, a_all, Ks + Ks, 50, 10, 300)
+        sel, _, pair_ok = B.symcut_gate(c, cnt, mcd, mer, n0 + n1, Ks + Ks, is_cand + is_cand,
+                                       GATE_ANY if force_gate else GATE_REFERENCE)
+        lab = B.symcut_labels(xyz_all, off_all, Ks + Ks, sel)
+        lab0, lab1 = lab[:off0[-1]], lab[off0[-1]:]
+        sorted_rows = B.partition_by_label(lab0, off0_t, P)
+        nn_cfg = B.knn_feat(baseF[sorted_rows], off0, posF, off1, k, qseg=cfg_pair, tseg=cfg_pair,
+                            qlabel=lab0[sorted_rows].contiguous(), tlabel=lab1, perm=perm_t)
+        dead = B.cfg_dead(nn_cfg, first_t, n_cfg, cfg_pair_t, pair_ok, P)
+        desc = np.stack([np.asarray([off0[p] for p in cfg_pair], np.int64), row_start[:-1],
+                         np.asarray([off1[p] for p in cfg_pair], np.int64), lens, lead + row_start[:-1]], 1)
+        s_src, s_tgt = B.corr_assemble(xyz0, xyz1, sorted_rows, nn_cfg, desc, n_sym, int(lens.max()),
+                                       out=None if split else (s_src, s_tgt))
+        offs = np.concatenate([[0], np.cumsum(prob_len[P:] if split else prob_len)]).tolist()
+        part = B.ransac_batch(s_src, s_tgt, offs, max_corr, 10, max_iter, confidence, seed,
+                              dead=dead[P:] if split else dead)
+    except BaseException:
+        if vanilla is not None:
+            try:
+                vanilla.result()
+            except Exception:
+                pass
+        raise
+    if split:
+        first = vanilla.result()
+        cur = torch.cuda.current_stream(dev)
+        for t in first:
+            t.record_stream(cur)
+        T, inl, rmse, iters = (torch.cat([a, b]) for a, b in zip(first, part))
+    else:
+        T, inl, rmse, iters = part
+
+    every_pair = list(range(P)) + cfg_pair
+    cd = B.chamfer_1dir(xyz0, off0, xyz1, off1, every_pair, every_pair, T)
+    best_t, T_best, cd_best = B.sympose_select(cd, dead, T, cfg_first_t, P)
+
+    dead_h, ok_h, best, bad_q, bad_c = to_host(dead, pair_ok, best_t, *nonfinite)
+    _refuse_nonfinite(bad_q, bad_c)
+    live = np.flatnonzero(dead_h == 0)
+    if live.size < P + n_cfg:
+        new_index = np.cumsum(dead_h == 0) - 1
+        best = new_index[best]
+        live_t = torch.from_numpy(live).to(dev)
+        T, cd, inl, iters = T[live_t], cd[live_t], inl[live_t], iters[live_t]
+    res = SymPoseResult(T_best=T_best, cd_best=cd_best, T_ransac=T[:P], cd_ransac=cd[:P], ok=ok_h > 0, iters=iters,
+                        n_problems=int(live.size), T_all=T, cd_all=cd, inliers=inl,
+                        prob_pair=[every_pair[j] for j in live],
+                        prob_cfg=[None] * P + [[c for c in perms[j - P] if c >= 0] for j in live[P:]], best=best)
+    return _refine(res, estimator, xyz0, off0, xyz1, off1, icp_max_iter, icp_max_dist, icp_estimation, icp_normal_k, normals1,
+                   icp_normal_radius, icp_with_scaling, icp_scale_bounds, icp_kernel, icp_kernel_scale)
 
 
 def sym_pose_batch(*args, registration="ransac", fgr_mu_floor=0.025, fgr_iterations=64, fgr_tuple_test=True, **kwargs):
diff --git a/include/corsair_hip.h b/include/corsair_hip.h
--- a/include/corsair_hip.h
+++ b/include/corsair_hip.h
@@ -105,6 +105,10 @@
                     double max_corr, int ransac_n, int max_iter, double confidence, uint64_t seed,
                     float* d_T, int32_t* d_inliers, double* d_rmse, int32_t* d_iters,
                     void* stream);
+int cs_ransac_batch_masked(const float* d_src, const float* d_tgt, const int64_t* h_off, int n_prob,
+                           double max_corr, int ransac_n, int max_iter, double confidence, uint64_t seed,
+                           const int32_t* d_dead, float* d_T, int32_t* d_inliers, double* d_rmse, int32_t* d_iters,
+                           void* stream);
 void cs_ransac_prefilter_stats(uint64_t out[5], int reset);
 
 int cs_symcut_fit(const float* d_feat, int dim, const float* d_xyz, const int64_t* h_off,
@@ -114,10 +118,18 @@
                   void* stream);
 int cs_symcut_labels(const float* d_xyz, const int64_t* h_off, int n_cloud, const int32_t* h_K,
                      const double* d_sel_centers, int32_t* d_labels, void* stream);
+int cs_symcut_gate(const double* d_centers, const int32_t* d_counts, const double* d_min_center_dist,
+                   const double* d_max_error, int n_pair, int n_anchor, const int64_t* h_n, const int32_t* h_K,
+                   const int32_t* h_cand, double gate_min_cdist, double gate_max_err, double* d_sel, int32_t* d_ok,
+                   int32_t* d_pair_ok, void* stream);
 
 int cs_partition_by_label(const int32_t* d_label, const int64_t* d_off, int n_cloud, int64_t* d_order, void* stream);
 int cs_cfg_bad(const int32_t* d_nn, int k, const int64_t* d_first, int n_cfg, int32_t* d_bad, void* stream);
 int cs_rows_nonfinite(const float* d_x, int dim, const int64_t* d_first, int n_seg, int32_t* d_bad, void* stream);
+int cs_cfg_dead(const int32_t* d_nn, int k, const int64_t* d_first, int n_cfg, const int32_t* d_cfg_pair,
+                const int32_t* d_pair_ok, int n_lead, int32_t* d_dead, void* stream);
+int cs_sympose_select(const double* d_cd, const int32_t* d_dead, const float* d_T, const int64_t* d_cfg_first, int n_pair,
+                      int64_t* d_best, float* d_T_best, double* d_cd_best, void* stream);
 int cs_corr_assemble(const float* d_xyz0, const float* d_xyz1, const int64_t* d_rows, const int32_t* d_nn, int k,
                      const int64_t* d_desc, int n_cfg, int64_t max_len, float* d_src, float* d_tgt, void* stream);
 
```

Result: no change. 2127, median of 2 (+0.3%).
